# PengfeiRen96/DIR

Measured on AMD Instinct MI355X. Metric: images/sec at 256x256 bs=64, 3 stage outputs (DIR.forward eval), higher is better.
Workload: dtype f16

## Files before the change

### dir_amd/_capi.py

```python
import ctypes as C
import os

_HERE = os.path.dirname(os.path.abspath(__file__))
LIB_PATH = os.environ.get('DIR_LIB_PATH') or os.path.join(_HERE, 'lib', 'libdir_hip.so')
_lib = None


class DirHipError(RuntimeError):
    pass


class ManoTables(C.Structure):
    _fields_ = [('shapedirs_t', C.c_void_p), ('posedirs_t', C.c_void_p), ('v_template', C.c_void_p),
                ('j_template', C.c_void_p), ('j_shapedirs', C.c_void_p), ('weights', C.c_void_p), ('hands_mean', C.c_void_p),
                ('comps', C.c_void_p), ('side', C.c_int32), ('center_idx', C.c_int32), ('root_palm', C.c_int32)]


class ConvDesc(C.Structure):
    _fields_ = [(n, C.c_int32) for n in (
        'B', 'H', 'W', 'Cin', 'in_cstride', 'in_coff', 'Cout', 'out_cstride', 'out_coff', 'res_cstride', 'res_coff',
        'kh', 'kw', 'stride', 'pad', 'in_dtype', 'out_dtype', 'flags', 'Ho', 'Wo')] + [('in_scale', C.c_float), ('out_split_scale', C.c_float)]


class ConvBnBwd(C.Structure):
    _fields_ = [(n, C.c_void_p) for n in ('z', 'mean', 'rstd', 'w', 'b')] + [('relu', C.c_int32)] + [(n, C.c_void_p) for n in ('p1', 'p2')]


class ConvSrc2(C.Structure):
    _fields_ = [(n, C.c_int32) for n in ('H', 'W', 'Cin', 'in_cstride', 'in_coff', 'stride')]


class TrainWeight(C.Structure):
    _fields_ = [(n, C.c_void_p) for n in ('w', 'fwd', 'fwd_scale', 'dgrad', 'dgrad_scale')] + [(n, C.c_int32) for n in ('Cout', 'Cin', 'kh', 'kw')] + [
        ('fwd_inv_in', C.c_float), ('dgrad_inv_in', C.c_float)]


class BneckChainParams(C.Structure):
    _fields_ = [(n, C.c_void_p) for n in ('w2', 'scale2', 'shift2', 'w3', 'scale3', 'shift3', 'w1n', 'scale1n', 'shift1n', 'wd')] + [
        ('n_next', C.c_int32), ('out_decimate', C.c_int32), ('dtype', C.c_int32)]


class BneckTailParams(C.Structure):
    _fields_ = [(n, C.c_void_p) for n in ('wstream', 'scale3', 'shift3', 'scale1n', 'shift1n')] + [('planes', C.c_int32), ('n_next', C.c_int32), ('waves', C.c_int32), ('dtype', C.c_int32)]


class ResChainParams(C.Structure):
    _fields_ = [(n, C.c_void_p) for n in ('w1', 'w2', 'w3', 'pre_scale', 'pre_shift', 'scale1', 'shift1', 'scale2', 'shift2', 'shift3')] + [
        (n, C.c_int32) for n in ('Cin', 'Cmid', 'Cout', 'dtype')]


class GemmDesc(C.Structure):
    _fields_ = [(n, C.c_int32) for n in ('M', 'N', 'K', 'lda', 'ldb', 'ldc', 'trans_a', 'trans_b', 'accumulate', 'batch')] + \
               [(n, C.c_int64) for n in ('stride_a', 'stride_b', 'stride_c')]


class GemmGroups(C.Structure):
    _fields_ = [(n, C.c_int32) for n in ('ny', 'nx', 'reduce', 'reserved')] + [(n, C.c_int64) for n in ('a_y', 'a_x', 'b_y', 'b_x', 'c_y', 'c_x')]


class TokenMlp(C.Structure):
    _fields_ = [(n, C.c_void_p) for n in ('w1t', 's1', 'b1', 'w2t', 'b2')]


class PgcnLayer(C.Structure):
    _fields_ = [(n, C.c_void_p) for n in ('W', 'e1', 'bias', 'bn_scale', 'bn_shift')] + [('relu', C.c_int32), ('w_dtype', C.c_int32)]


class SteBlock(C.Structure):
    _fields_ = [(n, C.c_void_p) for n in ('ln1_w', 'ln1_b', 'qkv_wt', 'qkv_b', 'proj_wt', 'proj_b', 'ln2_w', 'ln2_b',
                                          'fc1_wt', 'fc1_b', 'fc2_wt', 'fc2_b')]


class SteParams(C.Structure):
    _fields_ = [('pos_embed', C.c_void_p), ('blocks', SteBlock * 3), ('num_blocks', C.c_int32)] + \
               [(n, C.c_void_p) for n in ('snorm_w', 'snorm_b', 'head_ln_w', 'head_ln_b', 'head_wt', 'head_b')] + \
               [('weight_dtype', C.c_int32)]


class RegressParams(C.Structure):
    _fields_ = [('mano_wt', C.c_void_p), ('mano_b', C.c_void_p * 2), ('off_w', C.c_void_p), ('off_b', C.c_void_p),
                ('emb', TokenMlp)]


class InitHeadParams(C.Structure):
    _fields_ = [('attn_w', C.c_void_p * 2), ('attn_b', C.c_float * 2), ('mano_wt', C.c_void_p),
                ('mano_b', C.c_void_p * 2), ('off_w', C.c_void_p), ('off_b', C.c_void_p)]


class BoneFusionParams(C.Structure):
    _fields_ = [(n, C.c_void_p) for n in ('w_g', 'scale', 'shift')] + [('exact_f32', C.c_int32), ('g_scale', C.c_float)]


class EvalInputs(C.Structure):
    _fields_ = [('verts_pd', C.c_void_p * 2), ('pd_offset', C.c_void_p), ('verts_gt', C.c_void_p * 2),
                ('verts2d_gt', C.c_void_p * 2), ('cam', C.c_void_p), ('jr', C.c_void_p * 2)]


class LossPred(C.Structure):
    _fields_ = [('joint_uv', C.c_void_p * 2), ('mesh_uv', C.c_void_p * 2), ('proj', C.c_void_p * 2), ('joint_xyz', C.c_void_p * 2),
                ('mesh_xyz', C.c_void_p * 2), ('offset', C.c_void_p)]


class LossTarget(C.Structure):
    _fields_ = [('joint_2d', C.c_void_p * 2), ('mesh_2d', C.c_void_p * 2), ('joint_3d', C.c_void_p * 2),
                ('mesh_3d', C.c_void_p * 2), ('center', C.c_void_p * 2), ('faces', C.c_void_p * 2),
                ('c2', C.c_int32), ('n_faces', C.c_int32)]


class LossPredGrad(C.Structure):
    _fields_ = [('joint_uv', C.c_void_p * 2), ('mesh_uv', C.c_void_p * 2), ('joint_xyz', C.c_void_p * 2),
                ('mesh_xyz', C.c_void_p * 2), ('offset', C.c_void_p)]


class EvalOutputs(C.Structure):
    _fields_ = [(n, C.c_void_p) for n in ('joint_err', 'vert_err', 'joint2d_err', 'vert2d_err', 'joints_pd', 'joints_gt',
                                          'root_err')]


class ValMetricsDesc(C.Structure):
    _fields_ = [('joints_pd', (C.c_void_p * 2) * 8), ('verts_pd', (C.c_void_p * 2) * 8), ('joints_gt', C.c_void_p * 2),
                ('verts_gt', C.c_void_p * 2), ('sample_sums', C.c_void_p), ('acc', C.c_void_p), ('batches', C.c_void_p)]


class FrameDesc(C.Structure):
    _fields_ = [('offset', C.c_longlong), ('height', C.c_int32), ('width', C.c_int32), ('row_stride', C.c_longlong)]


class OneEuroSegment(C.Structure):
    _fields_ = [('n_points', C.c_int32), ('dims', C.c_int32), ('speed_scale', C.c_float)]


class RenderLights(C.Structure):
    _fields_ = [('ambient', C.c_float * 3), ('diffuse', C.c_float * 3), ('specular', C.c_float * 3), ('location', C.c_float * 3),
                ('shininess', C.c_float)]


ABI_VERSION = 48
DT_F32, DT_BF16, DT_F16X3, DT_F16X1, DT_F16X3P, DT_F16X1P, DT_F16 = 0, 1, 3, 4, 5, 6, 7
CONV_RELU, CONV_PRE_RELU = 1, 2

_p, _i = C.c_void_p, C.c_int
_SIGNATURES = {
    'dir_abi_version': (C.c_int, []),
    'dir_last_error': (C.c_char_p, []),
    'dir_device_info': (C.c_int, [C.c_char_p, _i, C.POINTER(C.c_int)]),
    'dir_launch_log_reset': (None, []),
    'dir_launch_log_get': (C.c_int, [C.c_char_p, _i]),
    'dir_launch_log_note': (None, [C.c_char_p, C.c_longlong]),
    'dir_probe_launch': (C.c_longlong, [_i, _p, C.c_longlong, _i, _p]),
    'dir_conv2d_forward': (C.c_int, [C.POINTER(ConvDesc), _p, _p, _p, _p, _p, _p, _p, _p, _p]),
    'dir_conv2d_forward_stats': (C.c_int, [C.POINTER(ConvDesc), _p, _p, _p, _p, _p, _p, _p, _p, _p, C.POINTER(C.c_int), _p]),
    'dir_conv2d_forward_masked': (C.c_int, [C.POINTER(ConvDesc), _p, _p, _p, _p, _p, _p, _p, _p, _p, _p]),
    'dir_conv2d_forward_ex': (C.c_int, [C.POINTER(ConvDesc), _p, _p, _p, _p, _p, _p, _p, _p, _p, C.POINTER(ConvBnBwd), C.POINTER(C.c_int), _p]),
    'dir_add_upsampled': (C.c_int, [_p, _p, _i, _i, _i, _i, _i, _i, _i, _p]),
    'dir_fuse_sum': (C.c_int, [_p, _p, _p, _p, _i, _i, _i, _i, _i, _i, _i, _p]),
    'dir_pack_f16x3_weights': (C.c_int, [_p, _p, _p, _p, _i, _i, _p]),
    'dir_train_pack_conv_weights': (C.c_int, [_p, _p, _i, _i, _p]),
    'dir_gemm_f32_splitk_workspace_bytes': (C.c_longlong, [C.POINTER(GemmDesc)]),
    'dir_gemm_f32_splitk': (C.c_int, [C.POINTER(GemmDesc), _p, _p, _p, _p, _p, C.c_longlong, _p]),
    'dir_axpy_multi_f32': (C.c_int, [_p, _p, _p, _i, C.c_float, _p]),
    'dir_split_f16_forward': (C.c_int, [_p, _p, C.c_longlong, _i, _i, _i, _p, _p, _i, C.c_float, _i, _p]),
    'dir_stem_prep': (C.c_int, [_p, _p, _i, _i, _i, _i, _i, _i, _i, _p]),
    'dir_stem_prep_s2d': (C.c_int, [_p, _p, _i, _i, _i, _i, _i, _i, _p]),
    'dir_image_normalize_forward': (C.c_int, [_p, _p, C.POINTER(C.c_float), C.POINTER(C.c_float), _i, _i, _i, _p]),
    'dir_stem_prep_s2d_u8': (C.c_int, [_p, _p, C.POINTER(C.c_float), C.POINTER(C.c_float), _i, _i, _i, _i, _i, _i, _p]),
    'dir_adamw_step': (C.c_int, [_p, _p, _p, _p, C.c_longlong, C.c_double, C.c_double, C.c_double, C.c_double, C.c_double,
                                 C.c_longlong, _p]),
    'dir_stage_losses_backward': (C.c_int, [C.POINTER(LossPred), C.POINTER(LossTarget), C.c_float, _p, C.POINTER(C.c_void_p * 2),
                                            C.POINTER(C.c_void_p * 2), C.POINTER(LossPredGrad), _i, _p]),
    'dir_dense_losses_backward_workspace_bytes': (C.c_longlong, [_i, _i]),
    'dir_dense_losses_backward': (C.c_int, [_p, _p, _p, _p, C.POINTER(C.c_float), C.c_float, _p, _p, C.c_longlong, _p, _p, _i, _i, _i, _i, _p]),
    'dir_stage_losses_forward': (C.c_int, [C.POINTER(LossPred), C.POINTER(LossTarget), C.c_float, _p, _p, _i, _p]),
    'dir_dense_losses_workspace_bytes': (C.c_longlong, [_i, _i]),
    'dir_dense_losses_forward': (C.c_int, [_p, _p, _p, _p, C.POINTER(C.c_float), C.c_float, _p, C.c_longlong, _p, _i, _i, _i, _i, _p]),
    'dir_bottleneck_chain_forward': (C.c_int, [C.POINTER(BneckChainParams), _p, _p, _p, _p, _p, _i, _i, _i, _p]),
    'dir_bottleneck_tail_forward': (C.c_int, [C.POINTER(BneckTailParams), _p, _p, _p, _p, C.c_longlong, _p]),
    'dir_residual_chain_supported': (C.c_int, [_i] * 11),
    'dir_residual_chain_forward': (C.c_int, [C.POINTER(ResChainParams), _p, _p, _i, _i, _i, _i, _i, _i, _i, _p]),
    'dir_stem_pool_forward': (C.c_int, [_p, _i, C.POINTER(C.c_float), C.POINTER(C.c_float), _p, _p, _p, _p, _i, _i, _i, _p]),
    'dir_stem_pool_forward_dt': (C.c_int, [_p, _i, _i, C.POINTER(C.c_float), C.POINTER(C.c_float), _p, _p, _p, _p, _i, _i, _i, _p]),
    'dir_maxpool3x3s2': (C.c_int, [_p, _p, _i, _i, _i, _i, _i, _p]),
    'dir_upsample2x_bilinear': (C.c_int, [_p, _p, _i, _i, _i, _i, _i, _i, _i, _p]),
    'dir_init_head_forward': (C.c_int, [C.POINTER(InitHeadParams), _p, _p, _p, _i, _p, _p, _p, _i, _i, _i, _i, _i, _p]),
    'dir_bone_proj_forward': (C.c_int, [_p, _p, _p, _p, _p, _p, _i, _i, C.c_float, _i, _p]),
    'dir_conv2d_dual_forward': (C.c_int, [C.POINTER(ConvDesc), _p, C.POINTER(ConvSrc2), _p, _p, _p, _p, _p]),
    'dir_conv2d_dual_scaled_forward': (C.c_int, [C.POINTER(ConvDesc), _p, C.POINTER(ConvSrc2), _p, _p, _p, _p, _p, _p]),
    'dir_conv1x1_stream_forward': (C.c_int, [C.POINTER(ConvDesc), _p, C.POINTER(ConvSrc2), _p, _p, _p, _p, _p, _p, _p, _p]),
    'dir_conv2d_as_supported': (C.c_int, [C.POINTER(ConvDesc), _i, _i]),
    'dir_conv2d_as_forward': (C.c_int, [C.POINTER(ConvDesc), _p, _p, _p, _p, _p, _p, _i, _i, _p]),
    'dir_conv2d_as_chain_supported': (C.c_int, [C.POINTER(ConvDesc), _i, _i]),
    'dir_conv2d_as_chain_forward': (C.c_int, [C.POINTER(ConvDesc), _p, _p, _p, _p, _p, _p, _p, _i, _i, _p, _i, _i, _i, _p]),
    'dir_conv2d_sparse_forward': (C.c_int, [C.POINTER(ConvDesc), _p, _p, _p, _p, _p, _p, _p, _p]),
    'dir_grid_tokens_forward': (C.c_int, [_p, _i, _i, _i, _i, _i, _p, _p, _p, _p, _p, C.POINTER(TokenMlp),
                                          C.POINTER(TokenMlp), C.POINTER(TokenMlp), _p, _p, _i, _p]),
    'dir_pgcn_stack_forward': (C.c_int, [C.POINTER(PgcnLayer), _i, _p, _p, _p, C.c_longlong, _p, _i, _p]),
    'dir_pgcn_stack_forward_pair': (C.c_int, [C.POINTER(PgcnLayer), C.POINTER(PgcnLayer), _i, _p, _p, _p, _p, _i, _p]),
    'dir_pgcn_fused_sync_bytes': (C.c_longlong, []),
    'dir_pgcn_stack_forward_fused': (C.c_int, [C.POINTER(PgcnLayer), C.POINTER(PgcnLayer), _i, _p, _p, _p, _p, _p, _i, _i, _p]),
    'dir_ste_forward': (C.c_int, [C.POINTER(SteParams), _p, _p, _p, _i, _p]),
    'dir_regress_forward': (C.c_int, [C.POINTER(RegressParams), _p, _p, _p, _p, _p, _p, _p, _p, _i, _p]),
    'dir_bone_fusion_scratch_bytes': (C.c_size_t, [_i]),
    'dir_bone_fusion_prepare': (C.c_int, [C.POINTER(BoneFusionParams), _p, _p, _i, _p]),
    'dir_bone_fusion_forward': (C.c_int, [C.POINTER(BoneFusionParams), _p, _p, _p, _p, _i, _i, C.c_float, _i, _i, _i, _p]),
    'dir_bone_fusion_backward_workspace_bytes': (C.c_longlong, [_i, _i]),
    'dir_bone_fusion_backward': (C.c_int, [_p, _p, _p, _p, _p, _p, C.c_float, _p, _p, _p, _p, _p, C.c_longlong, _i, _i, _p]),
    'dir_gt_mano_forward': (C.c_int, [C.POINTER(ManoTables), _p, _p, _i, _p, _p, _p, _i, _i, _p, _p, _i, _p]),
    'dir_joint_regress_forward': (C.c_int, [_p, _p, _p, _i, _p]),
    'dir_eval_metrics_forward': (C.c_int, [C.POINTER(EvalInputs), C.POINTER(EvalOutputs), _i, _i, _i, _p]),
    'dir_val_metrics_forward': (C.c_int, [C.POINTER(ValMetricsDesc), _i, _i, _p]),
    'dir_mano_forward_pair': (C.c_int, [C.POINTER(ManoTables), _p, _i, _p, _i, _p, _i, _p, _p, _p, _p, _p, _i, _p]),
    'dir_mano_backward_pair': (C.c_int, [C.POINTER(ManoTables), _p, _i, _p, _i, _p, _i, _p, _p, _p, _p, _p, _i, _p, _i, _p, _i, _i, _i, _p]),
    'dir_regress_backward': (C.c_int, [_p] * 17 + [_i, _p]),
    'dir_gemm_f32': (C.c_int, [C.POINTER(GemmDesc), _p, _p, _p, _p, _p]),
    'dir_gemm_f32_grouped': (C.c_int, [C.POINTER(GemmDesc), C.POINTER(GemmGroups), _p, _p, _p, _p, _p]),
    'dir_colsum_workspace_bytes': (C.c_longlong, [_i, _i]),
    'dir_colsum_f32': (C.c_int, [_p, _p, _i, _i, _i, _i, _p, C.c_longlong, _p]),
    'dir_layernorm_forward': (C.c_int, [_p, _p, _p, _p, _p, _p, _i, _i, C.c_float, _p]),
    'dir_layernorm_backward': (C.c_int, [_p, _p, _p, _p, _p, _p, _p, _p, _i, _i, _i, _i, _p]),
    'dir_gelu_forward': (C.c_int, [_p, _p, C.c_longlong, _p]),
    'dir_gelu_backward': (C.c_int, [_p, _p, _p, C.c_longlong, _p]),
    'dir_attention_forward': (C.c_int, [_p, _p, _p, _i, _i, _i, C.c_float, _p]),
    'dir_attention_backward': (C.c_int, [_p, _p, _p, _p, _i, _i, _i, C.c_float, _p]),
    'dir_bn_train_workspace_bytes': (C.c_longlong, [_i, _i]),
    'dir_bn_train_forward': (C.c_int, [_p, _p, _p, _p, _p, _p, _p, _p, _i, _i, _i, C.c_float, C.c_float, _i, _p, _p, C.c_longlong, _p]),
    'dir_bn_train_backward_from_partials': (C.c_int, [_p, _p, _p, _p, _p, _p, _p, _p, _i, _p, _p, _p, _i, _i, _i, _i, _p, C.c_longlong, _p]),
    'dir_bn_train_stats': (C.c_int, [_p, _p, _p, _p, _p, _p, _p, _p, _p, _i, _i, _i, C.c_float, C.c_float, _p, C.c_longlong, _p]),
    'dir_bn_train_stats_from_partials': (C.c_int, [_p, _p, _i, _i, _p, _p, _p, _p, _p, _p, _p, _p, _i, _i, C.c_float, C.c_float, _p]),
    'dir_bn_train_apply': (C.c_int, [_p, _p, _p, _p, _p, _p, _i, _i, _i, _i, _p, _p]),
    'dir_bn_train_forward_from_partials': (C.c_int, [_p, _p, _p, _i, _i, _p, _p, _p, _p, _p, _p, _p, _i, _i, _i, C.c_float, C.c_float, _i, _p, _p]),
    'dir_bn_one_launch_status': (C.c_int, []),
    'dir_upsample_nearest_add_f32': (C.c_int, [_p, _p, _i, _i, _i, _i, _i, _p]),
    'dir_upsample_nearest_backward_f32': (C.c_int, [_p, _p, _i, _i, _i, _i, _i, _p]),
    'dir_bn_one_launch_enable': (C.c_int, [_i]),
    'dir_bn_train_backward': (C.c_int, [_p, _p, _p, _p, _p, _p, _p, _p, _p, _i, _i, _i, _i, _p, C.c_longlong, _p]),
    'dir_bn_frozen_workspace_bytes': (C.c_longlong, [_i, _i]),
    'dir_bn_sync_workspace_bytes': (C.c_longlong, [_i, _i]),
    'dir_bn_sync_local_stats': (C.c_int, [_p, _p, _i, _i, _i, _p, C.c_longlong, _p]),
    'dir_bn_sync_combine': (C.c_int, [_p, _i, _i, _p, _p, _p, _p, C.c_float, _p]),
    'dir_bn_sync_backward_sums': (C.c_int, [_p, _p, _p, _p, _p, _p, _p, _i, _i, _i, _i, _p, C.c_longlong, _p]),
    'dir_bn_sync_backward_apply': (C.c_int, [_p, _p, _p, _p, _p, _p, _p, _p, _i, C.c_float, _i, _i, _i, _p]),
    'dir_bn_frozen_forward': (C.c_int, [_p, _p, _p, _p, _p, _p, _p, _p, _i, _i, _i, C.c_float, _i, _p, _p]),
    'dir_bn_frozen_backward': (C.c_int, [_p, _p, _p, _p, _p, _p, _p, _p, _p, _i, _i, _i, _i, _p, C.c_longlong, _p]),
    'dir_relu_forward': (C.c_int, [_p, _p, C.c_longlong, _p]),
    'dir_relu_backward': (C.c_int, [_p, _p, _p, C.c_longlong, _p]),
    'dir_pgcn_adjacency_forward': (C.c_int, [_p, _p, _p]),
    'dir_pgcn_adjacency_backward': (C.c_int, [_p, _p, _p, _p, _p, _i, _p]),
    'dir_conv2d_splitk_workspace_bytes': (C.c_longlong, [C.POINTER(ConvDesc), _i]),
    'dir_conv2d_splitk_forward': (C.c_int, [C.POINTER(ConvDesc), _p, _p, _p, _p, _p, _p, _p, _p, _i, _p, C.c_longlong, _p]),
    'dir_conv2d_wgrad_workspace_bytes': (C.c_longlong, [C.POINTER(ConvDesc)]),
    'dir_conv2d_wgrad_f32': (C.c_int, [C.POINTER(ConvDesc), _p, _p, _p, _i, _p, C.c_longlong, _p]),
    'dir_conv2d_wgrad_f16x3_workspace_bytes': (C.c_longlong, [C.POINTER(ConvDesc)]),
    'dir_conv2d_wgrad_f16x3': (C.c_int, [C.POINTER(ConvDesc), _p, _p, _p, _i, _p, C.c_longlong, C.c_float, C.c_float, _p]),
    'dir_conv2d_wgrad_f16x3_pre': (C.c_int, [C.POINTER(ConvDesc), _p, _p, _p, _i, _p, C.c_longlong, C.c_float, C.c_float, _p, _p, _i, _p]),
    'dir_maxpool3x3s2_backward': (C.c_int, [_p, _p, _p, _i, _i, _i, _i, _p]),
    'dir_upsample2x_bilinear_backward': (C.c_int, [_p, _p, _i, _i, _i, _i, _i, _i, _p]),
    'dir_attn_pool_forward': (C.c_int, [_p, _p, _p, _p, _p, _i, _i, _i, _p]),
    'dir_attn_pool_backward': (C.c_int, [_p, _p, _p, _p, _p, _p, _p, _i, _i, _i, _i, _p]),
    'dir_bone_proj_backward_scratch_bytes': (C.c_longlong, [_i, _i]),
    'dir_bone_proj_backward': (C.c_int, [_p, _p, _p, _i, _i, C.c_float, _p, _p, _p, _i, _i, _i, _p]),
    'dir_axpy_f32': (C.c_int, [_p, _p, C.c_longlong, C.c_float, _p]),
    'dir_stage_positions': (C.c_int, [_p, _p, _p, _p, _p, _p, _p, _i, _p]),
    'dir_grid_rows_forward': (C.c_int, [_p, _p, _p, _i, _i, _i, _p]),
    'dir_grid_rows_backward': (C.c_int, [_p, _p, _i, _p, _i, _i, _i, _i, _p]),
    'dir_mano_forward': (C.c_int, [C.POINTER(ManoTables), _p, _i, _p, _i, _p, _i, _p, _p, _p, _p, _p, _i, _p]),
    'dir_jpeg_planes_bytes': (C.c_longlong, [C.c_longlong]),
    'dir_jpeg_decode_records': (C.c_int, [_p, C.c_longlong, _i, _i, _i, _p, C.c_longlong, _p, _p, _p]),
    'dir_train_noise_field': (C.c_int, [C.c_ulonglong, _p, _i, _p]),
    'dir_train_augment_images': (C.c_int, [_p, _p, _p, _p, _p, C.c_ulonglong, C.POINTER(C.c_float), C.POINTER(C.c_float), _p, _p, _p, _p, _p,
                                           _p, _i, _p]),
    'dir_train_augment_labels': (C.c_int, [_p, C.POINTER(C.c_void_p * 8), _p, C.POINTER(C.c_void_p * 10), _i, _p]),
    'dir_render_workspace_bytes': (C.c_longlong, [_i]),
    'dir_render_two_hands': (C.c_int, [_p, _p, _p, _p, _i, _i, _p, C.c_longlong, _p, _p, _p, _p, _p, _p, _p]),
    'dir_render_adjacency_bytes': (C.c_longlong, []),
    'dir_render_adjacency': (C.c_int, [_p, _p, C.c_longlong, _p]),
    'dir_render_vertex_normals': (C.c_int, [_p, _p, _p, _i, _p, _p]),
    'dir_render_shaded_workspace_bytes': (C.c_longlong, [_i]),
    'dir_render_joints': (C.c_int, [_p, _p, _p, _i, _i, C.c_float, C.c_float, _p]),
    'dir_render_shaded': (C.c_int, [_p, _p, _p, _p, _p, _p, _p, C.POINTER(RenderLights), _p, _i, _i, _p, C.c_longlong, _p, _p, _p, _p, _p, _p]),
    'dir_mesh_penetration': (C.c_int, [_p, _p, _p, _p, _i, _i, _i, _i, _i, _p, _p, _p, _p, _p, _p]),
    'dir_mesh_intersection_volume': (C.c_int, [_p, _p, _p, _p, _i, _i, _i, _i, _i, C.c_float, _i, _p, _p, _p, _p]),
    'dir_procrustes_align': (C.c_int, [_p, _p, _i, _i, _i, _p, _p, _p, _p]),
    'dir_point_set_nn': (C.c_int, [_p, _p, _i, _i, _i, _p, _p, _p]),
    'dir_threshold_counts': (C.c_int, [_p, C.c_longlong, _p, _i, _p, _p]),
    'dir_crop_matrices_from_boxes': (C.c_int, [_p, _i, C.c_double, _i, _p, _p, _p]),
    'dir_crop_matrices_from_meshes': (C.c_int, [_p, _p, _p, _p, _p, _i, C.c_double, _i, _p, _p, _p]),
    'dir_crop_frames': (C.c_int, [_p, C.c_longlong, _p, _p, _p, _i, _i, _p, _p, _p]),
    'dir_crop_frames_area': (C.c_int, [_p, C.c_longlong, _p, _p, _p, _i, _i, _p, _p, _p, _p]),
    'dir_one_euro_state_bytes': (C.c_longlong, [_i, _i, C.POINTER(C.c_longlong)]),
    'dir_one_euro_step': (C.c_int, [_p, _p, _i, C.POINTER(OneEuroSegment), _i, C.c_double, C.c_double, C.c_double, C.c_double, _i, _p, _p, _p, _p]),
}


PROFILE = None
_pending = {}
_NO_PROFILE = ('dir_conv2d_as_supported', 'dir_conv2d_as_chain_supported', 'dir_residual_chain_supported', 'dir_abi_version', 'dir_bn_one_launch_status', 'dir_bn_one_launch_enable', 'dir_last_error', 'dir_device_info', 'dir_launch_log_reset', 'dir_launch_log_get', 'dir_launch_log_note',
               'dir_bone_fusion_scratch_bytes', 'dir_dense_losses_workspace_bytes', 'dir_dense_losses_backward_workspace_bytes',
               'dir_gemm_f32_splitk_workspace_bytes', 'dir_bn_train_workspace_bytes', 'dir_bn_sync_workspace_bytes', 'dir_bn_frozen_workspace_bytes', 'dir_jpeg_planes_bytes', 'dir_render_workspace_bytes', 'dir_render_adjacency_bytes', 'dir_render_shaded_workspace_bytes', 'dir_colsum_workspace_bytes', 'dir_conv2d_wgrad_workspace_bytes', 'dir_conv2d_wgrad_f16x3_workspace_bytes',
               'dir_one_euro_state_bytes')


def annotate(**kw):
    if PROFILE is not None:
        _pending.update(kw)


class _ProfLib(object):
    def __init__(self, l):
        self._l = l

    def __getattr__(self, name):
        fn = getattr(self._l, name)
        if name in _NO_PROFILE:
            return fn
        import torch

        def call(*args):
            e0, e1 = torch.cuda.Event(enable_timing=True), torch.cuda.Event(enable_timing=True)
            self._l.dir_launch_log_reset()
            e0.record()
            rc = fn(*args)
            e1.record()
            buf = C.create_string_buffer(1024)
            self._l.dir_launch_log_get(buf, 1024)
            rec = dict(_pending, api=name, kernels=buf.value.decode(), e0=e0, e1=e1)
            _pending.clear()
            PROFILE.append(rec)
            return rc
        return call


def lib():
    global _lib
    if _lib is not None and PROFILE is not None:
        return _ProfLib(_lib)
    if _lib is None:
        import torch
        if not os.path.exists(LIB_PATH):
            raise DirHipError('%s is missing: build it with `python -c "import __graft_entry__ as g; g.build()"` '
                              '(or python dir_amd/build.py). There is no CPU fallback.' % LIB_PATH)
        l = C.CDLL(LIB_PATH)
        for name, (res, args) in _SIGNATURES.items():
            fn = getattr(l, name)
            fn.restype, fn.argtypes = res, args
        if l.dir_abi_version() != ABI_VERSION:
            raise DirHipError('libdir_hip.so ABI version %d != %d' % (l.dir_abi_version(), ABI_VERSION))
        _lib = l
    return _ProfLib(_lib) if PROFILE is not None else _lib


def check(rc, what):
    if rc != 0:
        raise DirHipError('%s failed (%d): %s' % (what, rc, lib().dir_last_error().decode()))


def ptr(t):
    return None if t is None else C.c_void_p(t.data_ptr())


def stream_ptr():
    import torch
    return C.c_void_p(torch.cuda.current_stream().cuda_stream)


def require_cuda(*tensors):
    for t in tensors:
        if t is not None and not t.is_cuda:
            raise DirHipError('dir_amd kernels run on the GPU only: got a %s tensor (no CPU fallback exists)'
                              % t.device)


def f32c(t):
    import torch
    if t.dtype != torch.float32:
        t = t.float()
    return t if t.is_contiguous() else t.contiguous()
```

### dir_amd/csrc/tail.hip

```cpp
#include "conv_common.h"

namespace dir {
namespace {

using convk::bf16_t;
using convk::f16s_t;
using convk::f32x16;
using convk::Half;
typedef __attribute__((ext_vector_type(4))) float f32x4;

#ifndef DIR_TAIL_RES16
#define DIR_TAIL_RES16 1
#endif
#ifndef DIR_TAIL_NT
#define DIR_TAIL_NT 0
#endif
#if DIR_TAIL_NT
typedef unsigned __attribute__((ext_vector_type(2))) u32x2_t;
typedef unsigned __attribute__((ext_vector_type(4))) u32x4_t;
__device__ __forceinline__ uint2 nt_load2(const uint2* p) { const u32x2_t v = __builtin_nontemporal_load(reinterpret_cast<const u32x2_t*>(p)); return make_uint2(v.x, v.y); }
__device__ __forceinline__ void nt_store4(uint4 v, uint4* p) { __builtin_nontemporal_store(u32x4_t{v.x, v.y, v.z, v.w}, reinterpret_cast<u32x4_t*>(p)); }
#define NT_LOAD(p) nt_load2(p)
#define NT_STORE(v, p) nt_store4(v, p)
#else
#define NT_LOAD(p) (*(p))
#define NT_STORE(v, p) (*(p) = (v))
#endif

constexpr int TM = 64;
constexpr int HC = 512;
constexpr int NTHR = 512;
constexpr int TPITCH = HC * 2 + 16;

struct TailArgs {
    const bf16_t* y2; const bf16_t* res; bf16_t* out; bf16_t* y1n;
    const uint4* wstream;
    const float* sc3; const float* sh3; const float* sc1n; const float* sh1n;
    int ntiles; unsigned y2_bytes;
};

template <typename H> __device__ __forceinline__ void unpack4(uint2 v, float (&f)[4]) {
    convk::unpack2<H>(v.x, f[0], f[1]);
    convk::unpack2<H>(v.y, f[2], f[3]);
}

template <int P, int N2, typename H = bf16_t>
__global__ __launch_bounds__(NTHR, 1) void tail_chain_kernel(TailArgs a) {
    convk::half_kernel_init<H>();
    constexpr int C4 = 4 * P, NH = C4 / HC;
    constexpr int YROW = P * 2;
    constexpr int GRP = P == 256 ? 4 : 8;
    constexpr int KBS = P / 16;
    constexpr int NBF = 2 * KBS;
    constexpr bool C16 = N2 == 128;
    constexpr int NCF = C16 ? HC / 32 : HC / 16;
    constexpr int NF = NBF + NCF, NG = NF / GRP;
    static_assert(NF % GRP == 0 && C4 % HC == 0 && (N2 == 128 || N2 == 256), "tail_chain_kernel: unsupported geometry");
    constexpr int YCH = TM * (P / 8) / NTHR;
    __shared__ __attribute__((aligned(16))) char s_t[TM * TPITCH];
    __shared__ __attribute__((aligned(16))) char s_y2[2][TM * YROW];
    __shared__ __attribute__((aligned(16))) float s_ss[2 * C4 + 2 * N2];
    const int tid = threadIdx.x, lane = tid & 63, wave = __builtin_amdgcn_readfirstlane(tid >> 6);
    const int l32 = lane & 31, h = lane >> 5, l16 = lane & 15, g16 = lane >> 4;

    for (int i = tid; i < C4; i += NTHR) { s_ss[i] = a.sc3[i]; s_ss[C4 + i] = a.sh3[i]; }
    for (int i = tid; i < N2; i += NTHR) { s_ss[2 * C4 + i] = a.sc1n[i]; s_ss[2 * C4 + N2 + i] = a.sh1n[i]; }

    const int tstep = gridDim.x;
    int t = blockIdx.x;
    if (t >= a.ntiles) return;

    const convk::i32x4 yd = {(int)(unsigned)(unsigned long long)a.y2, (int)(unsigned)((unsigned long long)a.y2 >> 32), (int)a.y2_bytes, 0x00020000};
    const unsigned y2_lds = (unsigned)(unsigned long long)(__attribute__((address_space(3))) char*)&s_y2[0][0];
    auto y2_dma = [&](int tile, int buf) {
#pragma unroll
        for (int i = 0; i < YCH; ++i) {
            const int slot = (8 * i + wave) * 64 + lane, px = slot / (P / 8), pos = slot % (P / 8);
            const unsigned voff = (unsigned)(((long long)tile * TM + px) * YROW) + (unsigned)((pos ^ (px & 15)) * 16);
            convk::lds_dma16_m0(yd, y2_lds + buf * (TM * YROW) + (8 * i + wave) * 1024, voff, 0);
        }
    };
#if DIR_TAIL_RES16
    uint4 xr[2][2][2];
    auto res_fetch = [&](int tile, int half) {
#pragma unroll
        for (int pb = 0; pb < 2; ++pb) {
            const bf16_t* rp = a.res + ((long long)tile * TM + 32 * pb + l32) * C4 + half * HC + 64 * wave + 8 * h;
#pragma unroll
            for (int cb = 0; cb < 2; ++cb)
#pragma unroll
                for (int j = 0; j < 2; ++j) xr[cb][pb][j] = *reinterpret_cast<const uint4*>(rp + 32 * cb + 16 * j);
        }
#else
    uint2 xr[2][2][4];
    auto res_fetch = [&](int tile, int half) {
#pragma unroll
        for (int pb = 0; pb < 2; ++pb) {
            const bf16_t* rp = a.res + ((long long)tile * TM + 32 * pb + l32) * C4 + half * HC + 64 * wave + 4 * h;
#pragma unroll
            for (int cb = 0; cb < 2; ++cb)
#pragma unroll
                for (int q = 0; q < 4; ++q) xr[cb][pb][q] = NT_LOAD(reinterpret_cast<const uint2*>(rp + 32 * cb + 8 * q));
        }
#endif
    };
    uint4 ring[2][GRP];
    auto ring_load = [&](auto Slot, int hf, int grp) {
        constexpr int slot = decltype(Slot)::value;
        const uint4* p = a.wstream + ((long long)(hf * 8 + wave) * NF + grp * GRP) * 64 + lane;
#pragma unroll
        for (int i = 0; i < GRP; ++i) ring[slot][i] = p[i * 64];
    };

    y2_dma(t, 0);
    ring_load(std::integral_constant<int, 0>{}, 0, 0);
    res_fetch(t, 0);
    convk::wait_vmcnt<0>();
    __syncthreads();
    int ybuf = 0;

    f32x16 accb[2];
    f32x16 accc32[C16 ? 1 : 2];
    f32x4 accc16[C16 ? 4 : 1];
    constexpr int NOP = C16 ? 4 : 2;
    uint4 bop[2][NOP];
    const char* ycur = s_y2[0];
    auto act_read = [&](auto F, auto Set) {
        constexpr int f = decltype(F)::value, set = decltype(Set)::value;
        if constexpr (f < NBF) {
            constexpr int ks = f % KBS;
#pragma unroll
            for (int pb = 0; pb < 2; ++pb)
                bop[set][pb] = *reinterpret_cast<const uint4*>(ycur + (32 * pb + l32) * YROW + (((2 * ks + h) ^ (l32 & 15)) << 4));
        } else {
            constexpr int fc = f - NBF;
            if constexpr (C16) {
#pragma unroll
                for (int u = 0; u < 4; ++u) bop[set][u] = *reinterpret_cast<const uint4*>(s_t + (16 * u + l16) * TPITCH + 64 * fc + 16 * g16);
            } else {
#pragma unroll
                for (int pb = 0; pb < 2; ++pb) bop[set][pb] = *reinterpret_cast<const uint4*>(s_t + (32 * pb + l32) * TPITCH + 32 * fc + 16 * h);
            }
        }
    };

    for (; t < a.ntiles; t += tstep) {
        const bool more = t + tstep < a.ntiles;
        if (more) y2_dma(t + tstep, ybuf ^ 1);
        ycur = s_y2[ybuf];
#pragma nounroll
        for (int hf = 0; hf < NH; ++hf) {
            const bool last_half = hf == NH - 1;
            if (hf == 0) {
                if constexpr (C16) {
#pragma unroll
                    for (int u = 0; u < 4; ++u) accc16[u] = f32x4{0.f, 0.f, 0.f, 0.f};
                } else {
#pragma unroll
                    for (int pb = 0; pb < 2; ++pb)
#pragma unroll
                        for (int r = 0; r < 16; ++r) accc32[pb][r] = 0.f;
                }
            }
            act_read(std::integral_constant<int, 0>{}, std::integral_constant<int, 0>{});
            [&]<int... G>(std::integer_sequence<int, G...>) {
                (([&] {
                     constexpr int grp = G, slot = G & 1;
                     if constexpr (grp + 1 < NG) ring_load(std::integral_constant<int, slot ^ 1>{}, hf, grp + 1);
                     else ring_load(std::integral_constant<int, slot ^ 1>{}, last_half ? 0 : hf + 1, 0);
                     [&]<int... I>(std::integer_sequence<int, I...>) {
                         (([&] {
                              constexpr int f = grp * GRP + I, set = f & 1;
                              if constexpr (f + 1 < NF && f + 1 != NBF) act_read(std::integral_constant<int, f + 1>{}, std::integral_constant<int, set ^ 1>{});
                              if constexpr (f < NBF) {
                                  constexpr int cb = f / KBS, ks = f - cb * KBS;
                                  if constexpr (ks == 0) {
#pragma unroll
                                      for (int pb = 0; pb < 2; ++pb)
#pragma unroll
                                          for (int r = 0; r < 16; ++r) accb[pb][r] = 0.f;
                                  }
#pragma unroll
                                  for (int pb = 0; pb < 2; ++pb)
                                      accb[pb] = Half<H>::mfma32(ring[slot][I], bop[set][pb], accb[pb]);
                                  if constexpr (ks == KBS - 1) {
#pragma unroll
                                      for (int q = 0; q < 4; ++q) {
                                          const int cl = 64 * wave + 32 * cb + 8 * q + 4 * h;
                                          const float4 sc = *reinterpret_cast<const float4*>(s_ss + hf * HC + cl);
                                          const float4 sh = *reinterpret_cast<const float4*>(s_ss + C4 + hf * HC + cl);
#pragma unroll
                                          for (int pb = 0; pb < 2; ++pb) {
                                              float v[4] = {fmaf(accb[pb][4 * q], sc.x, sh.x), fmaf(accb[pb][4 * q + 1], sc.y, sh.y),
                                                            fmaf(accb[pb][4 * q + 2], sc.z, sh.z), fmaf(accb[pb][4 * q + 3], sc.w, sh.w)};
                                              float rv[4];
#if DIR_TAIL_RES16
                                              {
                                                  const uint4 c = xr[cb][pb][q >> 1];
                                                  const auto sx = __builtin_amdgcn_permlane32_swap(c.x, c.z, false, false);
                                                  const auto sy = __builtin_amdgcn_permlane32_swap(c.y, c.w, false, false);
                                                  unpack4<H>(make_uint2(sx[q & 1], sy[q & 1]), rv);
                                              }
#else
                                              unpack4<H>(xr[cb][pb][q], rv);
#endif
#pragma unroll
                                              for (int e = 0; e < 4; ++e) v[e] += rv[e];
                                              uint2 o;
                                              o.x = Half<H>::pack2_relu(v[0], v[1]);
                                              o.y = Half<H>::pack2_relu(v[2], v[3]);
                                              *reinterpret_cast<uint2*>(s_t + (32 * pb + l32) * TPITCH + cl * 2) = o;
                                          }
                                          __builtin_amdgcn_sched_barrier(0);
                                      }
                                  }
                                  if constexpr (f == NBF - 1) {
                                      __syncthreads();
                                      act_read(std::integral_constant<int, NBF>{}, std::integral_constant<int, set ^ 1>{});
                                      if (!last_half) res_fetch(t, hf + 1);
                                      else if (more) res_fetch(t + tstep, 0);
#pragma unroll
                                      for (int i = 0; i < TM * (HC / 8) / NTHR; ++i) {
                                          const int c = tid + NTHR * i;
                                          NT_STORE(*reinterpret_cast<const uint4*>(s_t + (c >> 6) * TPITCH + (c & 63) * 16),
                                                   reinterpret_cast<uint4*>(a.out + ((long long)t * TM + (c >> 6)) * C4 + hf * HC + (c & 63) * 8));
                                          if (i & 1) __builtin_amdgcn_sched_barrier(0);
                                      }
                                  }
                              } else {
                                  if constexpr (C16) {
#pragma unroll
                                      for (int u = 0; u < 4; ++u)
                                          accc16[u] = Half<H>::mfma16(ring[slot][I], bop[set][u], accc16[u]);
                                  } else {
#pragma unroll
                                      for (int pb = 0; pb < 2; ++pb)
                                          accc32[pb] = Half<H>::mfma32(ring[slot][I], bop[set][pb], accc32[pb]);
                                  }
                              }
                              if constexpr (f == NF - 1) convk::wait_vmcnt<GRP>();
                              __builtin_amdgcn_sched_barrier(0);
                          }()),
                          ...);
                     }(std::make_integer_sequence<int, GRP>{});
                 }()),
                 ...);
            }(std::make_integer_sequence<int, NG>{});
            if (last_half) {
                if constexpr (C16) {
                    const int c0 = 16 * wave + 4 * g16;
                    const float4 sc = *reinterpret_cast<const float4*>(s_ss + 2 * C4 + c0);
                    const float4 sh = *reinterpret_cast<const float4*>(s_ss + 2 * C4 + N2 + c0);
#pragma unroll
                    for (int u = 0; u < 4; ++u) {
                        uint2 o;
                        o.x = Half<H>::pack2_relu(fmaf(accc16[u][0], sc.x, sh.x), fmaf(accc16[u][1], sc.y, sh.y));
                        o.y = Half<H>::pack2_relu(fmaf(accc16[u][2], sc.z, sh.z), fmaf(accc16[u][3], sc.w, sh.w));
                        *reinterpret_cast<uint2*>(a.y1n + ((long long)t * TM + 16 * u + l16) * N2 + c0) = o;
                    }
                } else {
#pragma unroll
                    for (int pb = 0; pb < 2; ++pb) {
                        uint2 o[4];
#pragma unroll
                        for (int q = 0; q < 4; ++q) {
                            const int c0 = 32 * wave + 8 * q + 4 * h;
                            const float4 sc = *reinterpret_cast<const float4*>(s_ss + 2 * C4 + c0);
                            const float4 sh = *reinterpret_cast<const float4*>(s_ss + 2 * C4 + N2 + c0);
                            o[q].x = Half<H>::pack2_relu(fmaf(accc32[pb][4 * q], sc.x, sh.x), fmaf(accc32[pb][4 * q + 1], sc.y, sh.y));
                            o[q].y = Half<H>::pack2_relu(fmaf(accc32[pb][4 * q + 2], sc.z, sh.z), fmaf(accc32[pb][4 * q + 3], sc.w, sh.w));
                        }
#if DIR_TAIL_RES16
#pragma unroll
                        for (int j = 0; j < 2; ++j) {
                            const auto dx = __builtin_amdgcn_permlane32_swap(o[2 * j].x, o[2 * j + 1].x, false, false);
                            const auto dy = __builtin_amdgcn_permlane32_swap(o[2 * j].y, o[2 * j + 1].y, false, false);
                            *reinterpret_cast<uint4*>(a.y1n + ((long long)t * TM + 32 * pb + l32) * N2 + 32 * wave + 16 * j + 8 * h) = make_uint4(dx[0], dy[0], dx[1], dy[1]);
                        }
#else
#pragma unroll
                        for (int q = 0; q < 4; ++q)
                            *reinterpret_cast<uint2*>(a.y1n + ((long long)t * TM + 32 * pb + l32) * N2 + 32 * wave + 8 * q + 4 * h) = o[q];
#endif
                    }
                }
            }
            __syncthreads();
        }
        ybuf ^= 1;
    }
}


constexpr int TTM = 32, TTHR = 256;

template <int P, int N2, typename H = bf16_t>
__global__ __launch_bounds__(TTHR, 2) void tail_thin_kernel(TailArgs a) {
    convk::half_kernel_init<H>();
    constexpr int C4 = 4 * P, NH = C4 / HC;
    constexpr int YROW = P * 2;
    constexpr int GRP = 8;
    constexpr int KBS = P / 16;
    constexpr int NBF = 4 * KBS;
    constexpr int NCC = N2 / 128;
    constexpr int NCF = 32 * NCC;
    constexpr int NF = NBF + NCF, NG = NF / GRP;
    static_assert(NF % GRP == 0 && NG % 2 == 0 && C4 % HC == 0 && (N2 == 128 || N2 == 256), "tail_thin_kernel: unsupported geometry");
    constexpr int YCH = TTM * (P / 8) / TTHR;
    __shared__ __attribute__((aligned(16))) char s_t[TTM * TPITCH];
    __shared__ __attribute__((aligned(16))) char s_y2[2][TTM * YROW];
    __shared__ __attribute__((aligned(16))) float s_ss[2 * C4 + 2 * N2];
    const int tid = threadIdx.x, lane = tid & 63, wave = __builtin_amdgcn_readfirstlane(tid >> 6);
    const int l32 = lane & 31, h = lane >> 5;

    for (int i = tid; i < C4; i += TTHR) { s_ss[i] = a.sc3[i]; s_ss[C4 + i] = a.sh3[i]; }
    for (int i = tid; i < N2; i += TTHR) { s_ss[2 * C4 + i] = a.sc1n[i]; s_ss[2 * C4 + N2 + i] = a.sh1n[i]; }

    const int tstep = gridDim.x;
    int t = blockIdx.x;
    if (t >= a.ntiles) return;

    const convk::i32x4 yd = {(int)(unsigned)(unsigned long long)a.y2, (int)(unsigned)((unsigned long long)a.y2 >> 32), (int)a.y2_bytes, 0x00020000};
    const unsigned y2_lds = (unsigned)(unsigned long long)(__attribute__((address_space(3))) char*)&s_y2[0][0];
    auto y2_dma = [&](int tile, int buf) {
#pragma unroll
        for (int i = 0; i < YCH; ++i) {
            const int slot = (4 * i + wave) * 64 + lane, px = slot / (P / 8), pos = slot % (P / 8);
            const unsigned voff = (unsigned)(((long long)tile * TTM + px) * YROW) + (unsigned)((pos ^ (px & 15)) * 16);
            convk::lds_dma16_m0(yd, y2_lds + buf * (TTM * YROW) + (4 * i + wave) * 1024, voff, 0);
        }
    };
    uint2 xr[4][4];
    auto res_fetch = [&](int tile, int half) {
        const bf16_t* rp = a.res + ((long long)tile * TTM + l32) * C4 + half * HC + 128 * wave + 4 * h;
#pragma unroll
        for (int cb = 0; cb < 4; ++cb)
#pragma unroll
            for (int q = 0; q < 4; ++q) xr[cb][q] = NT_LOAD(reinterpret_cast<const uint2*>(rp + 32 * cb + 8 * q));
    };
    uint4 ring[2][GRP];
    auto ring_load = [&](auto Slot, int hf, int grp) {
        constexpr int slot = decltype(Slot)::value;
        const uint4* p = a.wstream + ((long long)(hf * 4 + wave) * NF + grp * GRP) * 64 + lane;
#pragma unroll
        for (int i = 0; i < GRP; ++i) ring[slot][i] = p[i * 64];
    };

    y2_dma(t, 0);
    ring_load(std::integral_constant<int, 0>{}, 0, 0);
    res_fetch(t, 0);
    convk::wait_vmcnt<0>();
    __syncthreads();
    int ybuf = 0;

    f32x16 accb;
    f32x16 accc[NCC];
    uint4 bop[2];
    const char* ycur = s_y2[0];
    auto act_read = [&](auto F, auto Set) {
        constexpr int f = decltype(F)::value, set = decltype(Set)::value;
        if constexpr (f < NBF) {
            constexpr int ks = f % KBS;
            bop[set] = *reinterpret_cast<const uint4*>(ycur + l32 * YROW + (((2 * ks + h) ^ (l32 & 15)) << 4));
        } else {
            constexpr int ks = (f - NBF) / NCC;
            bop[set] = *reinterpret_cast<const uint4*>(s_t + l32 * TPITCH + 32 * ks + 16 * h);
        }
    };

    for (; t < a.ntiles; t += tstep) {
        const bool more = t + tstep < a.ntiles;
        if (more) y2_dma(t + tstep, ybuf ^ 1);
        ycur = s_y2[ybuf];
#pragma nounroll
        for (int hf = 0; hf < NH; ++hf) {
            const bool last_half = hf == NH - 1;
            if (hf == 0) {
#pragma unroll
                for (int cc = 0; cc < NCC; ++cc)
#pragma unroll
                    for (int r = 0; r < 16; ++r) accc[cc][r] = 0.f;
            }
            act_read(std::integral_constant<int, 0>{}, std::integral_constant<int, 0>{});
            [&]<int... G>(std::integer_sequence<int, G...>) {
                (([&] {
                     constexpr int grp = G, slot = G & 1;
                     if constexpr (grp + 1 < NG) ring_load(std::integral_constant<int, slot ^ 1>{}, hf, grp + 1);
                     else ring_load(std::integral_constant<int, slot ^ 1>{}, last_half ? 0 : hf + 1, 0);
                     [&]<int... I>(std::integer_sequence<int, I...>) {
                         (([&] {
                              constexpr int f = grp * GRP + I;
                              constexpr bool same_next = f >= NBF && f + 1 < NF && (f - NBF) / NCC == (f + 1 - NBF) / NCC;
                              constexpr int set = f < NBF ? (f & 1) : ((((f - NBF) / NCC) + NBF) & 1);
                              if constexpr (f + 1 < NF && f + 1 != NBF && !same_next)
                                  act_read(std::integral_constant<int, f + 1>{}, std::integral_constant<int, set ^ 1>{});
                              if constexpr (f < NBF) {
                                  constexpr int cb = f / KBS, ks = f - cb * KBS;
                                  if constexpr (ks == 0) {
#pragma unroll
                                      for (int r = 0; r < 16; ++r) accb[r] = 0.f;
                                  }
                                  accb = Half<H>::mfma32(ring[slot][I], bop[set], accb);
                                  if constexpr (ks == KBS - 1) {
#pragma unroll
                                      for (int q = 0; q < 4; ++q) {
                                          const int cl = 128 * wave + 32 * cb + 8 * q + 4 * h;
                                          const float4 sc = *reinterpret_cast<const float4*>(s_ss + hf * HC + cl);
                                          const float4 sh = *reinterpret_cast<const float4*>(s_ss + C4 + hf * HC + cl);
                                          float v[4] = {fmaf(accb[4 * q], sc.x, sh.x), fmaf(accb[4 * q + 1], sc.y, sh.y),
                                                        fmaf(accb[4 * q + 2], sc.z, sh.z), fmaf(accb[4 * q + 3], sc.w, sh.w)};
                                          float rv[4];
                                          unpack4<H>(xr[cb][q], rv);
#pragma unroll
                                          for (int e = 0; e < 4; ++e) v[e] += rv[e];
                                          uint2 o;
                                          o.x = Half<H>::pack2_relu(v[0], v[1]);
                                          o.y = Half<H>::pack2_relu(v[2], v[3]);
                                          *reinterpret_cast<uint2*>(s_t + l32 * TPITCH + cl * 2) = o;
                                      }
                                  }
                                  if constexpr (f == NBF - 1) {
                                      __syncthreads();
                                      act_read(std::integral_constant<int, NBF>{}, std::integral_constant<int, (NBF & 1)>{});
                                      if (!last_half) res_fetch(t, hf + 1);
                                      else if (more) res_fetch(t + tstep, 0);
#pragma unroll
                                      for (int i = 0; i < TTM * (HC / 8) / TTHR; ++i) {
                                          const int c = tid + TTHR * i;
                                          NT_STORE(*reinterpret_cast<const uint4*>(s_t + (c >> 6) * TPITCH + (c & 63) * 16),
                                                   reinterpret_cast<uint4*>(a.out + ((long long)t * TTM + (c >> 6)) * C4 + hf * HC + (c & 63) * 8));
                                          if (i & 1) __builtin_amdgcn_sched_barrier(0);
                                      }
                                  }
                              } else {
                                  constexpr int cc = (f - NBF) % NCC;
                                  accc[cc] = Half<H>::mfma32(ring[slot][I], bop[set], accc[cc]);
                              }
                              if constexpr (f == NF - 1) convk::wait_vmcnt<GRP>();
                              __builtin_amdgcn_sched_barrier(0);
                          }()),
                          ...);
                     }(std::make_integer_sequence<int, GRP>{});
                 }()),
                 ...);
            }(std::make_integer_sequence<int, NG>{});
            if (last_half) {
#pragma unroll
                for (int cc = 0; cc < NCC; ++cc)
#pragma unroll
                    for (int q = 0; q < 4; ++q) {
                        const int c0 = (N2 / 4) * wave + 32 * cc + 8 * q + 4 * h;
                        const float4 sc = *reinterpret_cast<const float4*>(s_ss + 2 * C4 + c0);
                        const float4 sh = *reinterpret_cast<const float4*>(s_ss + 2 * C4 + N2 + c0);
                        uint2 o;
                        o.x = Half<H>::pack2_relu(fmaf(accc[cc][4 * q], sc.x, sh.x), fmaf(accc[cc][4 * q + 1], sc.y, sh.y));
                        o.y = Half<H>::pack2_relu(fmaf(accc[cc][4 * q + 2], sc.z, sh.z), fmaf(accc[cc][4 * q + 3], sc.w, sh.w));
                        *reinterpret_cast<uint2*>(a.y1n + ((long long)t * TTM + l32) * N2 + c0) = o;
                    }
            }
            __syncthreads();
        }
        ybuf ^= 1;
    }
}

}
}

extern "C" int dir_bottleneck_tail_forward(const dir_bneck_tail_params* p, const void* y2, const void* residual, void* out, void* y1_next,
                                           long long M, void* stream) {
    using namespace dir;
    DIR_REQUIRE(p && y2 && residual && out && y1_next, "dir_bottleneck_tail_forward: null pointer");
    DIR_REQUIRE(p->wstream && p->scale3 && p->shift3 && p->scale1n && p->shift1n, "dir_bottleneck_tail_forward: missing parameters");
    DIR_REQUIRE(M > 0 && M % TM == 0 && M / TM < (1ll << 31), "dir_bottleneck_tail_forward: M must be a positive multiple of 64");
    DIR_REQUIRE(p->waves == 8 || p->waves == 4, "dir_bottleneck_tail_forward: the stream must be packed for 8 or 4 waves");
    DIR_REQUIRE(p->dtype == 0 || p->dtype == DIR_DT_BF16 || p->dtype == DIR_DT_F16, "dir_bottleneck_tail_forward: dtype must be bf16 (or 0) or f16");
    const bool f16 = p->dtype == DIR_DT_F16;
    TailArgs a;
    a.y2 = (const convk::bf16_t*)y2; a.res = (const convk::bf16_t*)residual; a.out = (convk::bf16_t*)out; a.y1n = (convk::bf16_t*)y1_next;
    a.wstream = (const uint4*)p->wstream; a.sc3 = p->scale3; a.sh3 = p->shift3; a.sc1n = p->scale1n; a.sh1n = p->shift1n;
    a.ntiles = (int)(M / TM);
    DIR_REQUIRE(M * p->planes * 2 < (1ll << 31), "dir_bottleneck_tail_forward: y2 must be < 2 GiB (32-bit buffer offsets)");
    a.y2_bytes = (unsigned)(M * p->planes * 2);
    static int num_cu = 0;
    if (!num_cu) {
        int dev = 0; hipDeviceProp_t pr;
        num_cu = (hipGetDevice(&dev) == hipSuccess && hipGetDeviceProperties(&pr, dev) == hipSuccess) ? pr.multiProcessorCount : 256;
    }
    hipStream_t s = (hipStream_t)stream;
    if (p->waves == 4) {
        a.ntiles = (int)(M / TTM);
        const int grid4 = a.ntiles < 2 * num_cu ? a.ntiles : 2 * num_cu;
#define DIR_TAIL4(P_, N2_) do { if (f16) DIR_LAUNCH((tail_thin_kernel<P_, N2_, f16s_t>), dim3(grid4), dim3(TTHR), 0, s, a); \
                                 else DIR_LAUNCH((tail_thin_kernel<P_, N2_, bf16_t>), dim3(grid4), dim3(TTHR), 0, s, a); } while (0)
        if (p->planes == 128 && p->n_next == 128) DIR_TAIL4(128, 128);
        else if (p->planes == 128 && p->n_next == 256) DIR_TAIL4(128, 256);
        else if (p->planes == 256 && p->n_next == 256) DIR_TAIL4(256, 256);
        else DIR_REQUIRE(false, "dir_bottleneck_tail_forward: (planes, n_next) must be (128,128), (128,256) or (256,256)");
#undef DIR_TAIL4
        return check_launch("dir_bottleneck_tail_forward");
    }
    const int grid = a.ntiles < num_cu ? a.ntiles : num_cu;
#define DIR_TAIL(P_, N2_) do { if (f16) DIR_LAUNCH((tail_chain_kernel<P_, N2_, f16s_t>), dim3(grid), dim3(NTHR), 0, s, a); \
                                else DIR_LAUNCH((tail_chain_kernel<P_, N2_, bf16_t>), dim3(grid), dim3(NTHR), 0, s, a); } while (0)
    if (p->planes == 128 && p->n_next == 128) DIR_TAIL(128, 128);
    else if (p->planes == 128 && p->n_next == 256) DIR_TAIL(128, 256);
    else if (p->planes == 256 && p->n_next == 256) DIR_TAIL(256, 256);
    else DIR_REQUIRE(false, "dir_bottleneck_tail_forward: (planes, n_next) must be (128,128), (128,256) or (256,256)");
#undef DIR_TAIL
    return check_launch("dir_bottleneck_tail_forward");
}
```

### dir_amd/engine.py

```python
import ctypes as C
import math
import json
import os
import threading

import torch

from . import _capi
from ._capi import CONV_PRE_RELU, CONV_RELU, DT_BF16, DT_F16, DT_F16X1, DT_F16X1P, DT_F16X3, DT_F16X3P, DT_F32, ConvDesc

F32 = torch.float32
IMAGENET_MEAN = (C.c_float * 3)(0.485, 0.456, 0.406)
IMAGENET_STD = (C.c_float * 3)(0.229, 0.224, 0.225)
_TLS = threading.local()


def _forced_variant():
    return getattr(_TLS, 'variant', None)


def _packing_arith():
    return getattr(_TLS, 'arith', None)


def _ann(family, flops, nbytes, shape):
    if _capi.PROFILE is not None:
        _capi.annotate(family=family, flops=float(flops), bytes=float(nbytes), shape=shape)


HALF = (torch.bfloat16, torch.float16)


def _dt(dtype):
    return DT_F32 if dtype == torch.float32 else DT_F16 if dtype == torch.float16 else DT_BF16


def _tok_wdt(dtype):
    return torch.bfloat16 if dtype in HALF else torch.float32


def bn_fold(sd, prefix, conv_bias=None, eps=1e-5):
    g, b = sd[prefix + '.weight'].double(), sd[prefix + '.bias'].double()
    m, v = sd[prefix + '.running_mean'].double(), sd[prefix + '.running_var'].double()
    scale = g / torch.sqrt(v + eps)
    shift = b - m * scale
    if conv_bias is not None:
        shift = shift + conv_bias.double() * scale
    return scale.float().contiguous(), shift.float().contiguous()


STREAM_VARIANT = 21
STREAM64_VARIANT = 22
STREAM32_VARIANT = 23
STREAMP_VARIANT = 24
STREAM_VARIANTS = (STREAM_VARIANT, STREAM64_VARIANT, STREAM32_VARIANT, STREAMP_VARIANT)
AS_VARIANTS = {25: (2, 2), 26: (2, 4), 27: (4, 2), 28: (1, 2)}


def pack_as_weights(w_ohwi, A):
    N, kh, kw, Cin = w_ohwi.shape
    assert N % (128 * A) == 0 and Cin % 64 == 0
    nt = kh * kw
    dev = w_ohwi.device
    w = w_ohwi.reshape(N, nt * Cin)
    lane = torch.arange(64, device=dev)
    l32, h = lane & 31, lane >> 5
    e = torch.arange(8, device=dev)
    g, wv, st, ks, cb = torch.meshgrid(torch.arange(N // (128 * A), device=dev), torch.arange(4, device=dev), torch.arange(nt * Cin // 64, device=dev),
                                       torch.arange(4, device=dev), torch.arange(A, device=dev), indexing='ij')
    row = (g * (128 * A) + (wv * A + cb) * 32)[..., None] + l32
    slab, tap = st // nt, st % nt
    k0 = (tap * Cin + 64 * slab + 8 * ks)[..., None] + 32 * h
    return w[row[..., None], k0[..., None] + e].contiguous()


def pack_stream_weights(w_nk, dtype=torch.bfloat16):
    out_dev = w_nk.device
    w = w_nk.detach().float().cpu()
    N, K = w.shape
    assert N % 128 == 0 and K % 64 == 0
    ncb = 2 if N % 256 == 0 else 1
    dev = w.device
    lane = torch.arange(64, device=dev)
    l32, h = lane & 31, lane >> 5
    e = torch.arange(8, device=dev)
    g, wv, c, ks, cb = torch.meshgrid(torch.arange(N // (128 * ncb), device=dev), torch.arange(4, device=dev), torch.arange(K // 64, device=dev),
                                      torch.arange(4, device=dev), torch.arange(ncb, device=dev), indexing='ij')
    row = (g * (128 * ncb) + (wv * ncb + cb) * 32)[..., None] + l32
    k0 = (64 * c + 8 * ks)[..., None] + 32 * h
    return w[row[..., None], k0[..., None] + e].to(dtype).contiguous().to(out_dev)


class ConvOp(object):
    def __init__(self, w_oihw, dtype, stride=1, pad=0, scale=None, shift=None, relu=False, pre=None, pre_relu=False,
                 out_dtype=None, arith=None):
        self.w = w_oihw.detach().permute(0, 2, 3, 1).contiguous().to(dtype)
        self.cout, self.kh, self.kw, self.cin = self.w.shape
        self.stride, self.pad, self.dtype = stride, pad, dtype
        self.out_dtype = out_dtype or dtype
        self.arith = (arith or _packing_arith()) if dtype == torch.float32 else None
        self.in_code = DT_F16X3 if self.arith == 'f16x3' else DT_F16X1 if self.arith == 'f16' else _dt(dtype)
        self.in_scale = 1.0
        if self.arith in ('f16x3', 'f16'):
            from .functional import pack_f16x3_weights
            self.w, scale = pack_f16x3_weights(self.w.reshape(self.cout, -1), scale)
            self.scale0 = scale.float().contiguous().clone()
        self.scale = None if scale is None else scale.float().contiguous()
        self.shift = None if shift is None else shift.float().contiguous()
        self.pre_scale, self.pre_shift = (None, None) if pre is None else (pre[0].contiguous(), pre[1].contiguous())
        self.flags = (CONV_RELU if relu else 0) | (CONV_PRE_RELU if pre_relu else 0)
        self.ho = self.wo = 0
        self.in_cs_override = None
        self.presplit = self.arith is not None and (ConvOp.PRESPLIT == 2 or (ConvOp.PRESPLIT == 1 and (
            self.kh * self.kw >= 9 or (self.cout >= 512 and self.cin >= 128))))
        self.split_consumer = None
        self.alg_k = self.kh * self.kw * self.cin
        self.variant = {}
        self.split, self._ws = {}, {}
        self._w_as = {}
        self.w_stream = None
        if (dtype in HALF and self.out_dtype == dtype and self.kh == 1 and self.kw == 1 and stride == 1 and pad == 0
                and self.cin % 64 == 0 and self.cout % 128 == 0 and self.cin <= 2304):
            self.w_stream = pack_stream_weights(self.w.reshape(self.cout, self.cin), dtype)

    PRESPLIT = int(os.environ.get('DIR_PRESPLIT', '1'))
    OUT_SPLIT = os.environ.get('DIR_OUT_SPLIT', '1') != '0'

    def link_split(self, consumer):
        if (self.arith is not None and isinstance(consumer, ConvOp) and consumer.arith == self.arith and consumer.pre_scale is None
                and consumer.in_cs_override is None and self.cout == consumer.cin and self.cout % 32 == 0 and self.out_dtype == F32):
            self.split_consumer = consumer

    def set_in_scale(self, s):
        assert self.arith in ('f16x3', 'f16') and s > 0 and math.frexp(s)[0] == 0.5
        self.in_scale = float(s)
        self.scale.copy_(self.scale0 / s)

    def _calibrate(self, xs):
        amax = max(float(t.abs().max()) for t in xs)
        if self.pre_scale is not None:
            amax = amax * float(self.pre_scale.abs().max()) + float(self.pre_shift.abs().max())
        self.set_in_scale(2.0 ** (10 - math.frexp(amax)[1]) if amax > 0 and math.isfinite(amax) else 1.0)

    def __call__(self, x, out=None, out_coff=0, in_coff=0, residual=None, res_coff=0, bbox=None, _replay_split=None):
        B, H, W, cbuf = x.shape
        x_arg, in_coff_arg = x, in_coff
        if self.arith is not None and getattr(_TLS, 'calibrating', False):
            self._calibrate([x[..., in_coff:in_coff + self.cin]] if self.in_cs_override is None else [x])
        ho = self.ho or (H + 2 * self.pad - self.kh) // self.stride + 1
        wo = self.wo or (W + 2 * self.pad - self.kw) // self.stride + 1
        out_given, residual_ok = out, True
        if out is None:
            out = torch.empty(B, ho, wo, self.cout, device=x.device, dtype=self.out_dtype)
        pre_scale, pre_shift, flags, in_code, in_cs = self.pre_scale, self.pre_shift, self.flags, self.in_code, self.in_cs_override or cbuf
        if getattr(x, '_dir_split', False):
            assert in_coff == 0 and cbuf == self.cin and pre_scale is None and bbox is None
            in_code = DT_F16X1P if self.arith == 'f16' else DT_F16X3P
        elif self.presplit and self.in_cs_override is None and bbox is None:
            xs = torch.empty(B, H, W, self.cin, device=x.device, dtype=F32)
            _ann('split_f16', 0, 2 * xs.numel() * 4, 'M=%d C=%d fp32 -> f16 hi | lo' % (B * H * W, self.cin))
            _capi.check(_capi.lib().dir_split_f16_forward(_capi.ptr(x), _capi.ptr(xs), B * H * W, self.cin, cbuf, in_coff, _capi.ptr(pre_scale), _capi.ptr(pre_shift),
                                                          1 if (flags & CONV_PRE_RELU) else 0, self.in_scale, 1 if self.arith == 'f16' else 0, _capi.stream_ptr()),
                        'dir_split_f16_forward')
            x, in_cs, in_coff, pre_scale, pre_shift = xs, self.cin, 0, None, None
            flags &= ~CONV_PRE_RELU
            in_code = DT_F16X1P if self.arith == 'f16' else DT_F16X3P
        d = ConvDesc(B, H, W, self.cin, in_cs, in_coff, self.cout, out.shape[3], out_coff,
                     residual.shape[3] if residual is not None else 0, res_coff, self.kh, self.kw, self.stride, self.pad,
                     in_code, _dt(out.dtype), flags, self.ho, self.wo, self.in_scale)
        cons = self.split_consumer
        write_split = (cons is not None and out_given is None and residual_ok and not getattr(_TLS, 'calibrating', False)
                       and not getattr(_TLS, 'no_out_split', False) and ConvOp.OUT_SPLIT)
        if _replay_split is not None:
            write_split = _replay_split
        if getattr(_TLS, 'capture', None) is not None:
            _TLS.capture.append((self, (x_arg,), dict(out=out, out_coff=out_coff, in_coff=in_coff_arg, residual=residual, res_coff=res_coff, bbox=bbox,
                                                  _replay_split=write_split)))
        if write_split:
            d.out_split_scale = -cons.in_scale if cons.arith == 'f16' else cons.in_scale
        v = _forced_variant() if _forced_variant() is not None else self.variant.get(B, self.variant.get(getattr(_TLS, 'parent_batch', None), 0))
        d.flags |= (v & 0xff) << 8
        if _capi.PROFILE is not None:
            nbytes = (B * H * W * self.cin * x.element_size() + self.w.numel() * self.w.element_size()
                      + B * ho * wo * self.cout * out.element_size() * (2 if residual is not None else 1))
            _capi.annotate(family='conv', flops=2.0 * B * ho * wo * self.cout * self.alg_k, bytes=nbytes, op=self, flops_real=2.0 * B * ho * wo * self.cout * self.alg_k * getattr(self, 'alg_scale', 1.0),
                           dtype=self.arith or ('f32' if self.dtype == F32 else 'bf16'),
                           shape='M=%d N=%d K=%d k%dx%d s%d' % (B * ho * wo, self.cout, self.kh * self.kw * self.cin, self.kh,
                                                              self.kw, self.stride))
        if v in AS_VARIANTS and bbox is None and pre_scale is None and self.dtype in HALF and out.dtype == self.dtype and self.arith is None:
            A_, PB_ = AS_VARIANTS[v]
            if _capi.lib().dir_conv2d_as_supported(d, A_, PB_):
                was = self._w_as.get(A_)
                if was is None:
                    was = self._w_as[A_] = pack_as_weights(self.w, A_)
                d.flags &= 0xff
                _capi.check(_capi.lib().dir_conv2d_as_forward(d, _capi.ptr(x), _capi.ptr(was), _capi.ptr(self.scale), _capi.ptr(self.shift), _capi.ptr(residual),
                                                              _capi.ptr(out), A_, PB_, _capi.stream_ptr()), 'dir_conv2d_as_forward')
                return out
            d.flags &= 0xff
        if v in STREAM_VARIANTS and self.w_stream is not None and residual is None and bbox is None and out.dtype == self.dtype:
            d.flags = (d.flags & 0xff) | ((v & 0xff) << 8 if v != STREAM_VARIANT else 0)
            _capi.check(_capi.lib().dir_conv1x1_stream_forward(d, _capi.ptr(x), None, None, _capi.ptr(self.w_stream), _capi.ptr(self.scale),
                                                               _capi.ptr(self.shift), _capi.ptr(self.pre_scale), _capi.ptr(self.pre_shift),
                                                               _capi.ptr(out), _capi.stream_ptr()), 'dir_conv1x1_stream_forward')
            return out
        S = self.splits(B, ho, wo) if (bbox is None and out.dtype in HALF and self.dtype in HALF) else 1
        if S > 1 and (_forced_variant() in (None, 0)):
            d.flags &= 0xff
            ws = self._splitk_ws(d, S, B, x.device)
            _capi.check(_capi.lib().dir_conv2d_splitk_forward(d, _capi.ptr(x), _capi.ptr(self.w), _capi.ptr(self.scale), _capi.ptr(self.shift),
                                                              _capi.ptr(self.pre_scale), _capi.ptr(self.pre_shift), _capi.ptr(residual),
                                                              _capi.ptr(out), S, _capi.ptr(ws), ws.numel(), _capi.stream_ptr()),
                        'dir_conv2d_splitk_forward')
            return out
        if bbox is not None:
            rc = _capi.lib().dir_conv2d_sparse_forward(d, _capi.ptr(x), _capi.ptr(self.w), _capi.ptr(self.scale),
                                                       _capi.ptr(self.shift), _capi.ptr(residual), _capi.ptr(out),
                                                       _capi.ptr(bbox), _capi.stream_ptr())
        else:
            rc = _capi.lib().dir_conv2d_forward(d, _capi.ptr(x), _capi.ptr(self.w), _capi.ptr(self.scale),
                                                _capi.ptr(self.shift), _capi.ptr(pre_scale),
                                                _capi.ptr(pre_shift), _capi.ptr(residual), _capi.ptr(out),
                                                _capi.stream_ptr())
        _capi.check(rc, 'dir_conv2d_forward')
        if write_split:
            out._dir_split = True
        return out


    SPLITK = os.environ.get('DIR_SPLITK', '0') == '1'

    def splits(self, B, ho, wo):
        S = self.split.get(B)
        if S is None:
            S = 1
            tiles = -(-(B * ho * wo) // 128) * -(-self.cout // 128)
            nk = self.kh * self.kw * self.cin // 64
            if ConvOp.SPLITK and self.cout % 8 == 0 and tiles <= 128 and nk >= 8:
                S = max(1, min(16, nk // 4, -(-512 // tiles)))
            self.split[B] = S
        return S

    def _splitk_ws(self, d, S, B, dev):
        key = (B, S, torch.cuda.current_stream(dev).cuda_stream)
        ws = self._ws.get(key)
        if ws is None:
            n = _capi.lib().dir_conv2d_splitk_workspace_bytes(d, S)
            assert n > 0
            ws = torch.empty(n, dtype=torch.uint8, device=dev)
            ws[:16384].zero_()
            self._ws[key] = ws
        return ws


class DualConvOp(object):
    def __init__(self, w3, s3, h3, wds, sds, hds, stride2, dtype, relu=True):
        self.relu = relu
        self.cout, self.cin = w3.shape[0], w3.shape[1]
        self.cin2, self.stride2, self.dtype = wds.shape[1], stride2, dtype
        w = torch.cat([w3.float().flatten(1) * s3.float()[:, None], wds.float().flatten(1) * sds.float()[:, None]], 1)
        self.w = w.contiguous().to(dtype)
        self.arith = _packing_arith() if dtype == torch.float32 else None
        self.scale = None
        if self.arith is not None:
            from .functional import pack_f16x3_weights
            self.w, self.scale = pack_f16x3_weights(self.w)
            self.scale0 = self.scale.clone()
        self.in_scale = 1.0
        self.shift = (h3.float() + hds.float()).contiguous()
        self.kh = self.kw = self.stride = 1
        self.pre_scale = None
        self.variant = {}
        self.w_stream = None
        if dtype in HALF and self.cin % 64 == 0 and self.cin2 % 64 == 0 and self.cout % 128 == 0:
            self.w_stream = pack_stream_weights(self.w, dtype)

    set_in_scale = ConvOp.set_in_scale
    pre_scale = None

    def __call__(self, y, x, out=None, out_coff=0, x_decimated=False):
        B, H, W, cbuf = y.shape
        if self.arith is not None and getattr(_TLS, 'calibrating', False):
            ConvOp._calibrate(self, [y[..., :self.cin], x[..., :self.cin2]])
        if out is None:
            out = torch.empty(B, H, W, self.cout, device=y.device, dtype=self.dtype)
        if getattr(_TLS, 'capture', None) is not None:
            _TLS.capture.append((self, (y, x), dict(out=out, out_coff=out_coff, x_decimated=x_decimated)))
        d = ConvDesc(B, H, W, self.cin, cbuf, 0, self.cout, out.shape[3], out_coff, 0, 0, 1, 1, 1, 0,
                     DT_F16X3 if self.arith == 'f16x3' else DT_F16X1 if self.arith == 'f16' else _dt(self.dtype), _dt(self.dtype),
                     CONV_RELU if self.relu else 0, 0, 0, self.in_scale)
        v = _forced_variant() if _forced_variant() is not None else self.variant.get(B, self.variant.get(getattr(_TLS, 'parent_batch', None), 0))
        d.flags |= (v & 0xff) << 8
        d2 = _capi.ConvSrc2(x.shape[1], x.shape[2], self.cin2, x.shape[3], 0, 1 if x_decimated else self.stride2)
        if _capi.PROFILE is not None:
            es, m = y.element_size(), B * H * W
            _capi.annotate(family='conv', flops=2.0 * m * self.cout * (self.cin + self.cin2), op=self,
                           bytes=(m * self.cin + m * self.cin2 + self.w.numel() + m * self.cout) * es,
                           dtype=self.arith or ('f32' if self.dtype == F32 else 'bf16'),
                           shape='M=%d N=%d K=%d+%d dual s%d' % (m, self.cout, self.cin, self.cin2, self.stride2))
        if v in STREAM_VARIANTS and self.w_stream is not None:
            d.flags = (d.flags & 0xff) | ((v & 0xff) << 8 if v != STREAM_VARIANT else 0)
            _capi.check(_capi.lib().dir_conv1x1_stream_forward(d, _capi.ptr(y), d2, _capi.ptr(x), _capi.ptr(self.w_stream), None, _capi.ptr(self.shift),
                                                               None, None, _capi.ptr(out), _capi.stream_ptr()), 'dir_conv1x1_stream_forward')
            return out
        if self.scale is not None:
            _capi.check(_capi.lib().dir_conv2d_dual_scaled_forward(d, _capi.ptr(y), d2, _capi.ptr(x), _capi.ptr(self.w), _capi.ptr(self.scale),
                                                                   _capi.ptr(self.shift), _capi.ptr(out), _capi.stream_ptr()),
                        'dir_conv2d_dual_scaled_forward')
            return out
        _capi.check(_capi.lib().dir_conv2d_dual_forward(d, _capi.ptr(y), d2, _capi.ptr(x), _capi.ptr(self.w), _capi.ptr(self.shift),
                                                        _capi.ptr(out), _capi.stream_ptr()), 'dir_conv2d_dual_forward')
        return out


def pack_token_mlp(sd, prefix, keep):
    w1 = sd[prefix + '.0.weight'][:, :, 0]
    s1, b1 = bn_fold(sd, prefix + '.1', sd[prefix + '.0.bias'])
    t = dict(w1t=w1.t().contiguous().float(), s1=s1, b1=b1,
             w2t=sd[prefix + '.3.weight'][:, :, 0].t().contiguous().float(), b2=sd[prefix + '.3.bias'].float().contiguous())
    keep.append(t)
    return _capi.TokenMlp(*(t[k].data_ptr() for k in ('w1t', 's1', 'b1', 'w2t', 'b2')))


def pack_pgcn(sd, prefix, keep, num_layers=4, weight_dtype=torch.float32):
    arr = (_capi.PgcnLayer * num_layers)()
    for i in range(num_layers):
        p = '%s.gconv_layers.%d' % (prefix, i)
        s, b = bn_fold(sd, p + '.bn')
        W = sd[p + '.gconv.W']
        W = W.float().contiguous() if weight_dtype == torch.float32 else W.detach().transpose(2, 3).contiguous().to(torch.bfloat16)
        t = dict(W=W, e1=sd[p + '.gconv.e_1'].float().reshape(-1).contiguous(),
                 bias=sd[p + '.gconv.bias'].float().contiguous(), s=s, b=b)
        keep.append(t)
        arr[i] = _capi.PgcnLayer(t['W'].data_ptr(), t['e1'].data_ptr(), t['bias'].data_ptr(), s.data_ptr(), b.data_ptr(), 1,
                                 _dt(weight_dtype))
    return arr


def pack_ste(sd, prefix, keep, depth=4, weight_dtype=torch.float32):
    def f(k):
        t = sd[prefix + '.' + k].float().contiguous()
        keep.append(t)
        return t.data_ptr()

    def ft(k):
        w = sd[prefix + '.' + k]
        t = w.float().t().contiguous() if weight_dtype == torch.float32 else w.detach().to(torch.bfloat16).contiguous()
        keep.append(t)
        return t.data_ptr()
    P = _capi.SteParams()
    P.weight_dtype = _dt(weight_dtype)
    pe = sd[prefix + '.spatial_pos_embed'].float().reshape(42, 128).contiguous()
    keep.append(pe)
    P.pos_embed = pe.data_ptr()
    for i in range(1, depth):
        b = 'STEblocks.%d.' % i
        P.blocks[i - 1] = _capi.SteBlock(f(b + 'norm1.weight'), f(b + 'norm1.bias'), ft(b + 'attn.qkv.weight'),
                                         f(b + 'attn.qkv.bias'), ft(b + 'attn.proj.weight'), f(b + 'attn.proj.bias'),
                                         f(b + 'norm2.weight'), f(b + 'norm2.bias'), ft(b + 'mlp.fc1.weight'),
                                         f(b + 'mlp.fc1.bias'), ft(b + 'mlp.fc2.weight'), f(b + 'mlp.fc2.bias'))
    P.num_blocks = depth - 1
    P.snorm_w, P.snorm_b = f('spatial_norm.weight'), f('spatial_norm.bias')
    P.head_ln_w, P.head_ln_b = f('head.0.weight'), f('head.0.bias')
    P.head_wt, P.head_b = ft('head.1.weight'), f('head.1.bias')
    return P


def _pad_rows(t, width=2336):
    out = torch.zeros(t.shape[0], width, device=t.device, dtype=torch.float32)
    out[:, :t.shape[1]] = t
    return out


def pack_mano(sd, prefix, side, center_idx, keep):
    f = lambda k: sd[prefix + '.' + k].float()
    t = dict(shapedirs_t=_pad_rows(f('th_shapedirs').reshape(2334, 10).t()),
             posedirs_t=_pad_rows(f('th_posedirs').reshape(2334, 135).t()),
             v_template=f('th_v_template').reshape(2334).contiguous(),
             j_template=(f('th_J_regressor').double() @ f('th_v_template').double().reshape(778, 3)).float().contiguous(),
             j_shapedirs=torch.einsum('jv,vck->jck', f('th_J_regressor').double(),
                                      f('th_shapedirs').double()).float().contiguous(),
             weights=f('th_weights').contiguous(), hands_mean=f('th_hands_mean').reshape(45).contiguous(),
             comps=f('th_selected_comps').contiguous())
    keep.append(t)
    return _capi.ManoTables(t['shapedirs_t'].data_ptr(), t['posedirs_t'].data_ptr(), t['v_template'].data_ptr(),
                            t['j_template'].data_ptr(), t['j_shapedirs'].data_ptr(), t['weights'].data_ptr(), t['hands_mean'].data_ptr(),
                            t['comps'].data_ptr(), 0 if side == 'right' else 1,
                            -1 if center_idx is None else int(center_idx), 0)


class BneckChainOp(object):

    def __init__(self, c2, c3, c1n=None, dual=None):
        self.c2, self.c3, self.c1n, self.dual = c2, c3, c1n, dual
        self.cout, self.cin, self.kh, self.kw, self.stride = 256, c2.cin, 3, 3, 1
        self.variant = {}
        dev = c2.w.device
        if dual is None:
            self.w3 = c3.w.reshape(c3.cout, c3.cin).contiguous()
            self.wd, self.s3, self.h3 = None, c3.scale, c3.shift
        else:
            self.w3 = dual.w[:, :64].contiguous()
            self.wd = dual.w[:, 64:].contiguous()
            self.s3, self.h3 = torch.ones(256, device=dev, dtype=F32), dual.shift
        self.w1n = c1n.w.reshape(c1n.cout, c1n.cin).contiguous() if c1n is not None else None
        n = (lambda t: None) if c1n is None else _capi.ptr
        self.params = _capi.BneckChainParams(_capi.ptr(c2.w), _capi.ptr(c2.scale), _capi.ptr(c2.shift), _capi.ptr(self.w3),
                                             _capi.ptr(self.s3), _capi.ptr(self.h3), n(self.w1n),
                                             n(c1n.scale if c1n is not None else None), n(c1n.shift if c1n is not None else None),
                                             _capi.ptr(self.wd) if self.wd is not None else None, c1n.cout if c1n is not None else 0, 0, _dt(c2.dtype))

    @staticmethod
    def applies(c2, c3, c1n, dtype, dual=None):
        ok = dtype in HALF and c2.cin == 64 and c2.cout == 64 and c2.kh == 3 and c2.stride == 1 and c2.scale is not None
        if dual is None:
            ok = ok and c3.cin == 64 and c3.cout == 256 and c3.scale is not None
        else:
            ok = ok and dual.cin == 64 and dual.cin2 == 64 and dual.cout == 256 and dual.stride2 == 1 and dual.relu
        return ok and (c1n is None or (c1n.cin == 256 and c1n.cout in (64, 128) and c1n.kh == 1 and c1n.stride == 1 and c1n.scale is not None))

    def __call__(self, y1, x, decimate=False):
        residual, x2 = (None, x) if self.dual is not None else (x, None)
        B, H, W, _ = y1.shape
        if getattr(_TLS, 'capture_fused', None) is not None:
            _TLS.capture_fused.append((self, (y1, x), dict(decimate=decimate)))
        self.params.out_decimate = 1 if decimate else 0
        out = torch.empty((B, H // 2, W // 2, 256) if decimate else (B, H, W, 256), device=y1.device, dtype=y1.dtype)
        y1n = torch.empty(B, H, W, self.c1n.cout, device=y1.device, dtype=y1.dtype) if self.c1n is not None else None
        if _capi.PROFILE is not None:
            m, nx = B * H * W, self.c1n is not None
            n2 = self.c1n.cout if nx else 0
            _capi.annotate(family='conv', flops=2.0 * m * (64 * 576 + 256 * 64 * (2 if x2 is not None else 1) + n2 * 256), op=self, dtype='bf16',
                           shape='M=%d chain 3x3(64)+1x1(256)%s' % (m, '+1x1(%d)' % n2 if nx else ''),
                           bytes=(m * (64 + 256 * (1 if residual is not None else 0) + (64 if decimate else 256) + n2 + (64 if x2 is not None else 0))
                                  + self.c2.w.numel() + self.w3.numel() * (2 if x2 is not None else 1) + (self.w1n.numel() if nx else 0)) * 2)
        _capi.check(_capi.lib().dir_bottleneck_chain_forward(C.byref(self.params), _capi.ptr(y1), _capi.ptr(residual), _capi.ptr(x2), _capi.ptr(out),
                                                             _capi.ptr(y1n), B, H, W, _capi.stream_ptr()), 'dir_bottleneck_chain_forward')
        return out, y1n


def pack_tail_stream(w3, w1n, waves=8, dtype=torch.bfloat16):
    out_dev = w3.device
    w3 = w3.detach().float().reshape(w3.shape[0], -1).cpu()
    w1n = w1n.detach().float().reshape(w1n.shape[0], -1).cpu()
    C4, P = w3.shape
    N2 = w1n.shape[0]
    assert w1n.shape[1] == C4 and C4 == 4 * P and C4 % 512 == 0 and N2 in (128, 256)
    dev = w3.device
    lane = torch.arange(64, device=dev)
    l32, h, l16, g16 = lane & 31, lane >> 5, lane & 15, lane >> 4
    e = torch.arange(8, device=dev)
    KBS = P // 16
    out = []
    if waves == 4:
        ncc = N2 // 128
        for hf in range(C4 // 512):
            for w in range(4):
                for cb in range(4):
                    for ks in range(KBS):
                        out.append(w3[(hf * 512 + 128 * w + 32 * cb + l32)[:, None], (16 * ks + 8 * h)[:, None] + e])
                for ks in range(32):
                    for cc in range(ncc):
                        out.append(w1n[((N2 // 4) * w + 32 * cc + l32)[:, None], (hf * 512 + 16 * ks + 8 * h)[:, None] + e])
        return torch.stack(out).to(dtype).contiguous().to(out_dev)
    for hf in range(C4 // 512):
        for w in range(8):
            for cb in range(2):
                for ks in range(KBS):
                    ch = hf * 512 + 64 * w + 32 * cb + l32
                    k0 = 16 * ks + 8 * h
                    out.append(w3[ch[:, None], k0[:, None] + e])
            if N2 == 128:
                for fc in range(16):
                    out.append(w1n[(16 * w + l16)[:, None], (hf * 512 + 32 * fc + 8 * g16)[:, None] + e])
            else:
                for fc in range(32):
                    out.append(w1n[(32 * w + l32)[:, None], (hf * 512 + 16 * fc + 8 * h)[:, None] + e])
    return torch.stack(out).to(dtype).contiguous().to(out_dev)


class BneckTailOp(object):
    GEOMETRIES = ((128, 128), (128, 256), (256, 256))
    THIN_MAX_TILES = int(os.environ.get('DIR_TAIL_THIN_MAX_TILES', '0'))
    force_waves = int(os.environ.get('DIR_TAIL_WAVES', '0'))

    def __init__(self, c3, c1n):
        self.c3, self.c1n = c3, c1n
        self.cout, self.cin, self.kh, self.kw, self.stride = c3.cout, c3.cin, 1, 1, 1
        self.variant = {}
        self.stream = {n: pack_tail_stream(c3.w.reshape(c3.cout, c3.cin), c1n.w.reshape(c1n.cout, c1n.cin), n, dtype=c3.dtype) for n in (8, 4)}
        self.params = {n: _capi.BneckTailParams(_capi.ptr(self.stream[n]), _capi.ptr(c3.scale), _capi.ptr(c3.shift), _capi.ptr(c1n.scale),
                                                _capi.ptr(c1n.shift), c3.cin, c1n.cout, n, _dt(c3.dtype)) for n in (8, 4)}

    @staticmethod
    def applies(c3, c1n, dtype):
        return (dtype in HALF and c3.kh == 1 and c3.stride == 1 and c3.scale is not None and c3.cout == 4 * c3.cin
                and c1n.kh == 1 and c1n.stride == 1 and c1n.cin == c3.cout and c1n.scale is not None and c1n.pre_scale is None
                and (c3.cin, c1n.cout) in BneckTailOp.GEOMETRIES)

    def __call__(self, y2, x, out=None, y1n=None):
        B, H, W, P = y2.shape
        M = B * H * W
        if getattr(_TLS, 'capture_fused', None) is not None:
            _TLS.capture_fused.append((self, (y2, x), {}))
        if out is None:
            out = torch.empty(B, H, W, self.c3.cout, device=y2.device, dtype=y2.dtype)
        if y1n is None:
            y1n = torch.empty(B, H, W, self.c1n.cout, device=y2.device, dtype=y2.dtype)
        if _capi.PROFILE is not None:
            c4, n2 = self.c3.cout, self.c1n.cout
            _capi.annotate(family='conv', flops=2.0 * M * (P * c4 + c4 * n2), op=self, dtype='bf16',
                           shape='M=%d tail 1x1(%d->%d)+res+1x1(->%d)' % (M, P, c4, n2),
                           bytes=(M * (P + 2 * c4 + n2) + c4 * P + n2 * c4) * 2)
        waves = self.force_waves or (4 if M // 64 <= self.THIN_MAX_TILES else 8)
        _capi.check(_capi.lib().dir_bottleneck_tail_forward(C.byref(self.params[waves]), _capi.ptr(y2), _capi.ptr(x), _capi.ptr(out), _capi.ptr(y1n),
                                                            M, _capi.stream_ptr()), 'dir_bottleneck_tail_forward')
        return out, y1n


def stem_conv_op(w, scale, shift, dtype):
    wp = torch.zeros(64, 64, 4, 1, device=w.device, dtype=F32)
    for r in range(4):
        for dy in range(2):
            ky = 2 * r + dy - 1
            if not 0 <= ky <= 6:
                continue
            for j in range(4):
                for dx in range(2):
                    kx = 2 * j + dx - 1
                    if 0 <= kx <= 6:
                        c0 = j * 16 + (dy * 2 + dx) * 4
                        wp[:, c0:c0 + 3, r, 0] = w[:, :, ky, kx]
    op = ConvOp(wp, dtype, stride=1, pad=0, scale=scale, shift=shift, relu=True)
    op.ho = op.wo = 128
    op.in_cs_override = 16
    op.alg_k = 147
    return op


class BackboneOp(object):
    fold_downsample = os.environ.get('DIR_FOLD_DOWNSAMPLE', '1') != '0'
    fused_stem = os.environ.get('DIR_FUSED_STEM', '1') != '0'
    bneck_chain = os.environ.get('DIR_BNECK_CHAIN', '1') != '0'
    bneck_tail = os.environ.get('DIR_BNECK_TAIL', '1') != '0'

    def __init__(self, sd, p, dtype, device):
        dt = self.dtype = dtype
        self.device = device
        w = sd[p + '.conv1.weight']
        wk = torch.zeros(64, 7, 8, 4, device=w.device, dtype=F32)
        wk[:, :, :7, :3] = w.permute(0, 2, 3, 1)
        self.stem_w = wk.to(dtype if dtype in HALF else torch.bfloat16).contiguous().to(device)
        s_, h_ = bn_fold(sd, p + '.bn1')
        self.stem_scale, self.stem_shift = s_.float().contiguous().to(device), h_.float().contiguous().to(device)
        self.stem = stem_conv_op(sd[p + '.conv1.weight'], s_, h_, dt)
        self.layers = []
        for li, n in enumerate((3, 4, 6, 3), start=1):
            blocks = []
            for b in range(n):
                q = '%s.layer%d.%d' % (p, li, b)
                stride = 2 if (b == 0 and li > 1) else 1
                s1, h1 = bn_fold(sd, q + '.bn1')
                s2, h2 = bn_fold(sd, q + '.bn2')
                s3, h3 = bn_fold(sd, q + '.bn3')
                blk = dict(c1=ConvOp(sd[q + '.conv1.weight'], dt, scale=s1, shift=h1, relu=True),
                           c2=ConvOp(sd[q + '.conv2.weight'], dt, stride=stride, pad=1, scale=s2, shift=h2, relu=True),
                           c3=ConvOp(sd[q + '.conv3.weight'], dt, scale=s3, shift=h3, relu=True), ds=None)
                if (q + '.downsample.0.weight') in sd:
                    sd_, hd_ = bn_fold(sd, q + '.downsample.1')
                    if self.fold_downsample:
                        blk['dual'] = DualConvOp(sd[q + '.conv3.weight'], s3, h3, sd[q + '.downsample.0.weight'], sd_, hd_, stride, dt)
                    else:
                        blk['ds'] = ConvOp(sd[q + '.downsample.0.weight'], dt, stride=stride, scale=sd_, shift=hd_)
                blk['c1'].link_split(blk['c2'])
                if 'dual' not in blk and blk['ds'] is None:
                    blk['c2'].link_split(blk['c3'])
                blocks.append(blk)
            self.layers.append(blocks)
        if self.bneck_chain:
            l1 = self.layers[0]
            for i, blk in enumerate(l1):
                nxt = l1[i + 1]['c1'] if i + 1 < len(l1) else self.layers[1][0]['c1']
                if 'dual' in blk:
                    if BneckChainOp.applies(blk['c2'], None, nxt, dt, dual=blk['dual']):
                        blk['chain'] = BneckChainOp(blk['c2'], None, nxt, dual=blk['dual'])
                elif blk['ds'] is None and BneckChainOp.applies(blk['c2'], blk['c3'], nxt, dt):
                    blk['chain'] = BneckChainOp(blk['c2'], blk['c3'], nxt)

        if self.bneck_tail:
            for li in (1, 2):
                blocks = self.layers[li]
                for i, blk in enumerate(blocks):
                    if 'dual' in blk or blk['ds'] is not None or 'chain' in blk:
                        continue
                    nxt = blocks[i + 1]['c1'] if i + 1 < len(blocks) else self.layers[li + 1][0]['c1']
                    if BneckTailOp.applies(blk['c3'], nxt, dt):
                        blk['tail'] = BneckTailOp(blk['c3'], nxt)

    def __call__(self, img):
        L, dt, dev = _capi.lib(), self.dtype, self.device
        B = img.shape[0]
        if self.fused_stem and dt in HALF:
            x = torch.empty(B, 64, 64, 64, device=dev, dtype=dt)
            u8 = img.dtype == torch.uint8
            _ann('stem', 2.0 * B * 128 * 128 * 64 * 147, img.numel() * img.element_size() + x.numel() * 2 + self.stem_w.numel() * 2,
                 'B=%d 7x7/2 conv + bn + relu + maxpool' % B)
            nb = self.subbatch
            last2 = self.layers[1][-1]
            if nb and nb < B and B % nb == 0 and 'tail' in last2 and not getattr(_TLS, 'capture_fused', None) and not getattr(_TLS, 'no_out_split', False):
                c2 = torch.empty(B, 32, 32, 512, device=dev, dtype=dt)
                y1n = torch.empty(B, 32, 32, last2['tail'].c1n.cout, device=dev, dtype=dt)
                _TLS.parent_batch = B
                try:
                    for b0 in range(0, B, nb):
                        isub = img[b0:b0 + nb]
                        xs = x[b0:b0 + nb]
                        _ann('stem', 2.0 * nb * 128 * 128 * 64 * 147, isub.numel() * isub.element_size() + xs.numel() * 2 + self.stem_w.numel() * 2,
                             'B=%d 7x7/2 conv + bn + relu + maxpool' % nb)
                        _capi.check(L.dir_stem_pool_forward_dt(_capi.ptr(isub), 2 if u8 else 0, _dt(dt), IMAGENET_MEAN, IMAGENET_STD, _capi.ptr(self.stem_w),
                                                            _capi.ptr(self.stem_scale), _capi.ptr(self.stem_shift), _capi.ptr(xs), nb, 256, 256,
                                                            _capi.stream_ptr()), 'dir_stem_pool_forward')
                        self._layers(xs, upto=2, out_last=(c2[b0:b0 + nb], y1n[b0:b0 + nb]))
                finally:
                    _TLS.parent_batch = None
                return [None, c2] + self._layers(c2, start=2, y1=y1n)
            _capi.check(L.dir_stem_pool_forward_dt(_capi.ptr(img), 2 if u8 else 0, _dt(dt), IMAGENET_MEAN, IMAGENET_STD, _capi.ptr(self.stem_w),
                                                _capi.ptr(self.stem_scale), _capi.ptr(self.stem_shift), _capi.ptr(x), B, 256, 256,
                                                _capi.stream_ptr()), 'dir_stem_pool_forward')
            return self._layers(x)
        Hs, Ws = 131, 132
        xp = torch.empty(B, Hs, Ws, 16, device=dev, dtype=dt)
        _ann('stem', 0, img.numel() * img.element_size() + xp.numel() * xp.element_size(), 'B=%d space-to-depth staging' % B)
        if img.dtype == torch.uint8:
            _capi.check(L.dir_stem_prep_s2d_u8(_capi.ptr(img), _capi.ptr(xp), IMAGENET_MEAN, IMAGENET_STD, B, 256, 256, Hs, Ws,
                                               _dt(dt), _capi.stream_ptr()), 'dir_stem_prep_s2d_u8')
        else:
            _capi.check(L.dir_stem_prep_s2d(_capi.ptr(img), _capi.ptr(xp), B, 256, 256, Hs, Ws, _dt(dt), _capi.stream_ptr()),
                        'dir_stem_prep_s2d')
        s1 = self.stem(xp)
        x = torch.empty(B, 64, 64, 64, device=dev, dtype=dt)
        _ann('stem', 0, (s1.numel() + x.numel()) * x.element_size(), 'B=%d maxpool 3x3/2' % B)
        _capi.check(L.dir_maxpool3x3s2(_capi.ptr(s1), _capi.ptr(x), B, 128, 128, 64, _dt(dt), _capi.stream_ptr()),
                    'dir_maxpool3x3s2')
        return self._layers(x)

    decimate_c1 = os.environ.get('DIR_DECIMATE_C1', '1') != '0'
    subbatch = int(os.environ.get('DIR_SUBBATCH', '0'))

    def _layers(self, x, start=0, upto=4, y1=None, out_last=None):
        feats = []
        x_dec = False
        for li in range(start, upto):
            blocks = self.layers[li]
            for bi, blk in enumerate(blocks):
                if 'chain' in blk:
                    dec = (self.decimate_c1 and li == 0 and bi == len(blocks) - 1 and blk['chain'].c1n is not None and 'dual' in self.layers[1][0]
                           and self.layers[1][0]['dual'].stride2 == 2 and 'chain' not in self.layers[1][0] and not getattr(_TLS, 'no_out_split', False))
                    x, y1 = blk['chain'](y1 if y1 is not None else blk['c1'](x), x, decimate=dec)
                    x_dec = dec
                    continue
                if 'tail' in blk and (x.shape[0] * x.shape[1] * x.shape[2]) % 64 == 0:
                    if out_last is not None and li == upto - 1 and bi == len(blocks) - 1:
                        x, y1 = blk['tail'](blk['c2'](y1 if y1 is not None else blk['c1'](x)), x, out=out_last[0], y1n=out_last[1])
                        continue
                    x, y1 = blk['tail'](blk['c2'](y1 if y1 is not None else blk['c1'](x)), x)
                elif 'dual' in blk:
                    x, y1 = blk['dual'](blk['c2'](y1 if y1 is not None else blk['c1'](x)), x, x_decimated=x_dec), None
                    x_dec = False
                else:
                    idn = blk['ds'](x) if blk['ds'] is not None else x
                    x, y1 = blk['c3'](blk['c2'](y1 if y1 is not None else blk['c1'](x)), residual=idn), None
            feats.append(None if x_dec else x)
        return feats


def backbone_standalone(module, x, compute_dtype=torch.float32):
    _capi.require_cuda(x)
    if module.training:
        raise NotImplementedError('dir_amd implements the inference path (eval-mode BatchNorm); call .eval()')
    sd = {'b.' + k: v.detach() for k, v in module.state_dict().items()}
    op = BackboneOp(sd, 'b', compute_dtype, x.device)
    op.decimate_c1 = False
    with torch.cuda.device(x.device):
        feats = op(_capi.f32c(x.detach()))
    return [f.permute(0, 3, 1, 2).float() for f in feats]


def _padc(c):
    return (c + 63) // 64 * 64


def _pad_conv_bn(sd, conv_key, bn_prefix, dtype, stride=1, relu=True):
    w = sd[conv_key]
    co, ci, kh, kw = w.shape
    wp = torch.zeros(_padc(co), _padc(ci), kh, kw, device=w.device, dtype=torch.float32)
    wp[:co, :ci] = w.float()
    sc, sh = bn_fold(sd, bn_prefix)
    scp, shp = torch.zeros(_padc(co), device=w.device), torch.zeros(_padc(co), device=w.device)
    scp[:co], shp[:co] = sc.to(w.device), sh.to(w.device)
    op = ConvOp(wp, dtype, stride=stride, pad=kh // 2, scale=scp, shift=shp, relu=relu)
    op.alg_scale = (co * ci) / float(_padc(co) * _padc(ci))
    return op


class HRNetOp(object):
    WIDTHS = (48, 96, 192, 384)
    MODULES = ((2, 1), (3, 4), (4, 3))

    def __init__(self, sd, p, dtype, device):
        dt = self.dtype = dtype
        self.device = device
        w = sd[p + '.conv1.weight'].float()
        wp = torch.zeros(64, 64, 3, 1, device=w.device)
        for j in range(3):
            wp[:, 4 * j:4 * j + 3, :, 0] = w[:, :, :, j]
        s1, h1 = bn_fold(sd, p + '.bn1')
        self.conv1 = ConvOp(wp, dt, stride=2, pad=0, scale=s1, shift=h1, relu=True)
        self.conv1.ho = self.conv1.wo = 0
        self.conv1.in_cs_override = 4
        self.conv1.alg_k = 27
        s2, h2 = bn_fold(sd, p + '.bn2')
        self.conv2 = ConvOp(sd[p + '.conv2.weight'], dt, stride=2, pad=1, scale=s2, shift=h2, relu=True)
        self.layer1 = []
        for b in range(4):
            q = '%s.layer1.%d' % (p, b)
            sa, ha = bn_fold(sd, q + '.bn1'); sb, hb = bn_fold(sd, q + '.bn2'); sc, hc = bn_fold(sd, q + '.bn3')
            blk = dict(c1=ConvOp(sd[q + '.conv1.weight'], dt, scale=sa, shift=ha, relu=True),
                       c2=ConvOp(sd[q + '.conv2.weight'], dt, pad=1, scale=sb, shift=hb, relu=True))
            if (q + '.downsample.0.weight') in sd:
                sd_, hd_ = bn_fold(sd, q + '.downsample.1')
                blk['dual'] = DualConvOp(sd[q + '.conv3.weight'], sc, hc, sd[q + '.downsample.0.weight'], sd_, hd_, 1, dt)
            else:
                blk['c3'] = ConvOp(sd[q + '.conv3.weight'], dt, scale=sc, shift=hc, relu=True)
            blk['c1'].link_split(blk['c2'])
            if 'c3' in blk:
                blk['c2'].link_split(blk['c3'])
            self.layer1.append(blk)
        self.trans = {(1, 0): _pad_conv_bn(sd, p + '.transition1.0.0.weight', p + '.transition1.0.1', dt),
                      (1, 1): _pad_conv_bn(sd, p + '.transition1.1.0.weight', p + '.transition1.1.1', dt, stride=2),
                      (2, 2): _pad_conv_bn(sd, p + '.transition2.0.weight', p + '.transition2.1', dt, stride=2),
                      (3, 3): _pad_conv_bn(sd, p + '.transition3.0.weight', p + '.transition3.1', dt, stride=2)}
        self.stages = []
        for st, n in self.MODULES:
            mods = []
            for m in range(n):
                q = '%s.stage%d.%d' % (p, st, m)
                branches = [[(_pad_conv_bn(sd, '%s.branches.%d.%d.conv1.weight' % (q, b, k), '%s.branches.%d.%d.bn1' % (q, b, k), dt),
                              _pad_conv_bn(sd, '%s.branches.%d.%d.conv2.weight' % (q, b, k), '%s.branches.%d.%d.bn2' % (q, b, k), dt))
                             for k in range(4)] for b in range(st)]
                for br in branches:
                    for c1, c2 in br:
                        c1.link_split(c2)
                fuse = {}
                for i in range(st):
                    for j in range(st):
                        f = '%s.fuse_layers.%d.%d' % (q, i, j)
                        if j > i:
                            fuse[(i, j)] = [_pad_conv_bn(sd, f + '.0.weight', f + '.1', dt, relu=False)]
                        elif j < i:
                            fuse[(i, j)] = [_pad_conv_bn(sd, '%s.%d.0.weight' % (f, t), '%s.%d.1' % (f, t), dt, stride=2, relu=(t < i - j - 1))
                                            for t in range(i - j)]
                mods.append((branches, fuse))
            self.stages.append(mods)
        self.incre = [_pad_conv_bn(sd, '%s.incre.%d.0.weight' % (p, b), '%s.incre.%d.1' % (p, b), dt) for b in range(4)]

    def _fuse_sum(self, base, srcs, factors, relu, out=None):
        import ctypes as C
        B, H, W, Cc = base.shape
        out = torch.empty_like(base) if out is None else out
        n = len(srcs)
        _ann('hr_fuse', 0, (2 * base.numel() + sum(t.numel() for t in srcs)) * base.element_size(), 'sum %dx%dx%d (%d terms)' % (H, W, Cc, n + 1))
        ps = (C.c_void_p * max(n, 1))(*[t.data_ptr() for t in srcs])
        fs = (C.c_int * max(n, 1))(*factors)
        _capi.check(_capi.lib().dir_fuse_sum(_capi.ptr(out), _capi.ptr(base), ps, fs, n, B, H, W, Cc, 1 if relu else 0, _dt(self.dtype), _capi.stream_ptr()), 'dir_fuse_sum')
        return out

    def _module(self, xs, mod):
        branches, fuse = mod
        nb = len(xs)
        ys = []
        for b in range(nb):
            y = xs[b]
            for c1, c2 in branches[b]:
                y = c2(c1(y), residual=y)
            ys.append(y)
        outs = []
        for i in range(nb):
            acc = None
            for j in range(i):
                t = ys[j]
                chain = fuse[(i, j)]
                for op in chain[:-1]:
                    t = op(t)
                acc = chain[-1](t) if acc is None else chain[-1](t, residual=acc)
            ups = [fuse[(i, j)][0](ys[j]) for j in range(i + 1, nb)]
            facs = [2 ** (j - i) for j in range(i + 1, nb)]
            if acc is None:
                outs.append(self._fuse_sum(ys[i], ups, facs, True))
            else:
                outs.append(self._fuse_sum(acc, [ys[i]] + ups, [1] + facs, True, out=acc))
        return outs

    def __call__(self, img):
        L, dt, dev = _capi.lib(), self.dtype, self.device
        assert img.dtype == F32, 'the HRNet path takes the normalised float image (NCHW)'
        B, _, H, W = img.shape
        Hp, Wp = H + 2, W + 2
        xp = torch.empty(B, Hp, Wp, 4, device=dev, dtype=dt)
        _ann('stem', 0, img.numel() * 4 + xp.numel() * xp.element_size(), 'B=%d NHWC4 staging' % B)
        _capi.check(L.dir_stem_prep(_capi.ptr(img), _capi.ptr(xp), B, H, W, Hp, Wp, 1, _dt(dt), _capi.stream_ptr()), 'dir_stem_prep')
        self.conv1.ho, self.conv1.wo = H // 2, W // 2
        x = self.conv2(self.conv1(xp))
        for blk in self.layer1:
            y = blk['c2'](blk['c1'](x))
            x = blk['dual'](y, x) if 'dual' in blk else blk['c3'](y, residual=x)
        xs = [self.trans[(1, 0)](x), self.trans[(1, 1)](x)]
        for si, (st, n) in enumerate(self.MODULES):
            if st > 2:
                xs = xs + [self.trans[(st - 1, st - 1)](xs[-1])]
            for mod in self.stages[si]:
                xs = self._module(xs, mod)
        return [self.incre[b](xs[b]) for b in range(4)]


def hrnet_standalone(module, x, compute_dtype=torch.float32):
    _capi.require_cuda(x)
    sd = {'b.' + k: v.detach() for k, v in module.state_dict().items()}
    op = HRNetOp(sd, 'b', compute_dtype, x.device)
    with torch.cuda.device(x.device):
        feats = op(_capi.f32c(x.detach()))
    return [f.permute(0, 3, 1, 2).float() for f in feats]


class ResidualOp(object):

    def __init__(self, sd, p, dtype):
        w = lambda k: sd['%s.%s.conv.weight' % (p, k)]
        b = lambda k: sd['%s.%s.conv.bias' % (p, k)]
        self.need_skip = w('skip_layer').shape[0] != w('skip_layer').shape[1]
        self.skip = ConvOp(w('skip_layer'), dtype, shift=b('skip_layer'))
        s2, h2 = bn_fold(sd, p + '.bn2', b('conv1'))
        self.c1 = ConvOp(w('conv1'), dtype, scale=s2, shift=h2, relu=True, pre=bn_fold(sd, p + '.bn1'), pre_relu=True)
        s3, h3 = bn_fold(sd, p + '.bn3', b('conv2'))
        self.c2 = ConvOp(w('conv2'), dtype, pad=1, scale=s3, shift=h3, relu=True)
        self.c3 = ConvOp(w('conv3'), dtype, shift=b('conv3'))
        self.dual = None
        if self.need_skip and self.fold_skip:
            one = torch.ones(w('conv3').shape[0], device=w('conv3').device)
            self.dual = DualConvOp(w('conv3'), one, b('conv3'), w('skip_layer'), one, b('skip_layer'), 1, dtype, relu=False)
        self.c1.link_split(self.c2)
        if self.dual is None:
            self.c2.link_split(self.c3)
        self.chain = None
        self.cout, self.cin, self.kh, self.kw, self.stride = self.c3.cout, self.c1.cin, 3, 3, 1
        self.variant = {}
        if (self.res_chain and dtype in HALF and self.dual is not None and self.dual.w_stream is not None
                and _capi.lib().dir_residual_chain_supported(_dt(dtype), self.c1.cin, self.c1.cout, self.dual.cout, 1, 32, 32, self.c1.cin, 0, self.dual.cout, 0)):
            self.chain_w = (pack_as_weights(self.c1.w, 1), pack_as_weights(self.c2.w, 1),
                            pack_as_weights(self.dual.w.reshape(self.dual.cout, 1, 1, self.dual.cin + self.dual.cin2), 1))
            self.chain = _capi.ResChainParams(*([_capi.ptr(t) for t in self.chain_w] + [_capi.ptr(t) for t in (
                self.c1.pre_scale, self.c1.pre_shift, self.c1.scale, self.c1.shift, self.c2.scale, self.c2.shift, self.dual.shift)]
                + [self.c1.cin, self.c1.cout, self.dual.cout, _dt(dtype)]))

    fold_skip = os.environ.get('DIR_FOLD_SKIP', '1') != '0'
    res_chain = os.environ.get('DIR_RES_CHAIN', '1') != '0'

    def _chain_call(self, x, out=None, out_coff=0):
        B, H, W, cbuf = x.shape
        cs = out.shape[3] if out is not None else self.cout
        if x.dtype != self.c1.dtype or (out is not None and out.dtype != x.dtype) or not x.is_contiguous() or (out is not None and not out.is_contiguous()):
            return None
        if not _capi.lib().dir_residual_chain_supported(_dt(x.dtype), self.cin, self.c1.cout, self.cout, B, H, W, cbuf, 0, cs, out_coff):
            return None
        if out is None:
            out = torch.empty(B, H, W, self.cout, device=x.device, dtype=x.dtype)
        if getattr(_TLS, 'capture', None) is not None:
            _TLS.capture.append((self, (x,), dict(out=out, out_coff=out_coff)))
        if _capi.PROFILE is not None:
            m, mid = B * H * W, self.c1.cout
            _capi.annotate(family='conv', flops=2.0 * m * (mid * self.cin + mid * 9 * mid + self.cout * (mid + self.cin)), op=self, dtype='bf16',
                           shape='M=%d residual 1x1(%d->%d)+3x3+1x1(->%d)+skip' % (m, self.cin, mid, self.cout),
                           bytes=(m * (self.cin + self.cout) + self.c1.w.numel() + self.c2.w.numel() + self.dual.w.numel()) * 2)
        _capi.check(_capi.lib().dir_residual_chain_forward(C.byref(self.chain), _capi.ptr(x), _capi.ptr(out), B, H, W, cbuf, 0, cs, out_coff,
                                                           _capi.stream_ptr()), 'dir_residual_chain_forward')
        return out

    def __call__(self, x, out=None, out_coff=0):
        if self.chain is not None and self.res_chain:
            y = self._chain_call(x, out, out_coff)
            if y is not None:
                return y
        if self.dual is not None:
            return self.dual(self.c2(self.c1(x)), x, out=out, out_coff=out_coff)
        res = self.skip(x) if self.need_skip else x
        return self.c3(self.c2(self.c1(x)), out=out, out_coff=out_coff, residual=res)


class ConvChainOp(object):

    head_chain = os.environ.get('DIR_HEAD_CHAIN', '1') != '0'

    def __init__(self, c3, c1):
        self.c3, self.c1 = c3, c1
        self.cout, self.cin, self.kh, self.kw, self.stride = c3.cout, c3.cin, c3.kh, c3.kw, c3.stride
        self.variant = c3.variant
        self.w = None
        f32_out = c1.out_dtype == F32
        if (c3.dtype in HALF and c1.dtype == c3.dtype and c3.arith is None and c3.pre_scale is None and c1.pre_scale is None and (c1.flags & ~CONV_RELU) == 0
                and (c1.kh, c1.kw, c1.stride, c1.pad, c1.cin) == (1, 1, 1, 0, c3.cout) and (f32_out or c1.out_dtype == c3.dtype)
                and _capi.lib().dir_conv2d_as_chain_supported(self._desc(1, 32, 32, c3.cin), c1.cout, _dt(c1.out_dtype))):
            w1 = c3._w_as.setdefault(2, pack_as_weights(c3.w, 2))
            if f32_out:
                wp = torch.zeros(128, 1, 1, c1.cin, device=c1.w.device, dtype=c1.w.dtype)
                wp[:c1.cout] = c1.w
                self.w = (w1, pack_as_weights(wp, 1))
            else:
                self.w = (w1, pack_as_weights(c1.w, 2))

    def _desc(self, B, H, W, cbuf):
        c3 = self.c3
        return ConvDesc(B, H, W, c3.cin, cbuf, 0, c3.cout, c3.cout, 0, 0, 0, 3, 3, c3.stride, c3.pad, _dt(c3.dtype), _dt(c3.dtype), c3.flags & CONV_RELU, 0, 0, 1.0)

    def __call__(self, x, out=None):
        c3, c1 = self.c3, self.c1
        B, H, W, cbuf = x.shape
        if (self.w is None or not self.head_chain or x.dtype != c3.dtype or not x.is_contiguous() or getattr(_TLS, 'calibrating', False)
                or (out is not None and (out.dtype != c1.out_dtype or out.shape != (B, H, W, c1.cout) or not out.is_contiguous()))):
            return c1(c3(x), out=out)
        d = self._desc(B, H, W, cbuf)
        if not _capi.lib().dir_conv2d_as_chain_supported(d, c1.cout, _dt(c1.out_dtype)):
            return c1(c3(x), out=out)
        if out is None:
            out = torch.empty(B, H, W, c1.cout, device=x.device, dtype=c1.out_dtype)
        if getattr(_TLS, 'capture', None) is not None:
            _TLS.capture.append((self, (x,), dict(out=out)))
        if _capi.PROFILE is not None:
            m = B * H * W
            _capi.annotate(family='conv', flops=2.0 * m * (c3.cout * c3.alg_k + c1.cout * c1.alg_k), op=c3, covers=(c1,), dtype='bf16',
                           shape='M=%d N=%d K=%d k3x3 s1 + 1x1 -> %d' % (m, c3.cout, c3.alg_k, c1.cout),
                           bytes=m * c3.cin * x.element_size() + (c3.w.numel() + c1.w.numel()) * c3.w.element_size() + m * c1.cout * out.element_size())
        _capi.check(_capi.lib().dir_conv2d_as_chain_forward(d, _capi.ptr(x), _capi.ptr(self.w[0]), _capi.ptr(c3.scale), _capi.ptr(c3.shift),
                                                            _capi.ptr(self.w[1]), _capi.ptr(c1.scale), _capi.ptr(c1.shift), c1.cout, 1 if c1.flags & CONV_RELU else 0,
                                                            _capi.ptr(out), c1.cout, 0, _dt(c1.out_dtype), _capi.stream_ptr()), 'dir_conv2d_as_chain_forward')
        return out


class StageOp(object):

    def __init__(self, sd, p, S, distance, dtype, root_joint, keep):
        self.S, self.distance, self.dtype = S, float(distance), dtype
        self.img2joint = (_capi.TokenMlp * 2)(pack_token_mlp(sd, p + '.img2joint_left.filters', keep),
                                              pack_token_mlp(sd, p + '.img2joint_right.filters', keep))
        self.pos_emb = (_capi.TokenMlp * 2)(pack_token_mlp(sd, p + '.pos_emb_left', keep),
                                            pack_token_mlp(sd, p + '.pos_emb_right', keep))
        self.gpos = pack_token_mlp(sd, p + '.global_pos_emb', keep)
        self.gcn = (pack_pgcn(sd, p + '.gcn_left', keep, weight_dtype=_tok_wdt(dtype)), pack_pgcn(sd, p + '.gcn_right', keep, weight_dtype=_tok_wdt(dtype)))
        self.ste = pack_ste(sd, p + '.interaction', keep, weight_dtype=_tok_wdt(dtype))
        R = _capi.RegressParams()
        t = dict(wt=torch.cat([sd[p + '.regressor.mano_left.weight'].float().t(),
                               sd[p + '.regressor.mano_right.weight'].float().t()], 1).contiguous(),
                 bl=sd[p + '.regressor.mano_left.bias'].float().contiguous(),
                 br=sd[p + '.regressor.mano_right.bias'].float().contiguous(),
                 wo=sd[p + '.regressor.offset.weight'].float().contiguous(),
                 bo=sd[p + '.regressor.offset.bias'].float().contiguous())
        keep.append(t)
        R.mano_wt, R.mano_b[0], R.mano_b[1] = (t[k].data_ptr() for k in ('wt', 'bl', 'br'))
        R.off_w, R.off_b = t['wo'].data_ptr(), t['bo'].data_ptr()
        R.emb = pack_token_mlp(sd, p + '.proj_feat_emb', keep)
        self.reg = R
        self.mano = (pack_mano(sd, p + '.regressor.mano_layer_left', 'left', root_joint, keep),
                     pack_mano(sd, p + '.regressor.mano_layer_right', 'right', root_joint, keep))
        s, h = bn_fold(sd, p + '.fusion.1', sd[p + '.fusion.0.bias'])
        self.fusion0 = ConvOp(sd[p + '.fusion.0.weight'], dtype, pad=1, scale=s, shift=h, relu=True)
        self.bone_fusion = None
        if dtype in HALF or _packing_arith() is not None:
            exact = dtype == torch.float32
            w = sd[p + '.fusion.0.weight'].detach()
            w = w.float() if exact else w.to(dtype).float()
            s_f, h_f = bn_fold(sd, p + '.fusion.1', sd[p + '.fusion.0.bias'])
            t = dict(w_g=w.reshape(256, 40, 64, 9).permute(3, 1, 2, 0).contiguous(), scale=s_f.to(w.device), shift=h_f.to(w.device))
            keep.append(t)
            self.bone_fusion = _capi.BoneFusionParams(t['w_g'].data_ptr(), t['scale'].data_ptr(), t['shift'].data_ptr(), 1 if exact else 2 if dtype == torch.float16 else 0)
        self.fusion3 = ConvOp(sd[p + '.fusion.3.weight'], dtype, shift=sd[p + '.fusion.3.bias'])


def run_mano_pair(tables_lr, para_l, para_r, B, flags=None, mesh_uv=False):
    dev = para_l.device
    out = [[torch.empty(B, 778, 3, device=dev, dtype=F32), torch.empty(B, 21, 3, device=dev, dtype=F32),
            torch.empty(B, 21, 2, device=dev, dtype=F32)] for _ in range(2)]
    if mesh_uv:
        for o in out:
            o.append(torch.empty(B, 778, 2, device=dev, dtype=F32))
    P2 = C.c_void_p * 2
    base = (para_l.data_ptr(), para_r.data_ptr())
    tabs = (_capi.ManoTables * 2)(tables_lr[0], tables_lr[1])
    _ann('mano', 2.0 * B * 1.2e6, 2 * B * (64 + 778 * 3 + 21 * 3 + 21 * 2) * 4 + 2 * (145 * 2336 + 2334 + 778 * 16 + 16 * 33 + 45 * 46) * 4,
         'B=%d x 2 hands (rot6d + PCA + blend shapes + LBS + projection)' % B)
    rc = _capi.lib().dir_mano_forward_pair(
        tabs, P2(base[0], base[1]), 64, P2(base[0] + 51 * 4, base[1] + 51 * 4), 64, P2(base[0] + 61 * 4, base[1] + 61 * 4), 64,
        P2(out[0][0].data_ptr(), out[1][0].data_ptr()), P2(out[0][1].data_ptr(), out[1][1].data_ptr()),
        P2(out[0][2].data_ptr(), out[1][2].data_ptr()), P2(out[0][3].data_ptr(), out[1][3].data_ptr()) if mesh_uv else None,
        None if flags is None else P2(flags[0].data_ptr(), flags[1].data_ptr()), B, _capi.stream_ptr())
    _capi.check(rc, 'dir_mano_forward_pair')
    return out


class DirEngine(object):
    def __init__(self, state_dict, dtype=torch.bfloat16, root_joint=0, device='cuda', sparse_fusion=True, arith=None):
        assert dtype in (torch.bfloat16, torch.float16, torch.float32)
        assert arith in (None, 'f16x3', 'f16') and (arith is None or dtype == torch.float32)
        self.arith = arith
        self.tuned_batches = set()
        self.sparse_fusion = sparse_fusion
        _capi.lib()
        self.dtype, self.device = dtype, torch.device(device)
        sd = {k: v.detach().to(self.device) for k, v in state_dict.items()}
        self.keep = []
        self._pgcn_ws = {}
        _TLS.arith = arith
        try:
            self._pack(sd, root_joint)
        finally:
            _TLS.arith = None

    def _pack(self, sd, root_joint):
        dt, keep = self.dtype, self.keep
        hr = 'backbone.stage4.0.fuse_layers.0.1.0.weight' in sd
        self.bb = HRNetOp(sd, 'backbone', dt, self.device) if hr else BackboneOp(sd, 'backbone', dt, self.device)
        p = 'init_regressor'
        H = _capi.InitHeadParams()
        t = {}
        aw, asc, ash = [], [], []
        for i, side in enumerate(('left', 'right')):
            a = '%s.attention_%s' % (p, side)
            s, h = bn_fold(sd, a + '.1', sd[a + '.0.bias'])
            aw.append(sd[a + '.0.weight']); asc.append(s); ash.append(h)
            t['aw%d' % i] = sd[a + '.3.weight'].float().reshape(-1).contiguous()
            H.attn_w[i] = t['aw%d' % i].data_ptr()
            H.attn_b[i] = float(sd[a + '.3.bias'].float().item())
            t['mb%d' % i] = sd['%s.mano_%s.bias' % (p, side)].float().contiguous()
            H.mano_b[i] = t['mb%d' % i].data_ptr()
        self.attn = ConvOp(torch.cat(aw, 0), dt, pad=1, scale=torch.cat(asc), shift=torch.cat(ash), relu=True)
        t['mwt'] = torch.cat([sd[p + '.mano_left.weight'].float().t(), sd[p + '.mano_right.weight'].float().t()],
                             1).contiguous()
        H.mano_wt = t['mwt'].data_ptr()
        t['ow'], t['ob'] = sd[p + '.offset.weight'].float().contiguous(), sd[p + '.offset.bias'].float().contiguous()
        H.off_w, H.off_b = t['ow'].data_ptr(), t['ob'].data_ptr()
        keep.append(t)
        self.init_head = H
        self.init_mano = (pack_mano(sd, p + '.mano_layer_left', 'left', root_joint, keep),
                          pack_mano(sd, p + '.mano_layer_right', 'right', root_joint, keep))
        d = 'decoder'
        self.res = {k: ResidualOp(sd, '%s.%s' % (d, k), dt) for k in (
            'skip_layer4', 'fusion_layer4', 'enhance_layer4', 'skip_layer3', 'fusion_layer3', 'enhance_layer3')}
        self.stage4 = StageOp(sd, d + '.projecter_4', 16, 1, dt, root_joint, keep)
        self.stage3 = StageOp(sd, d + '.projecter_3', 32, 2, dt, root_joint, keep)
        self.stages_x, self.res_x = [], []
        while ('%s.projecter_x.%d.fusion.0.weight' % (d, len(self.stages_x))) in sd:
            i = len(self.stages_x)
            self.stages_x.append(StageOp(sd, '%s.projecter_x.%d' % (d, i), 32, 2, dt, root_joint, keep))
            self.res_x.append(ResidualOp(sd, '%s.enhance_layer_x.%d' % (d, i), dt))
        s, h = bn_fold(sd, d + '.conv_final.1')
        self.final0 = ConvOp(sd[d + '.conv_final.0.weight'], dt, pad=1, scale=s, shift=h, relu=True)
        self.final3 = ConvOp(sd[d + '.conv_final.3.weight'], dt, shift=sd[d + '.conv_final.3.bias'])
        w0, s0, h0, w3, b3 = [], [], [], torch.zeros(6, 256, 1, 1, device=self.device), []
        for i, k in enumerate(('seg', 'dense')):
            s, h = bn_fold(sd, '%s.%s.1' % (d, k), sd['%s.%s.0.bias' % (d, k)])
            w0.append(sd['%s.%s.0.weight' % (d, k)]); s0.append(s); h0.append(h)
            w3[3 * i:3 * i + 3, 128 * i:128 * i + 128] = sd['%s.%s.3.weight' % (d, k)]
            b3.append(sd['%s.%s.3.bias' % (d, k)])
        self.heads0 = ConvOp(torch.cat(w0, 0), dt, pad=1, scale=torch.cat(s0), shift=torch.cat(h0), relu=True)
        self.heads3 = ConvOp(w3, dt, shift=torch.cat(b3), out_dtype=F32)
        self.final0.link_split(self.final3)
        self.final3.link_split(self.heads0)
        self.heads0.link_split(self.heads3)
        self.final_chain = ConvChainOp(self.final0, self.final3)
        self.heads_chain = ConvChainOp(self.heads0, self.heads3)

    def init_regressor(self, c4):
        L, dev = _capi.lib(), self.device
        B = c4.shape[0]
        hh = self.attn(c4)
        ch = hh.shape[3] // 2
        esz = hh.element_size()
        para_l = torch.empty(B, 64, device=dev, dtype=F32)
        para_r = torch.empty(B, 64, device=dev, dtype=F32)
        off = torch.empty(B, 3, device=dev, dtype=F32)
        npx = c4.shape[1] * c4.shape[2]
        _ann('init_head', 2.0 * B * (2 * npx * ch + 2 * npx * c4.shape[3] + c4.shape[3] * 128),
             (c4.numel() + hh.numel()) * esz + (c4.shape[3] * 128 + 2 * ch + 131 * 3) * 4 + B * 131 * 4, 'B=%d attention pooling + 3 Linears' % B)
        _capi.check(L.dir_init_head_forward(self.init_head, _capi.ptr(c4), C.c_void_p(hh.data_ptr()),
                                            C.c_void_p(hh.data_ptr() + ch * esz), 2 * ch, _capi.ptr(para_l),
                                            _capi.ptr(para_r), _capi.ptr(off), B, c4.shape[1] * c4.shape[2], c4.shape[3],
                                            ch, _dt(self.dtype), _capi.stream_ptr()), 'dir_init_head_forward')
        return self.mano_outputs(self.init_mano, para_l, para_r, off, self._flags[0] if self._flags is not None else None)

    def mano_outputs(self, tables, para_l, para_r, off, flags=None):
        B = para_l.shape[0]
        (vl, jl, uvl), (vr, jr, uvr) = run_mano_pair(tables, para_l, para_r, B, flags)
        return {'pd_offset': off, 'pd_mano_para_left': para_l, 'pd_mano_para_right': para_r,
                'pd_proj_left': para_l[:, 61:64], 'pd_proj_right': para_r[:, 61:64],
                'pd_mesh_xyz_left': vl, 'pd_mesh_xyz_right': vr, 'pd_joint_xyz_left': jl, 'pd_joint_xyz_right': jr,
                'pd_joint_uv_left': uvl, 'pd_joint_uv_right': uvr, 'pd_rel_joint': None}

    def stage(self, st, feat_buf, feat_cs, prev, img_out, img_coff, want_vis):
        L, dev = _capi.lib(), self.device
        B, S = feat_buf.shape[0], st.S
        sp = _capi.stream_ptr()
        x0 = torch.empty(2, B, 21, 128, device=dev, dtype=F32)
        gp = torch.empty(2, B, 21, 128, device=dev, dtype=F32)
        es = feat_buf.element_size()
        mlp = lambda cin: cin * 128 + 128 * 128
        _ann('grid_tokens', 2.0 * 2 * B * 21 * (mlp(256) + 2 * mlp(3)), 2 * B * 21 * 4 * 256 * es + (2 * mlp(256) + 3 * mlp(3)) * 4 + 4 * B * 21 * 128 * 4,
             'B=%d S=%d bilinear gather + 3 token MLPs, 2 hands' % (B, S))
        _capi.check(L.dir_grid_tokens_forward(
            _capi.ptr(feat_buf), _dt(self.dtype), S, 256, feat_cs, 0, _capi.ptr(prev['pd_joint_uv_left']),
            _capi.ptr(prev['pd_joint_uv_right']), _capi.ptr(prev['pd_joint_xyz_left']),
            _capi.ptr(prev['pd_joint_xyz_right']), _capi.ptr(prev['pd_offset']), st.img2joint, st.pos_emb,
            C.byref(st.gpos), _capi.ptr(x0), _capi.ptr(gp), B, sp), 'dir_grid_tokens_forward')
        tok = torch.empty(B, 42, 128, device=dev, dtype=F32)
        scratch = torch.empty(4, B, 21, 256, device=dev, dtype=F32)
        wes = 2 if self.dtype in HALF else 4
        _ann('pgcn', 2.0 * 4 * 2 * B * 21 * 2 * 128 * 128, 4 * 2 * (2 * 21 * 128 * 128 * wes + 2 * B * 21 * 128 * 4),
             'B=%d 4 layers x 2 hands (per-node W0/W1 %s + neighbour mix + BN + ReLU)' % (B, 'bf16' if wes == 2 else 'f32'))
        if self.pgcn_fused:
            _capi.check(L.dir_pgcn_stack_forward_fused(st.gcn[0], st.gcn[1], 4, _capi.ptr(x0), _capi.ptr(gp), _capi.ptr(tok), _capi.ptr(scratch),
                                                       _capi.ptr(self._pgcn_sync()), 0, B, sp), 'dir_pgcn_stack_forward_fused')
        else:
            _capi.check(L.dir_pgcn_stack_forward_pair(st.gcn[0], st.gcn[1], 4, _capi.ptr(x0), _capi.ptr(gp), _capi.ptr(tok),
                                                      _capi.ptr(scratch), B, sp), 'dir_pgcn_stack_forward_pair')
        y = torch.empty(B, 42, 64, device=dev, dtype=F32)
        blk = 42 * 128 * 384 + 4 * 2 * 42 * 42 * 32 + 42 * 128 * 128 + 2 * 42 * 128 * 256
        _ann('ste', 2.0 * B * (3 * blk + 42 * 128 * 64), B * 42 * (128 + 64) * 4 + (3 * (128 * 384 + 128 * 128 + 2 * 128 * 256) + 128 * 64) * wes,
             'B=%d 42 tokens x 128, 3 blocks + head' % B)
        _capi.check(L.dir_ste_forward(C.byref(st.ste), _capi.ptr(tok), None, _capi.ptr(y), B, sp), 'dir_ste_forward')
        para_l = torch.empty(B, 64, device=dev, dtype=F32)
        para_r = torch.empty(B, 64, device=dev, dtype=F32)
        off = torch.empty(B, 3, device=dev, dtype=F32)
        emb = torch.empty(B, 42, 64, device=dev, dtype=F32)
        _ann('regress', 2.0 * B * (2 * 1408 * 64 + 2691 * 3 + 42 * 2 * 64 * 64), (2 * 1408 * 64 + 2691 * 3 + 2 * 64 * 64) * 4 + B * (42 * 64 * 2 + 2 * 64 * 2 + 6) * 4,
             'B=%d 2 x Linear 1408->64 + Linear 2691->3 + proj_feat_emb' % B)
        _capi.check(L.dir_regress_forward(C.byref(st.reg), _capi.ptr(y), _capi.ptr(prev['pd_mano_para_left']),
                                          _capi.ptr(prev['pd_mano_para_right']), _capi.ptr(prev['pd_offset']),
                                          _capi.ptr(para_l), _capi.ptr(para_r), _capi.ptr(off), _capi.ptr(emb), B, sp),
                    'dir_regress_forward')
        factorised = st.bone_fusion is not None and self.factorised_fusion
        if factorised:
            scratch = torch.empty(L.dir_bone_fusion_scratch_bytes(B), device=dev, dtype=torch.uint8)
            main, side = torch.cuda.current_stream(), self._side_stream()
            side.wait_stream(main)
            with torch.cuda.stream(side):
                _ann('bone_fusion', 2.0 * B * 9 * 80 * 64 * 256, 9 * 40 * 64 * 256 * 4 + B * 42 * 64 * 4 + B * 9 * 80 * 256 * (4 if self.dtype == F32 else 2),
                     'B=%d G = f_end . W (9 taps x 80 bone ends x 256)' % B)
                _capi.check(L.dir_bone_fusion_prepare(st.bone_fusion, _capi.ptr(emb), _capi.ptr(scratch), B, _capi.stream_ptr()),
                            'dir_bone_fusion_prepare')
        res = self.mano_outputs(st.mano, para_l, para_r, off, self._flags[self._stage_index(st)] if self._flags is not None else None)
        vis = torch.empty(B, 1280, S, S, device=dev, dtype=F32) if want_vis else None
        if factorised:
            main.wait_stream(side)
            if self.arith is not None and getattr(_TLS, 'calibrating', False):
                amax = float(scratch.view(F32)[:B * 9 * 40 * 256 * 2].abs().max())
                st.bone_fusion.g_scale = 2.0 ** (10 - math.frexp(amax)[1]) if amax > 0 and math.isfinite(amax) else 1.0
            fused = torch.empty(B, S, S, 256, device=dev, dtype=self.dtype)
            _ann('bone_fusion', 2.0 * B * S * S * 256 * 720, (B * 9 * 80 * 256 + B * S * S * 256) * (4 if self.dtype == F32 else 2) + B * 42 * 2 * 4,
                 'B=%d S=%d factorised bone_proj + 3x3 fusion conv (K=720)' % (B, S))
            _capi.check(L.dir_bone_fusion_forward(st.bone_fusion, _capi.ptr(res['pd_joint_uv_left']),
                                                  _capi.ptr(res['pd_joint_uv_right']), _capi.ptr(scratch),
                                                  _capi.ptr(fused), B, S, st.distance, 256, 0, 1, sp), 'dir_bone_fusion_forward')
            if want_vis:
                _ann('proj_feat', 30.0 * B * S * S * 40, B * 1280 * S * S * 4 + B * 42 * 64 * 4, 'B=%d S=%d proj_feat output (fp32 NCHW)' % (B, S))
                _capi.check(L.dir_bone_proj_forward(_capi.ptr(res['pd_joint_uv_left']), _capi.ptr(res['pd_joint_uv_right']),
                                                    _capi.ptr(emb), None, _capi.ptr(vis), None, B, S, st.distance,
                                                    _dt(self.dtype), sp), 'dir_bone_proj_forward')
            st.fusion3(fused, out=img_out, out_coff=img_coff)
        else:
            bone = torch.empty(B, S, S, 2560, device=dev, dtype=self.dtype)
            bbox = torch.empty(B, 40, 4, device=dev, dtype=torch.int32)
            _ann('bone_proj', 30.0 * B * S * S * 40, bone.numel() * bone.element_size() + (B * 1280 * S * S * 4 if want_vis else 0) + B * 42 * 64 * 4,
                 'B=%d S=%d materialised bone map' % (B, S))
            _capi.check(L.dir_bone_proj_forward(_capi.ptr(res['pd_joint_uv_left']), _capi.ptr(res['pd_joint_uv_right']),
                                                _capi.ptr(emb), _capi.ptr(bone), _capi.ptr(vis), _capi.ptr(bbox), B, S,
                                                st.distance, _dt(self.dtype), sp), 'dir_bone_proj_forward')
            st.fusion3(st.fusion0(bone, bbox=bbox if self.sparse_fusion else None), out=img_out, out_coff=img_coff)
        res['joint_feat'] = emb
        res['vis_img_feat'] = vis
        return res

    pgcn_fused = os.environ.get('DIR_PGCN_FUSED', '0') == '1'

    def _pgcn_sync(self):
        key = torch.cuda.current_stream(self.device).cuda_stream
        ws = self._pgcn_ws.get(key)
        if ws is None:
            ws = torch.zeros(int(_capi.lib().dir_pgcn_fused_sync_bytes()) // 4, dtype=torch.int32, device=self.device)
            self._pgcn_ws[key] = ws
        return ws

    def pgcn_sync_error(self):
        return any(int(ws[-4].item()) != 0 for ws in self._pgcn_ws.values())

    def _stage_index(self, st):
        return 1 if st is self.stage4 else 2 if st is self.stage3 else 3 + self.stages_x.index(st)

    def upsample_into(self, x, out, coff):
        B, H, W, Cc = x.shape
        _ann('upsample', 0, 5 * x.numel() * x.element_size(), 'B=%d %dx%dx%d -> 2x' % (B, H, W, Cc))
        _capi.check(_capi.lib().dir_upsample2x_bilinear(_capi.ptr(x), _capi.ptr(out), B, H, W, Cc, out.shape[3], coff,
                                                        _dt(self.dtype), _capi.stream_ptr()), 'dir_upsample2x_bilinear')

    factorised_fusion = os.environ.get('DIR_FACTORISED_FUSION', '1') != '0'
    overlap = os.environ.get('DIR_OVERLAP', '0') == '1'

    def _side_stream(self):
        if not self.overlap:
            return torch.cuda.current_stream()
        if getattr(self, '_side', None) is None:
            self._side = torch.cuda.Stream(device=self.device)
        return self._side

    CONV_VARIANTS = (0, 1, 2, 3, 4, 17, 18, 20, 8, 9, 10, 11, 12, 13, 14, 15, STREAM_VARIANT, STREAM64_VARIANT, STREAM32_VARIANT, 25, 26, 27, 28)

    def _profiled_forwards(self, img, n):
        _capi.PROFILE = []
        try:
            for _ in range(n):
                self.forward(img)
            torch.cuda.synchronize()
            return [r for r in _capi.PROFILE if r.get('op') is not None]
        finally:
            _capi.PROFILE = None

    PIPE_MARGIN = float(os.environ.get('DIR_TUNE_PIPE_MARGIN', '0.03'))
    TUNE_EXCLUDE = tuple(int(v) for v in os.environ.get('DIR_TUNE_EXCLUDE', '').split(',') if v)
    STREAM_MARGIN = float(os.environ.get('DIR_TUNE_STREAM_MARGIN', '0.03'))

    def autotune(self, img, reps=2):
        B = img.shape[0]
        saved_overlap, saved_profile = self.overlap, _capi.PROFILE
        self.overlap = False
        best, covers = {}, {}
        try:
            for v in self.CONV_VARIANTS:
                if v in self.TUNE_EXCLUDE:
                    continue
                _TLS.variant = v
                self._profiled_forwards(img, 1)
                acc = {}
                for rec in self._profiled_forwards(img, reps):
                    acc.setdefault(rec['op'], []).append(rec['e0'].elapsed_time(rec['e1']))
                    covers[rec['op']] = rec.get('covers', ())
                for op, ts in acc.items():
                    t = min(ts)
                    margin = self.PIPE_MARGIN if v in (8, 9, 10, 11, 12, 13, 14, 15) else self.STREAM_MARGIN if v in STREAM_VARIANTS else 0.03
                    if op not in best or t < best[op][0] * (1.0 - margin):
                        best[op] = (t, v)
        finally:
            _TLS.variant = None
            _capi.PROFILE = saved_profile
            self.overlap = saved_overlap
        for op, (t, v) in best.items():
            op.variant[B] = v
        self.tuned_batches.add(B)
        self._tuned_order = getattr(self, '_tuned_order', {})
        self._tuned_order[B] = self._layer_ops(dict(op=op, covers=covers.get(op, ())) for op in best)
        for op in self._tuned_order[B]:
            op.variant.setdefault(B, 0)
        return {op: op.variant[B] for op in self._tuned_order[B]}

    @staticmethod
    def _layer_ops(recs):
        ops = []
        for rec in recs:
            for op in (rec['op'],) + tuple(rec.get('covers', ())):
                if op not in ops:
                    ops.append(op)
        return ops

    def autotune_energy(self, img, seconds=None, slack=2.6, idle_w=None, log=None, max_calls=None, min_saving=0.0, near=1.12):
        import time as _time
        from . import power
        B = img.shape[0]
        if B not in getattr(self, '_tuned_order', {}):
            self.autotune(img)
        counter = power.energy_joules() is not None
        if not counter and power.smi_sample() is None:
            raise RuntimeError('autotune_energy: neither the amdsmi energy counter nor rocm-smi gives a reading on this machine')
        if seconds is None:
            seconds = 0.2 if counter else 0.8
        saved_overlap, self.overlap = self.overlap, False
        torch.cuda.synchronize(self.device)
        if idle_w is None:
            idle_w = power.IDLE_W
        rows = []
        try:
            _TLS.capture = []
            self.forward(img)
            torch.cuda.synchronize(self.device)
            calls, _TLS.capture = _TLS.capture, None
            seen = set()
            for op, args, kw in (calls if max_calls is None else calls[:max_calls]):
                if id(op) in seen:
                    continue
                seen.add(id(op))
                times = {}
                for v in self.CONV_VARIANTS:
                    if v in self.TUNE_EXCLUDE:
                        continue
                    _TLS.variant = v
                    for _ in range(3):
                        op(*args, **kw)
                    e0, e1 = torch.cuda.Event(enable_timing=True), torch.cuda.Event(enable_timing=True)
                    e0.record()
                    for _ in range(10):
                        op(*args, **kw)
                    e1.record()
                    torch.cuda.synchronize(self.device)
                    times[v] = e0.elapsed_time(e1) / 10 * 1e3
                tb = min(times.values())
                row = {}
                for v, us in times.items():
                    if us > slack * tb:
                        continue
                    _TLS.variant = v
                    burst = max(10, min(100, int(0.02 / (us * 1e-6))))
                    if counter:
                        for _ in range(burst):
                            op(*args, **kw)
                        torch.cuda.synchronize(self.device)
                        e0 = power.energy_joules()
                    else:
                        smp = power.Sampler(skip=0.6 * seconds, period=0.03).start()
                    t0, n = _time.perf_counter(), 0
                    while _time.perf_counter() - t0 < seconds:
                        for _ in range(burst):
                            op(*args, **kw)
                        torch.cuda.synchronize(self.device)
                        n += burst
                    dt = _time.perf_counter() - t0
                    if counter:
                        e1 = power.energy_joules()
                        w = (e1[0] - e0[0]) / dt if e0 and e1 else float('nan')
                    else:
                        w = power.median(smp.stop(), 'w')
                    if w == w:
                        row[v] = (dt / n * 1e6, w)
                _TLS.variant = None
                if not row:
                    continue
                joules = lambda v: row[v][0] * max(row[v][1] - idle_w, 1.0)
                fastest = min(row, key=lambda v: row[v][0])
                base = min((v for v in row if row[v][0] <= near * row[fastest][0]), key=joules)
                best = min(row, key=joules)
                if joules(best) > (1.0 - min_saving) * joules(base):
                    best = base
                op.variant[B] = best
                rows.append(dict(cout=op.cout, cin=getattr(op, 'cin', 0), kh=getattr(op, 'kh', 1), stride=getattr(op, 'stride', 1), chosen=best,
                                 us=round(row[best][0], 1), w=round(row[best][1]), fastest=fastest, fastest_us=round(row[fastest][0], 1),
                                 fastest_w=round(row[fastest][1])))
                if log is not None:
                    log(rows[-1])
                for c in ((op.c1,) if isinstance(op, ConvChainOp) else ()):
                    c.variant.setdefault(B, 0)
        finally:
            _TLS.capture, _TLS.variant = None, None
            self.overlap = saved_overlap
        return {'idle_w': idle_w, 'layers': rows, 'instrument': 'amdsmi energy accumulator, %.2f s windows' % seconds if counter else 'rocm-smi power, last 40 %% of %.2f s windows' % seconds}

    TUNING_DIR = os.path.join(os.path.dirname(os.path.abspath(__file__)), 'tuning')

    def load_tuning_table(self, img, name):
        path = os.path.join(self.TUNING_DIR, name + '.json')
        if not os.path.exists(path):
            return None
        with open(path) as f:
            t = json.load(f)
        if t.get('batch') != img.shape[0] or any(int(r[5]) not in self.CONV_VARIANTS for r in t['table']):
            return None
        try:
            self.import_tuning(img, t['table'])
        except ValueError:
            return None
        return t.get('meta', {})

    def export_tuning(self, B):
        return [[op.cout, op.cin, op.kh, op.kw, op.stride, op.variant.get(B, 0)] for op in self._tuned_order[B]]

    def import_tuning(self, img, table):
        B = img.shape[0]
        saved_overlap, saved_profile, self.overlap = self.overlap, _capi.PROFILE, False
        try:
            ops = self._layer_ops(self._profiled_forwards(img, 1))
        finally:
            _capi.PROFILE, self.overlap = saved_profile, saved_overlap
        if len(ops) != len(table) or any([op.cout, op.cin, op.kh, op.kw, op.stride] != row[:5] for op, row in zip(ops, table)):
            raise ValueError('tuning table does not match this engine')
        for op, row in zip(ops, table):
            op.variant[B] = int(row[5])
        self.tuned_batches.add(B)
        self._tuned_order = getattr(self, '_tuned_order', {})
        self._tuned_order[B] = ops

    pending_tuning = None

    def export_all_tuning(self):
        return {B: self.export_tuning(B) for B in getattr(self, '_tuned_order', {})}

    def tune_for(self, img):
        B = img.shape[0]
        if B in self.tuned_batches:
            return
        if self.pending_tuning and B in self.pending_tuning:
            try:
                self.import_tuning(img, self.pending_tuning[B])
                return
            except ValueError:
                pass
        order = getattr(self, '_tuned_order', {})
        if order:
            self.copy_tuning(min(order, key=lambda b: abs(b - B)), B)
        else:
            self.autotune(img)

    def copy_tuning(self, B_from, B_to):
        for op in self._tuned_order.get(B_from, []):
            op.variant[B_to] = op.variant.get(B_from, 0)
        self._tuned_order[B_to] = self._tuned_order[B_from]
        self.tuned_batches.add(B_to)

    calibrated = False

    def calibrate(self, img):
        if self.arith is None:
            return
        _TLS.calibrating = True
        try:
            self.forward(img)
            torch.cuda.synchronize(self.device)
        finally:
            _TLS.calibrating = False
        self.calibrated = True

    _flags = None

    def forward(self, img, want_proj_feat=True, taps=None, reflection_flags=None):
        _capi.require_cuda(img)
        self._flags = reflection_flags
        _TLS.no_out_split = taps is not None
        try:
            return self._forward(img, want_proj_feat, taps)
        finally:
            self._flags = None
            _TLS.no_out_split = False

    def _forward(self, img, want_proj_feat, taps):
        if img.dtype == torch.uint8:
            assert img.is_contiguous() and img.shape[1:] == (256, 256, 3)
        else:
            assert img.dtype == F32 and img.is_contiguous() and img.shape[1:] == (3, 256, 256)
        dt, dev = self.dtype, self.device
        B = img.shape[0]
        feats = self.bb(img)
        c1, c2, c3, c4 = feats
        cat4 = torch.empty(B, 16, 16, 2304, device=dev, dtype=dt)
        cat3 = torch.empty(B, 32, 32, 512, device=dev, dtype=dt)
        main = torch.cuda.current_stream()
        side = self._side_stream()
        ev_tok = torch.cuda.Event()
        side.wait_stream(main)
        with torch.cuda.stream(side):
            self.res['skip_layer4'](c3, out=cat4, out_coff=2048)
            ev_s4 = torch.cuda.Event()
            ev_s4.record()
        init = self.init_regressor(c4)
        self.upsample_into(c4, cat4, 0)
        main.wait_event(ev_s4)
        enh4_in = torch.empty(B, 16, 16, 512, device=dev, dtype=dt)
        self.res['fusion_layer4'](cat4, out=enh4_in, out_coff=0)
        ev_tok.record()
        with torch.cuda.stream(side):
            side.wait_event(ev_tok)
            self.res['skip_layer3'](c2, out=cat3, out_coff=256)
        r4 = self.stage(self.stage4, enh4_in, 512, init, enh4_in, 256, False)
        e4 = self.res['enhance_layer4'](enh4_in)
        self.upsample_into(e4, cat3, 0)
        main.wait_stream(side)
        enh3_in = torch.empty(B, 32, 32, 512, device=dev, dtype=dt)
        self.res['fusion_layer3'](cat3, out=enh3_in, out_coff=0)
        nx = len(self.stages_x)
        r3 = self.stage(self.stage3, enh3_in, 512, r4, enh3_in, 256, want_proj_feat and nx == 0)
        extra, buf, prev = [], enh3_in, r3
        for i in range(nx):
            nxt = torch.empty(B, 32, 32, 512, device=dev, dtype=dt)
            (self.res['enhance_layer3'] if i == 0 else self.res_x[i - 1])(buf, out=nxt, out_coff=0)
            prev = self.stage(self.stages_x[i], nxt, 512, prev, nxt, 256, want_proj_feat and i == nx - 1)
            extra.append(prev)
            buf = nxt
        e3 = (self.res['enhance_layer3'] if nx == 0 else self.res_x[nx - 1])(buf)
        feat = self.final_chain(e3)
        sd6 = self.heads_chain(feat)
        seg, dense = sd6[..., :3], sd6[..., 3:]
        if taps is not None:
            taps.update(c1=c1, c2=c2, c3=c3, c4=c4, fusion4=enh4_in[..., :256], proj4=enh4_in[..., 256:], enh4=e4,
                        fusion3=enh3_in[..., :256], proj3=enh3_in[..., 256:], enh3=e3, final=feat,
                        skip4=cat4[..., 2048:])
        outs = []
        for o in [init, r4, r3] + extra:
            outs.append({k: o[k] for k in ('pd_joint_uv_left', 'pd_joint_uv_right', 'pd_mesh_xyz_left',
                                           'pd_mesh_xyz_right', 'pd_joint_xyz_left', 'pd_joint_xyz_right',
                                           'pd_proj_left', 'pd_proj_right', 'pd_offset', 'pd_rel_joint')})
        outs.append({'dense': dense.permute(0, 3, 1, 2), 'seg': seg.permute(0, 3, 1, 2),
                     'proj_feat': (extra[-1] if extra else r3)['vis_img_feat']})
        return outs


class ForwardPipeline(object):

    def __init__(self, eng, imgs, want_proj_feat=True, streams=None):
        assert len(imgs) >= 1 and (streams is None or len(streams) == len(imgs))
        self.eng, self.imgs = eng, list(imgs)
        self.streams, self.graphs, self.outs, self.done = [], [], [], []
        cur = torch.cuda.current_stream()
        for i, img in enumerate(self.imgs):
            s = streams[i] if streams is not None else torch.cuda.Stream(device=eng.device)
            s.wait_stream(cur)
            with torch.cuda.stream(s):
                eng.forward(img, want_proj_feat)
                s.synchronize()
                g = torch.cuda.CUDAGraph()
                with torch.cuda.graph(g, stream=s):
                    o = eng.forward(img, want_proj_feat)
            self.streams.append(s); self.graphs.append(g); self.outs.append(o)
            self.done.append(torch.cuda.Event())
        torch.cuda.synchronize(eng.device)

    def __len__(self):
        return len(self.graphs)

    def refill(self, slot, batch):
        with torch.cuda.stream(self.streams[slot]):
            self.imgs[slot].copy_(batch, non_blocking=True)

    def launch(self, slot):
        s = self.streams[slot]
        with torch.cuda.stream(s):
            self.graphs[slot].replay()
            self.done[slot].record(s)

    def wait(self, slot):
        self.done[slot].synchronize()
        return self.outs[slot]
```

### include/dir_hip.h

```cpp
#ifndef DIR_HIP_H
#define DIR_HIP_H

#include <stddef.h>
#include <stdint.h>

#ifdef __cplusplus
extern "C" {
#endif

#define DIR_OK 0
#define DIR_E_INVALID (-1)
#define DIR_E_LAUNCH (-2)
#define DIR_E_NODEVICE (-3)

#define DIR_ABI_VERSION 48

int dir_abi_version(void);
const char* dir_last_error(void);
int dir_device_info(char* arch_host, int arch_len, int* num_cu_host);
void dir_launch_log_reset(void);
int dir_launch_log_get(char* buf_host, int len);
void dir_launch_log_note(const char* name, long long times);
long long dir_probe_launch(int mode, void* buf, long long bytes, int iters, void* stream);

typedef struct dir_mano_tables {
    const float* shapedirs_t;
    const float* posedirs_t;
    const float* v_template;
    const float* j_template;
    const float* j_shapedirs;
    const float* weights;
    const float* hands_mean;
    const float* comps;
    int32_t side;
    int32_t center_idx;
    int32_t root_palm;
} dir_mano_tables;

int dir_mano_forward(const dir_mano_tables* tables_host, const float* pose, int pose_stride,
                     const float* betas, int betas_stride, const float* cam, int cam_stride,
                     float* verts, float* joints, float* joint_uv, float* mesh_uv, int32_t* flags_out,
                     int B, void* stream);

int dir_mano_forward_pair(const dir_mano_tables* tables_lr_host, const float* const* pose_lr_host, int pose_stride,
                          const float* const* betas_lr_host, int betas_stride, const float* const* cam_lr_host,
                          int cam_stride, float* const* verts_lr_host, float* const* joints_lr_host,
                          float* const* joint_uv_lr_host, float* const* mesh_uv_lr_host, int32_t* const* flags_lr_host, int B,
                          void* stream);

int dir_mano_backward_pair(const dir_mano_tables* tables_lr_host, const float* const* pose_lr_host, int pose_stride,
                           const float* const* betas_lr_host, int betas_stride, const float* const* cam_lr_host, int cam_stride,
                           const float* const* g_verts_lr_host, const float* const* g_joints_lr_host,
                           const float* const* g_joint_uv_lr_host, const float* const* g_mesh_uv_lr_host,
                           float* const* g_pose_lr_host, int g_pose_stride, float* const* g_betas_lr_host, int g_betas_stride,
                           float* const* g_cam_lr_host, int g_cam_stride, int hands, int B, void* stream);

int dir_regress_backward(const float* w_left, const float* w_right, const float* w_offset, const float* tok,
                         const float* prev_para_left, const float* prev_para_right, const float* prev_offset,
                         const float* g_para_left, const float* g_para_right, const float* g_offset,
                         float* gw_left, float* gb_left, float* gw_right, float* gb_right, float* gw_offset, float* gb_offset,
                         float* g_tok, int B, void* stream);

typedef struct dir_gemm_desc {
    int32_t M, N, K, lda, ldb, ldc, trans_a, trans_b, accumulate, batch;
    int64_t stride_a, stride_b, stride_c;
} dir_gemm_desc;
int dir_gemm_f32(const dir_gemm_desc* desc_host, const float* A, const float* B, const float* bias, float* C, void* stream);
typedef struct dir_gemm_groups {
    int32_t ny, nx, reduce, reserved;
    int64_t a_y, a_x, b_y, b_x, c_y, c_x;
} dir_gemm_groups;
int dir_gemm_f32_grouped(const dir_gemm_desc* desc_host, const dir_gemm_groups* groups_host, const float* A, const float* B, const float* bias,
                         float* C, void* stream);
long long dir_gemm_f32_splitk_workspace_bytes(const dir_gemm_desc* desc_host);
int dir_gemm_f32_splitk(const dir_gemm_desc* desc_host, const float* A, const float* B, const float* bias, float* C, float* workspace,
                        long long workspace_bytes, void* stream);
long long dir_colsum_workspace_bytes(int R, int N);
int dir_colsum_f32(const float* x, float* out, int R, int N, int ld, int accumulate, float* workspace, long long workspace_bytes, void* stream);
int dir_layernorm_forward(const float* x, const float* w, const float* b, float* y, float* mean, float* rstd, int R, int C, float eps, void* stream);
int dir_layernorm_backward(const float* gy, const float* x, const float* w, const float* mean, const float* rstd, float* gx, float* gw,
                           float* gb, int R, int C, int accumulate_x, int accumulate_wb, void* stream);
int dir_gelu_forward(const float* x, float* y, long long n, void* stream);
int dir_gelu_backward(const float* gy, const float* x, float* gx, long long n, void* stream);
int dir_attention_forward(const float* qkv, float* probs, float* out, int B, int T, int H, float scale, void* stream);
int dir_attention_backward(const float* qkv, const float* probs, const float* gout, float* gqkv, int B, int T, int H, float scale, void* stream);
long long dir_bn_train_workspace_bytes(int R, int C);
int dir_bn_one_launch_status(void);
int dir_bn_one_launch_enable(int on);
int dir_bn_train_forward(const float* x, const float* w, const float* b, float* y, float* save_mean, float* save_rstd, float* running_mean,
                         float* running_var, int R, int C, int ld, float eps, float momentum, int relu, const float* residual,
                         float* workspace, long long workspace_bytes, void* stream);
int dir_bn_train_backward(const float* gy, const float* x, const float* w, const float* b, const float* save_mean, const float* save_rstd, float* gx,
                          float* gw, float* gb, int R, int C, int ld, int relu, float* workspace, long long workspace_bytes, void* stream);
int dir_bn_train_backward_from_partials(const float* gy, const float* x, const float* w, const float* b, const float* save_mean, const float* save_rstd,
                                        const float* p1, const float* p2, int chunks, float* gx, float* gw, float* gb, int R, int C, int ld, int relu,
                                        float* workspace, long long workspace_bytes, void* stream);
int dir_bn_train_stats(const float* x, const float* w, const float* b, float* save_mean, float* save_rstd, float* pre_scale, float* pre_shift,
                       float* running_mean, float* running_var, int R, int C, int ld, float eps, float momentum, float* workspace,
                       long long workspace_bytes, void* stream);
int dir_bn_train_stats_from_partials(float* p1, float* p2, int chunk_rows, int cap_rows, const float* w, const float* b, float* save_mean, float* save_rstd,
                                     float* pre_scale, float* pre_shift, float* running_mean, float* running_var, int R, int C, float eps, float momentum,
                                     void* stream);
int dir_bn_train_apply(const float* x, const float* w, const float* b, const float* save_mean, const float* save_rstd, float* y, int R, int C, int ld,
                       int relu, const float* residual, void* stream);
int dir_bn_train_forward_from_partials(const float* x, float* p1, float* p2, int chunk_rows, int cap_rows, const float* w, const float* b, float* y,
                                       float* save_mean, float* save_rstd, float* running_mean, float* running_var, int R, int C, int ld, float eps,
                                       float momentum, int relu, const float* residual, void* stream);
long long dir_bn_frozen_workspace_bytes(int R, int C);
int dir_bn_frozen_forward(const float* x, const float* w, const float* b, float* y, float* save_mean, float* save_rstd, const float* running_mean,
                          const float* running_var, int R, int C, int ld, float eps, int relu, const float* residual, void* stream);
int dir_bn_frozen_backward(const float* gy, const float* x, const float* w, const float* b, const float* save_mean, const float* save_rstd, float* gx,
                           float* gw, float* gb, int R, int C, int ld, int relu, float* workspace, long long workspace_bytes, void* stream);
long long dir_bn_sync_workspace_bytes(int R, int C);
int dir_bn_sync_local_stats(const float* x, float* part, int R, int C, int ld, float* workspace, long long workspace_bytes, void* stream);
int dir_bn_sync_combine(const float* parts, int world, int C, float* mean, float* var, float* running_mean, float* running_var, float momentum, void* stream);
int dir_bn_sync_backward_sums(const float* gy, const float* x, const float* w, const float* b, const float* save_mean, const float* save_rstd, float* sums,
                              int R, int C, int ld, int relu, float* workspace, long long workspace_bytes, void* stream);
int dir_bn_sync_backward_apply(const float* gy, const float* x, const float* w, const float* b, const float* save_mean, const float* save_rstd,
                               const float* sums_pooled, float* gx, int R, float rows_pooled, int C, int ld, int relu, void* stream);
int dir_relu_forward(const float* x, float* y, long long n, void* stream);
int dir_relu_backward(const float* gy, const float* y, float* gx, long long n, void* stream);
int dir_upsample_nearest_add_f32(const float* src, float* dst, int B, int h, int w, int C, int factor, void* stream);
int dir_upsample_nearest_backward_f32(const float* gy, float* gx, int B, int h, int w, int C, int factor, void* stream);
int dir_grid_rows_forward(const float* feat_nhwc, const float* uv, float* rows, int B, int S, int C, void* stream);
int dir_grid_rows_backward(const float* const* g_rows_h_host, const float* const* uv_h_host, int hands, float* g_feat_nhwc, int B, int S, int C,
                           int zero_first, void* stream);
int dir_maxpool3x3s2_backward(const float* x, const float* gy, float* gx, int B, int H, int W, int C, void* stream);
int dir_upsample2x_bilinear_backward(const float* gy, float* gx, int B, int H, int W, int C, int gy_cstride, int gy_coff, void* stream);
int dir_attn_pool_forward(const float* feat, const float* logit, float* attn, float* pooled, float* mean, int B, int HW, int C, void* stream);
int dir_attn_pool_backward(const float* feat, const float* attn, const float* pooled, const float* g_pooled, const float* g_mean, float* g_feat,
                           float* g_logit, int B, int HW, int C, int accumulate, void* stream);
long long dir_bone_proj_backward_scratch_bytes(int B, int hands);
int dir_bone_proj_backward(const float* const* uv_lr_host, const float* emb, const float* g_img, int img_cstride, int img_coff, float distance,
                           float* g_emb, float* const* g_uv_lr_host, float* scratch, int B, int S, int hands, void* stream);
int dir_axpy_f32(float* dst, const float* src, long long n, float alpha, void* stream);
int dir_axpy_multi_f32(float* const* dst_host, const float* const* src_host, const long long* n_host, int count, float alpha, void* stream);
int dir_stage_positions(const float* xyz_left, const float* xyz_right, const float* offset, float* pos_left, float* pos_right,
                        float* gpos_left, float* gpos_right, int B, void* stream);
int dir_pgcn_adjacency_forward(const float* e1, float* A, void* stream);
int dir_pgcn_adjacency_backward(const float* e1, const float* gz, const float* h1, float* scratch40, float* g_e1, int B, void* stream);

#define DIR_DT_F32 0
#define DIR_DT_BF16 1
#define DIR_DT_U8 2
#define DIR_DT_F16X3 3
#define DIR_DT_F16X1 4
#define DIR_DT_F16X3P 5
#define DIR_DT_F16X1P 6
#define DIR_DT_F16 7
#define DIR_CONV_RELU 1
#define DIR_CONV_PRE_RELU 2
#define DIR_CONV_VARIANT(v) (((v) & 0xff) << 8)

typedef struct dir_conv_desc {
    int32_t B, H, W;
    int32_t Cin, in_cstride, in_coff;
    int32_t Cout, out_cstride, out_coff;
    int32_t res_cstride, res_coff;
    int32_t kh, kw, stride, pad;
    int32_t in_dtype, out_dtype;
    int32_t flags;
    int32_t Ho, Wo;
    float in_scale;
    float out_split_scale;
} dir_conv_desc;

int dir_conv2d_forward(const dir_conv_desc* desc_host, const void* x, const void* w, const float* scale,
                       const float* shift, const float* pre_scale, const float* pre_shift,
                       const void* residual, void* y, void* stream);
int dir_conv2d_forward_masked(const dir_conv_desc* desc, const void* x, const void* w, const float* scale, const float* shift, const float* pre_scale,
                              const float* pre_shift, const void* residual, const float* mask, void* y, void* stream);
typedef struct dir_conv_bn_bwd {
    const float *z, *mean, *rstd, *w, *b;
    int32_t relu;
    float *p1, *p2;
} dir_conv_bn_bwd;
int dir_conv2d_forward_ex(const dir_conv_desc* desc, const void* x, const void* w, const float* scale, const float* shift, const float* pre_scale,
                          const float* pre_shift, const void* residual, const float* mask, void* y, const dir_conv_bn_bwd* bn, int* chunk_rows, void* stream);
int dir_conv2d_forward_stats(const dir_conv_desc* desc, const void* x, const void* w, const float* scale, const float* shift, const float* pre_scale,
                             const float* pre_shift, void* y, float* p1, float* p2, int* chunk_rows, void* stream);

int dir_split_f16_forward(const float* x, void* y, long long pixels, int C, int in_cstride, int in_coff, const float* pre_scale,
                          const float* pre_shift, int pre_relu, float in_scale, int hi_only, void* stream);

int dir_pack_f16x3_weights(const float* w, void* packed, float* scale_out, const float* scale_in, int N, int K, void* stream);

typedef struct {
    const float* w; void* fwd; float* fwd_scale; void* dgrad; float* dgrad_scale;
    int32_t Cout, Cin, kh, kw;
    float fwd_inv_in, dgrad_inv_in;
} dir_train_weight;
int dir_train_pack_conv_weights(const dir_train_weight* table, const int* wg_start, int entries, int total_workgroups, void* stream);

long long dir_conv2d_splitk_workspace_bytes(const dir_conv_desc* d, int splits);
int dir_conv2d_splitk_forward(const dir_conv_desc* d, const void* x, const void* w, const float* scale, const float* shift,
                              const float* pre_scale, const float* pre_shift, const void* residual, void* y, int splits,
                              void* workspace, long long workspace_bytes, void* stream);

long long dir_conv2d_wgrad_workspace_bytes(const dir_conv_desc* d);
int dir_conv2d_wgrad_f32(const dir_conv_desc* d, const float* x, const float* gy, float* gw, int accumulate, float* workspace,
                         long long workspace_bytes, void* stream);

long long dir_conv2d_wgrad_f16x3_workspace_bytes(const dir_conv_desc* d);
int dir_conv2d_wgrad_f16x3(const dir_conv_desc* d, const float* x, const float* gy, float* gw, int accumulate, float* workspace,
                           long long workspace_bytes, float x_scale, float gy_scale, void* stream);
int dir_conv2d_wgrad_f16x3_pre(const dir_conv_desc* d, const float* x, const float* gy, float* gw, int accumulate, float* workspace,
                               long long workspace_bytes, float x_scale, float gy_scale, const float* pre_scale, const float* pre_shift, int pre_relu,
                               void* stream);

typedef struct dir_conv_src2 {
    int32_t H, W, Cin, in_cstride, in_coff, stride;
} dir_conv_src2;
int dir_conv2d_dual_forward(const dir_conv_desc* desc, const void* x, const dir_conv_src2* src2, const void* x2, const void* w,
                            const float* shift, void* y, void* stream);
int dir_conv2d_dual_scaled_forward(const dir_conv_desc* desc, const void* x, const dir_conv_src2* src2, const void* x2, const void* w,
                                   const float* scale, const float* shift, void* y, void* stream);

int dir_conv1x1_stream_forward(const dir_conv_desc* desc, const void* x, const dir_conv_src2* src2, const void* x2,
                               const void* w_stream, const float* scale, const float* shift, const float* pre_scale,
                               const float* pre_shift, void* y, void* stream);

int dir_conv2d_as_supported(const dir_conv_desc* desc, int blocks_per_wave, int pixel_blocks);
int dir_conv2d_as_forward(const dir_conv_desc* desc, const void* x, const void* w_as, const float* scale, const float* shift,
                          const void* residual, void* y, int blocks_per_wave, int pixel_blocks, void* stream);

int dir_conv2d_as_chain_supported(const dir_conv_desc* desc, int cout2, int out2_dtype);
int dir_conv2d_as_chain_forward(const dir_conv_desc* desc, const void* x, const void* w_as, const float* scale, const float* shift,
                                const void* w2_as, const float* scale2, const float* shift2, int cout2, int relu2,
                                void* y, int out_cstride, int out_coff, int out_dtype, void* stream);

int dir_conv2d_sparse_forward(const dir_conv_desc* desc_host, const void* x, const void* w, const float* scale,
                              const float* shift, const void* residual, void* y, const int32_t* group_bbox,
                              void* stream);

int dir_stem_prep(const float* img_nchw, void* out, int B, int H, int W, int Hp, int Wp, int pad, int dtype,
                  void* stream);
int dir_stem_prep_s2d(const float* img_nchw, void* out, int B, int H, int W, int Hs, int Ws, int dtype, void* stream);
int dir_maxpool3x3s2(const void* x, void* y, int B, int H, int W, int C, int dtype, void* stream);
int dir_upsample2x_bilinear(const void* x, void* y, int B, int H, int W, int C, int out_cstride, int out_coff,
                            int dtype, void* stream);
int dir_add_upsampled(void* acc, const void* src, int B, int H, int W, int C, int factor, int relu, int dtype, void* stream);
int dir_fuse_sum(void* out, const void* base, const void* const* srcs, const int* factors, int nsrc, int B, int H, int W, int C, int relu, int dtype,
                 void* stream);

typedef struct dir_init_head_params {
    const float* attn_w[2];
    float attn_b[2];
    const float* mano_wt;
    const float* mano_b[2];
    const float* off_w;
    const float* off_b;
} dir_init_head_params;
int dir_init_head_forward(const dir_init_head_params* params_host, const void* c4, const void* h_left,
                          const void* h_right, int h_cstride, float* para_left, float* para_right, float* offset,
                          int B, int HW, int C, int Ch, int dtype, void* stream);

int dir_bone_proj_forward(const float* uv_left, const float* uv_right, const float* emb, void* out, float* vis_nchw,
                          int32_t* group_bbox, int B, int S, float distance, int dtype, void* stream);

typedef struct dir_token_mlp {
    const float* w1t;
    const float* s1;
    const float* b1;
    const float* w2t;
    const float* b2;
} dir_token_mlp;

int dir_grid_tokens_forward(const void* feat, int feat_dtype, int S, int C, int feat_cstride, int feat_coff,
                            const float* uv_left,
                            const float* uv_right, const float* xyz_left, const float* xyz_right, const float* offset,
                            const dir_token_mlp* img2joint_lr_host, const dir_token_mlp* pos_emb_lr_host,
                            const dir_token_mlp* global_pos_emb_host, float* x0, float* gpos, int B, void* stream);

typedef struct dir_pgcn_layer {
    const float* W;
    const float* e1;
    const float* bias;
    const float* bn_scale;
    const float* bn_shift;
    int32_t relu;
    int32_t w_dtype;
} dir_pgcn_layer;
int dir_pgcn_stack_forward(const dir_pgcn_layer* layers_host, int num_layers, const float* x, const float* add,
                           float* out, long long out_bstride, float* scratch, int B, void* stream);

int dir_pgcn_stack_forward_pair(const dir_pgcn_layer* layers_left_host, const dir_pgcn_layer* layers_right_host,
                                int num_layers, const float* x_lr, const float* add_lr, float* tokens, float* scratch,
                                int B, void* stream);

long long dir_pgcn_fused_sync_bytes(void);
int dir_pgcn_stack_forward_fused(const dir_pgcn_layer* layers_left_host, const dir_pgcn_layer* layers_right_host, int num_layers,
                                 const float* x_lr, const float* add_lr, float* tokens, float* scratch, void* sync_ws, int splits, int B,
                                 void* stream);

typedef struct dir_ste_block {
    const float *ln1_w, *ln1_b, *qkv_wt, *qkv_b, *proj_wt, *proj_b, *ln2_w, *ln2_b, *fc1_wt, *fc1_b, *fc2_wt, *fc2_b;
} dir_ste_block;
typedef struct dir_ste_params {
    const float* pos_embed;
    dir_ste_block blocks[3];
    int32_t num_blocks;
    const float *snorm_w, *snorm_b, *head_ln_w, *head_ln_b, *head_wt , *head_b;
    int32_t weight_dtype;
} dir_ste_params;
int dir_ste_forward(const dir_ste_params* params_host, const float* x, float* x_pos_out, float* y, int B,
                    void* stream);

typedef struct dir_regress_params {
    const float* mano_wt;
    const float* mano_b[2];
    const float* off_w;
    const float* off_b;
    dir_token_mlp emb;
} dir_regress_params;
int dir_regress_forward(const dir_regress_params* params_host, const float* tok, const float* prev_para_left,
                        const float* prev_para_right, const float* prev_offset, float* para_left, float* para_right,
                        float* offset, float* emb, int B, void* stream);

typedef struct dir_bone_fusion_params {
    const float* w_g;
    const float* scale;
    const float* shift;
    int32_t exact_f32;
    float g_scale;
} dir_bone_fusion_params;
size_t dir_bone_fusion_scratch_bytes(int B);
int dir_bone_fusion_prepare(const dir_bone_fusion_params* params_host, const float* emb, void* scratch, int B, void* stream);
int dir_bone_fusion_forward(const dir_bone_fusion_params* params_host, const float* uv_left, const float* uv_right,
                            const void* scratch, void* y, int B, int S, float distance, int out_cstride, int out_coff,
                            int relu, void* stream);
long long dir_bone_fusion_backward_workspace_bytes(int B, int S);
int dir_bone_fusion_backward(const float* w_g, const float* emb, const float* uv_left, const float* uv_right, const void* g_scratch,
                             const float* gy, float distance, float* g_w_g, float* g_emb, float* g_uv_left, float* g_uv_right,
                             void* workspace, long long workspace_bytes, int B, int S, void* stream);

int dir_joint_regress_forward(const float* jr, const float* verts, float* joints, int B, void* stream);

typedef struct dir_eval_inputs {
    const float* verts_pd[2];
    const float* pd_offset;
    const float* verts_gt[2];
    const float* verts2d_gt[2];
    const float* cam;
    const float* jr[2];
} dir_eval_inputs;
typedef struct dir_eval_outputs {
    float *joint_err, *vert_err, *joint2d_err, *vert2d_err, *joints_pd, *joints_gt, *root_err;
} dir_eval_outputs;
int dir_eval_metrics_forward(const dir_eval_inputs* in_host, const dir_eval_outputs* out_host, int B, int root_joint,
                             int use_scale, void* stream);

#define DIR_VAL_MAX_STAGES 8
typedef struct dir_val_metrics_desc {
    const float* joints_pd[DIR_VAL_MAX_STAGES][2];
    const float* verts_pd[DIR_VAL_MAX_STAGES][2];
    const float* joints_gt[2];
    const float* verts_gt[2];
    double* sample_sums;
    double* acc;
    long long* batches;
} dir_val_metrics_desc;
int dir_val_metrics_forward(const dir_val_metrics_desc* desc_host, int n_stages, int B, void* stream);

int dir_gt_mano_forward(const dir_mano_tables* tables_host, const float* root_rotation, const float* pose, int ncomps,
                        const float* shape, const float* trans, const float* scale, int center_idx, int new_skel,
                        float* verts, float* joints, int B, void* stream);

int dir_image_normalize_forward(const uint8_t* img_bgr_hwc, float* out_nchw, const float* mean_host, const float* std_host,
                                int B, int H, int W, void* stream);
int dir_stem_prep_s2d_u8(const uint8_t* img_bgr_hwc, void* out, const float* mean_host, const float* std_host, int B, int H,
                         int W, int Hs, int Ws, int dtype, void* stream);

int dir_stem_pool_forward(const void* img, int img_dtype, const float* mean_host, const float* std_host, const void* w_packed,
                          const float* scale, const float* shift, void* y, int B, int H, int W, void* stream);
int dir_stem_pool_forward_dt(const void* img, int img_dtype, int out_dtype, const float* mean_host, const float* std_host, const void* w_packed,
                             const float* scale, const float* shift, void* y, int B, int H, int W, void* stream);

typedef struct dir_bneck_chain_params {
    const void* w2; const float* scale2; const float* shift2;
    const void* w3; const float* scale3; const float* shift3;
    const void* w1n; const float* scale1n; const float* shift1n;
    const void* wd;
    int32_t n_next;
    int32_t out_decimate;
    int32_t dtype;
} dir_bneck_chain_params;
int dir_bottleneck_chain_forward(const dir_bneck_chain_params* p, const void* y1, const void* residual, const void* x2, void* out,
                                 void* y1_next, int B, int H, int W, void* stream);

typedef struct dir_bneck_tail_params {
    const void* wstream;
    const float* scale3; const float* shift3;
    const float* scale1n; const float* shift1n;
    int32_t planes;
    int32_t n_next;
    int32_t waves;
    int32_t dtype;
} dir_bneck_tail_params;
int dir_bottleneck_tail_forward(const dir_bneck_tail_params* p, const void* y2, const void* residual, void* out, void* y1_next,
                                long long M, void* stream);

typedef struct dir_res_chain_params {
    const void* w1; const void* w2; const void* w3;
    const float* pre_scale; const float* pre_shift;
    const float* scale1; const float* shift1;
    const float* scale2; const float* shift2;
    const float* shift3;
    int32_t Cin, Cmid, Cout;
    int32_t dtype;
} dir_res_chain_params;
int dir_residual_chain_supported(int dtype, int Cin, int Cmid, int Cout, int B, int H, int W, int in_cstride, int in_coff, int out_cstride,
                                 int out_coff);
int dir_residual_chain_forward(const dir_res_chain_params* p, const void* x, void* out, int B, int H, int W, int in_cstride, int in_coff,
                               int out_cstride, int out_coff, void* stream);

typedef struct dir_loss_pred {
    const float* joint_uv[2];
    const float* mesh_uv[2];
    const float* proj[2];
    const float* joint_xyz[2];
    const float* mesh_xyz[2];
    const float* offset;
} dir_loss_pred;
typedef struct dir_loss_target {
    const float* joint_2d[2];
    const float* mesh_2d[2];
    const float* joint_3d[2];
    const float* mesh_3d[2];
    const float* center[2];
    const int32_t* faces[2];
    int32_t c2, n_faces;
} dir_loss_target;
int dir_stage_losses_forward(const dir_loss_pred* pred_host, const dir_loss_target* gt_host, float coord_weight, double* scratch,
                             float* out13, int B, void* stream);
long long dir_dense_losses_workspace_bytes(int B, int S);
int dir_dense_losses_forward(const float* seg_logits, const float* dense_pred, const float* gt_seg, const float* gt_dense,
                             const float* class_weight_host, float dense_weight, void* workspace, long long workspace_bytes,
                             float* out3, int B, int S, int H, int W, void* stream);

int dir_adamw_step(float* param, const float* grad, float* exp_avg, float* exp_avg_sq, long long n, double lr, double beta1,
                   double beta2, double eps, double weight_decay, long long step, void* stream);

typedef struct dir_loss_pred_grad {
    float* joint_uv[2]; float* mesh_uv[2]; float* joint_xyz[2]; float* mesh_xyz[2]; float* offset;
} dir_loss_pred_grad;
int dir_stage_losses_backward(const dir_loss_pred* pred_host, const dir_loss_target* gt_host, float coord_weight, const float* grad_out13,
                              const int32_t* const* vert_face_offsets, const int32_t* const* vert_face_index,
                              const dir_loss_pred_grad* grads_host, int B, void* stream);
long long dir_dense_losses_backward_workspace_bytes(int B, int S);
int dir_dense_losses_backward(const float* seg_logits, const float* dense_pred, const float* gt_seg, const float* gt_dense,
                              const float* class_weight_host, float dense_weight, const float* grad_out3, void* workspace,
                              long long workspace_bytes, float* grad_seg, float* grad_dense, int B, int S, int H, int W, void* stream);

long long dir_jpeg_planes_bytes(long long record_bytes);
int dir_jpeg_decode_records(const void* records, long long record_stride, int B, int H, int W, void* planes_scratch, long long scratch_bytes, void* out_bgr,
                            int32_t* err_flag, void* stream);


#define DIR_AUG_MAX_BLUR 9
#define DIR_AUG_MAX_BATCH 4096
typedef struct dir_aug_params {
    float M[6];
    int32_t flip;
    int32_t blur;
    double a[3];
    double b;
    float kernel[DIR_AUG_MAX_BLUR * DIR_AUG_MAX_BLUR];
    float pad_[3];
} dir_aug_params;
int dir_train_noise_field(unsigned long long seed, float* out, int B, void* stream);
int dir_train_augment_images(const dir_aug_params* params, const uint8_t* img, const uint8_t* mask, const uint8_t* dense,
                             const float* noise, unsigned long long seed, const float* mean_host, const float* std_host,
                             uint8_t* blur_scratch, float* img_nchw, float* img_rgb, float* mask_rgb, float* seg,
                             float* dense_out, int B, void* stream);
int dir_train_augment_labels(const dir_aug_params* params, const float* const* in_host, const float* camera, float* const* out_host,
                             int B, void* stream);

#define DIR_RENDER_VERTS 1556
#define DIR_RENDER_FACES 3076
#define DIR_RENDER_MIN_SIZE 16
#define DIR_RENDER_MAX_SIZE 1024
#define DIR_RENDER_MAX_BATCH 4096
long long dir_render_workspace_bytes(int B);
int dir_render_two_hands(const float* verts, const int32_t* faces, const float* K, const float* colors, int B, int S, void* workspace,
                         long long workspace_bytes, int32_t* pix_to_face, float* zbuf, float* bary, uint8_t* mask, uint8_t* color_u8,
                         float* color_f32, void* stream);

typedef struct dir_render_lights {
    float ambient[3], diffuse[3], specular[3];
    float location[3];
    float shininess;
} dir_render_lights;
long long dir_render_adjacency_bytes(void);
int dir_render_adjacency(const int32_t* faces, void* adjacency, long long adjacency_bytes, void* stream);
int dir_render_vertex_normals(const float* verts, const int32_t* faces, const void* adjacency, int B, float* normals, void* stream);
long long dir_render_shaded_workspace_bytes(int B);
int dir_render_shaded(const float* verts, const int32_t* faces, const void* adjacency, const float* K, const float* scale,
                      const float* trans2d, const float* colors, const dir_render_lights* lights, const uint8_t* background, int B, int S,
                      void* workspace, long long workspace_bytes, int32_t* pix_to_face, float* zbuf, float* bary, float* shaded_f32,
                      uint8_t* overlay_u8, void* stream);

int dir_render_joints(uint8_t* image, const float* uv_left, const float* uv_right, int B, int S, float joint_radius, float bone_radius,
                      void* stream);

#define DIR_MESH_MAX_VERTS 4096
#define DIR_MESH_MAX_FACES 8192
#define DIR_MESH_MAX_BATCH 65536
#define DIR_MESH_MAX_CELLS (1 << 24)
int dir_mesh_penetration(const float* verts_a, const int32_t* faces_a, const float* verts_b, const int32_t* faces_b, int B, int Va, int Fa,
                         int Vb, int Fb, float* winding, float* dist, int32_t* count, float* max_depth, float* sum_depth, void* stream);
int dir_mesh_intersection_volume(const float* verts_a, const int32_t* faces_a, const float* verts_b, const int32_t* faces_b, int B, int Va,
                                 int Fa, int Vb, int Fb, float h, int max_cells, float* volume, int32_t* n_both, int32_t* cells,
                                 void* stream);

#define DIR_ALIGN_SCALE 1
#define DIR_ALIGN_MAX_THRESHOLDS 1024
#define DIR_ALIGN_MAX_VALUES 2147483647LL
int dir_procrustes_align(const float* pd, const float* gt, int B, int N, int flags, float* transform, float* aligned, float* err,
                         void* stream);
int dir_point_set_nn(const float* a, const float* b, int B, int Na, int Nb, float* d_ab, float* d_ba, void* stream);
int dir_threshold_counts(const float* err, long long n, const float* thresholds, int K, long long* counts, void* stream);

#define DIR_CROP_MIN_SCALE 0.015625
#define DIR_CROP_MAX_SCALE 64.0
#define DIR_CROP_MAX_COORD 1048576.0
#define DIR_CROP_MIN_SIZE 16
#define DIR_CROP_MAX_SIZE 1024
#define DIR_CROP_MAX_BATCH 4096
#define DIR_CROP_MAX_SIDE 65536
#define DIR_CROP_MAX_STRIDE 1048576
#define DIR_CROP_INVALID 1
#define DIR_CROP_BAD_DESC 2
#define DIR_CROP_BAD_MATRIX 3
typedef struct dir_frame_desc {
    long long offset;
    int32_t height, width;
    long long row_stride;
} dir_frame_desc;
int dir_crop_matrices_from_boxes(const float* boxes, int B, double ratio, int size, double* M, int32_t* valid, void* stream);
int dir_crop_matrices_from_meshes(const float* mesh_left, const float* mesh_right, const float* proj_left, const float* proj_right,
                                  const double* M_prev, int B, double ratio, int size, double* M_next, int32_t* valid, void* stream);
int dir_crop_frames(const uint8_t* frames, long long frames_bytes, const dir_frame_desc* descs, const double* M, const int32_t* valid,
                    int B, int size, uint8_t* out, int32_t* status, void* stream);
int dir_crop_frames_area(const uint8_t* frames, long long frames_bytes, const dir_frame_desc* descs, const double* M, const int32_t* valid,
                         int B, int size, uint8_t* out, int32_t* status, int32_t* area, void* stream);

#define DIR_ONE_EURO_MAX_SEGMENTS 16
#define DIR_ONE_EURO_MAX_VALUES 16384
typedef struct dir_one_euro_segment {
    int32_t n_points, dims;
    float speed_scale;
} dir_one_euro_segment;
long long dir_one_euro_state_bytes(int F, int S, long long* offsets);
int dir_one_euro_step(const float* x, const int32_t* valid, int B, const dir_one_euro_segment* segments, int S, double fps, double min_cutoff,
                      double beta, double d_cutoff, int max_gap, void* state, float* y, int32_t* updated, void* stream);

#ifdef __cplusplus
}
#endif
#endif
```

Before: 28970.

## Fuse layer2 bottleneck 3x3 conv into the tail chain kernel

Adds a templated variant of the bottleneck tail kernel that computes the 3x3 conv (128->128, BN+ReLU) for a spatial 8x16 tile plus halo directly in LDS, then feeds it into the existing 1x1 expand, residual, and next-block 1x1 stages. Enabled by default for layer2 (li==1) blocks via DIR_L2_CHAIN. This removes a separate c2 conv launch and the global write/read of its intermediate activation. The trade-offs are halo recompute and reads, higher LDS use that may lower occupancy, and a tile ordering that groups tiles into contiguous chunks per block.

```diff
diff --git a/dir_amd/_capi.py b/dir_amd/_capi.py
--- a/dir_amd/_capi.py
+++ b/dir_amd/_capi.py
@@ -44,6 +44,10 @@
     _fields_ = [(n, C.c_void_p) for n in ('wstream', 'scale3', 'shift3', 'scale1n', 'shift1n')] + [('planes', C.c_int32), ('n_next', C.c_int32), ('waves', C.c_int32), ('dtype', C.c_int32)]
 
 
+class BneckC2TailParams(C.Structure):
+    _fields_ = [('tail', BneckTailParams)] + [(n, C.c_void_p) for n in ('w2', 'scale2', 'shift2')]
+
+
 class ResChainParams(C.Structure):
     _fields_ = [(n, C.c_void_p) for n in ('w1', 'w2', 'w3', 'pre_scale', 'pre_shift', 'scale1', 'shift1', 'scale2', 'shift2', 'shift3')] + [
         (n, C.c_int32) for n in ('Cin', 'Cmid', 'Cout', 'dtype')]
@@ -135,7 +139,7 @@
                 ('shininess', C.c_float)]
 
 
-ABI_VERSION = 48
+ABI_VERSION = 49
 DT_F32, DT_BF16, DT_F16X3, DT_F16X1, DT_F16X3P, DT_F16X1P, DT_F16 = 0, 1, 3, 4, 5, 6, 7
 CONV_RELU, CONV_PRE_RELU = 1, 2
 
@@ -175,6 +179,8 @@
     'dir_dense_losses_forward': (C.c_int, [_p, _p, _p, _p, C.POINTER(C.c_float), C.c_float, _p, C.c_longlong, _p, _i, _i, _i, _i, _p]),
     'dir_bottleneck_chain_forward': (C.c_int, [C.POINTER(BneckChainParams), _p, _p, _p, _p, _p, _i, _i, _i, _p]),
     'dir_bottleneck_tail_forward': (C.c_int, [C.POINTER(BneckTailParams), _p, _p, _p, _p, C.c_longlong, _p]),
+    'dir_bottleneck_c2tail_supported': (C.c_int, [C.POINTER(BneckC2TailParams), _i, _i, _i]),
+    'dir_bottleneck_c2tail_forward': (C.c_int, [C.POINTER(BneckC2TailParams), _p, _p, _p, _p, _i, _i, _i, _p]),
     'dir_residual_chain_supported': (C.c_int, [_i] * 11),
     'dir_residual_chain_forward': (C.c_int, [C.POINTER(ResChainParams), _p, _p, _i, _i, _i, _i, _i, _i, _i, _p]),
     'dir_stem_pool_forward': (C.c_int, [_p, _i, C.POINTER(C.c_float), C.POINTER(C.c_float), _p, _p, _p, _p, _i, _i, _i, _p]),
@@ -293,7 +299,7 @@
 
 PROFILE = None
 _pending = {}
-_NO_PROFILE = ('dir_conv2d_as_supported', 'dir_conv2d_as_chain_supported', 'dir_residual_chain_supported', 'dir_abi_version', 'dir_bn_one_launch_status', 'dir_bn_one_launch_enable', 'dir_last_error', 'dir_device_info', 'dir_launch_log_reset', 'dir_launch_log_get', 'dir_launch_log_note',
+_NO_PROFILE = ('dir_conv2d_as_supported', 'dir_conv2d_as_chain_supported', 'dir_residual_chain_supported', 'dir_bottleneck_c2tail_supported', 'dir_abi_version', 'dir_bn_one_launch_status', 'dir_bn_one_launch_enable', 'dir_last_error', 'dir_device_info', 'dir_launch_log_reset', 'dir_launch_log_get', 'dir_launch_log_note',
                'dir_bone_fusion_scratch_bytes', 'dir_dense_losses_workspace_bytes', 'dir_dense_losses_backward_workspace_bytes',
                'dir_gemm_f32_splitk_workspace_bytes', 'dir_bn_train_workspace_bytes', 'dir_bn_sync_workspace_bytes', 'dir_bn_frozen_workspace_bytes', 'dir_jpeg_planes_bytes', 'dir_render_workspace_bytes', 'dir_render_adjacency_bytes', 'dir_render_shaded_workspace_bytes', 'dir_colsum_workspace_bytes', 'dir_conv2d_wgrad_workspace_bytes', 'dir_conv2d_wgrad_f16x3_workspace_bytes',
                'dir_one_euro_state_bytes')
diff --git a/dir_amd/csrc/tail.hip b/dir_amd/csrc/tail.hip
--- a/dir_amd/csrc/tail.hip
+++ b/dir_amd/csrc/tail.hip
@@ -32,11 +32,22 @@
 constexpr int NTHR = 512;
 constexpr int TPITCH = HC * 2 + 16;
 
+constexpr int C2_TH = 8, C2_TW = 16, C2_NPX = C2_TH * C2_TW;
+constexpr int C2_PWD = C2_TW + 2, C2_NPP = (C2_TH + 2) * C2_PWD;
+constexpr int C2_YPITCH = 272;
+constexpr int C2_Y1ROW = 5120;
+constexpr int C2_Y1BYTES = (C2_TH + 2) * C2_Y1ROW, C2_Y2BYTES = C2_NPX * C2_YPITCH;
+constexpr int C2_FRAG = 4 * 64;
+constexpr int C2_STEPS = 18;
+constexpr int C2_NPIECE = (C2_NPP * 16 + NTHR - 1) / NTHR;
+
 struct TailArgs {
     const bf16_t* y2; const bf16_t* res; bf16_t* out; bf16_t* y1n;
     const uint4* wstream;
     const float* sc3; const float* sh3; const float* sc1n; const float* sh1n;
     int ntiles; unsigned y2_bytes;
+    const uint4* w2; const float* sc2; const float* sh2;
+    int H, W, tiles_x, tiles_y;
 };
 
 template <typename H> __device__ __forceinline__ void unpack4(uint2 v, float (&f)[4]) {
@@ -44,9 +55,10 @@
     convk::unpack2<H>(v.y, f[2], f[3]);
 }
 
-template <int P, int N2, typename H = bf16_t>
+template <int P, int N2, typename H = bf16_t, bool C2 = false>
 __global__ __launch_bounds__(NTHR, 1) void tail_chain_kernel(TailArgs a) {
     convk::half_kernel_init<H>();
+    static_assert(!C2 || P == 128, "tail_chain_kernel: the fused 3x3 is built for P = 128");
     constexpr int C4 = 4 * P, NH = C4 / HC;
     constexpr int YROW = P * 2;
     constexpr int GRP = P == 256 ? 4 : 8;
@@ -58,20 +70,36 @@
     static_assert(NF % GRP == 0 && C4 % HC == 0 && (N2 == 128 || N2 == 256), "tail_chain_kernel: unsupported geometry");
     constexpr int YCH = TM * (P / 8) / NTHR;
     __shared__ __attribute__((aligned(16))) char s_t[TM * TPITCH];
-    __shared__ __attribute__((aligned(16))) char s_y2[2][TM * YROW];
-    __shared__ __attribute__((aligned(16))) float s_ss[2 * C4 + 2 * N2];
+    __shared__ __attribute__((aligned(16))) char s_y2[C2 ? C2_Y1BYTES + C2_Y2BYTES : 2 * TM * YROW];
+    __shared__ __attribute__((aligned(16))) float s_ss[2 * C4 + 2 * N2 + (C2 ? 2 * P : 0)];
+    constexpr int NU = C2 ? 2 : NH;
     const int tid = threadIdx.x, lane = tid & 63, wave = __builtin_amdgcn_readfirstlane(tid >> 6);
     const int l32 = lane & 31, h = lane >> 5, l16 = lane & 15, g16 = lane >> 4;
 
     for (int i = tid; i < C4; i += NTHR) { s_ss[i] = a.sc3[i]; s_ss[C4 + i] = a.sh3[i]; }
     for (int i = tid; i < N2; i += NTHR) { s_ss[2 * C4 + i] = a.sc1n[i]; s_ss[2 * C4 + N2 + i] = a.sh1n[i]; }
-
-    const int tstep = gridDim.x;
-    int t = blockIdx.x;
-    if (t >= a.ntiles) return;
+    if constexpr (C2) {
+        if (tid < P) { s_ss[2 * C4 + 2 * N2 + tid] = a.sc2[tid]; s_ss[2 * C4 + 2 * N2 + P + tid] = a.sh2[tid]; }
+    }
+
+    int tstep = gridDim.x, t = blockIdx.x, tend = a.ntiles;
+    if constexpr (C2) {
+        if ((gridDim.x & 7) == 0 && a.ntiles % 8 == 0) {
+            const int per = a.ntiles >> 3;
+            t = (blockIdx.x & 7) * per + (blockIdx.x >> 3); tstep = gridDim.x >> 3; tend = ((blockIdx.x & 7) + 1) * per;
+        }
+    }
+    if (t >= tend) return;
+    auto tile_base = [&](auto tile) {
+        const int tx = tile % a.tiles_x, r_ = tile / a.tiles_x, b = r_ / a.tiles_y, ty = r_ - b * a.tiles_y;
+        return (b * a.H + ty * C2_TH) * a.W + tx * C2_TW;
+    };
+    auto gpix = [&](int tb, int u, int p) -> long long { return (long long)tb * TM + p; };
+    auto gpix2 = [&](int tb, int rows, int lrow, int lcol) -> long long { return ((long long)tb + rows * a.W) + (lrow * a.W + lcol); };
+    auto launder = [](int v) { asm volatile("" : "+v"(v)); return v; };
 
     const convk::i32x4 yd = {(int)(unsigned)(unsigned long long)a.y2, (int)(unsigned)((unsigned long long)a.y2 >> 32), (int)a.y2_bytes, 0x00020000};
-    const unsigned y2_lds = (unsigned)(unsigned long long)(__attribute__((address_space(3))) char*)&s_y2[0][0];
+    const unsigned y2_lds = (unsigned)(unsigned long long)(__attribute__((address_space(3))) char*)&s_y2[0];
     auto y2_dma = [&](int tile, int buf) {
 #pragma unroll
         for (int i = 0; i < YCH; ++i) {
@@ -85,7 +113,9 @@
     auto res_fetch = [&](int tile, int half) {
 #pragma unroll
         for (int pb = 0; pb < 2; ++pb) {
-            const bf16_t* rp = a.res + ((long long)tile * TM + 32 * pb + l32) * C4 + half * HC + 64 * wave + 8 * h;
+            const bf16_t* rp;
+            if constexpr (C2) { const int ll = launder(lane); rp = a.res + gpix2(tile, 4 * half + 2 * pb, (ll & 31) >> 4, ll & 15) * C4 + 64 * wave + 8 * (ll >> 5); }
+            else rp = a.res + gpix(tile, half, 32 * pb + l32) * C4 + half * HC + 64 * wave + 8 * h;
 #pragma unroll
             for (int cb = 0; cb < 2; ++cb)
 #pragma unroll
@@ -96,7 +126,9 @@
     auto res_fetch = [&](int tile, int half) {
 #pragma unroll
         for (int pb = 0; pb < 2; ++pb) {
-            const bf16_t* rp = a.res + ((long long)tile * TM + 32 * pb + l32) * C4 + half * HC + 64 * wave + 4 * h;
+            const bf16_t* rp;
+            if constexpr (C2) rp = a.res + gpix2(tile, 4 * half + 2 * pb, l32 >> 4, l32 & 15) * C4 + 64 * wave + 4 * h;
+            else rp = a.res + gpix(tile, half, 32 * pb + l32) * C4 + half * HC + 64 * wave + 4 * h;
 #pragma unroll
             for (int cb = 0; cb < 2; ++cb)
 #pragma unroll
@@ -112,9 +144,57 @@
         for (int i = 0; i < GRP; ++i) ring[slot][i] = p[i * 64];
     };
 
-    y2_dma(t, 0);
+    const int cb2 = wave & 3, pg2 = wave >> 2;
+    char* const s_y1 = s_y2;
+    char* const s_y2t = s_y2 + (C2 ? C2_Y1BYTES : 0);
+    const __amdgpu_buffer_rsrc_t r2 = __builtin_amdgcn_make_buffer_rsrc((void*)a.w2, 0, C2 ? P * 9 * P * 2 : 0, 0x00020000);
+    const int vB = (cb2 * C2_STEPS * C2_FRAG + lane) * 16;
+    convk::u32x4 wr[C2 ? 3 : 1][4];
+    auto wload = [&](auto S) {
+        constexpr int s = decltype(S)::value;
+#pragma unroll
+        for (int ks = 0; ks < 4; ++ks)
+            wr[s % 3][ks] = __builtin_bit_cast(convk::u32x4, __builtin_amdgcn_raw_buffer_load_b128(r2, vB, (s * C2_FRAG + ks * 64) * 16, 0));
+    };
+    static_assert(C2_NPIECE % 2 == 0, "patch pieces per unit");
+    constexpr int NPU = C2_NPIECE / 2;
+    uint4 pv[C2 ? NPU : 1];
+    auto patch_fetch = [&](auto tile, int u) {
+        const int tx = tile % a.tiles_x, r_ = tile / a.tiles_x, b = r_ / a.tiles_y, y0 = (r_ - b * a.tiles_y) * C2_TH, x0 = tx * C2_TW;
+        const int tl = launder(tid);
+#pragma unroll
+        for (int i = 0; i < NPU; ++i) {
+            const int e = tl + NTHR * (NPU * u + i), pp = min(e >> 4, C2_NPP - 1), pr = pp / C2_PWD, pc = pp - pr * C2_PWD;
+            const int iy = min(max(y0 - 1 + pr, 0), a.H - 1), ix = min(max(x0 - 1 + pc, 0), a.W - 1);
+            pv[i] = *reinterpret_cast<const uint4*>(a.y2 + ((long long)(b * a.H + iy) * a.W + ix) * P + (e & 15) * 8);
+        }
+    };
+    auto patch_store = [&](auto tile, int u) {
+        const int tx = tile % a.tiles_x, r_ = tile / a.tiles_x, b = r_ / a.tiles_y, y0 = (r_ - b * a.tiles_y) * C2_TH, x0 = tx * C2_TW;
+        const int tl = launder(tid);
+#pragma unroll
+        for (int i = 0; i < NPU; ++i) {
+            const int e = tl + NTHR * (NPU * u + i), pp = e >> 4, pr = pp / C2_PWD, pc = pp - pr * C2_PWD;
+            const int iy = y0 - 1 + pr, ix = x0 - 1 + pc;
+            const bool in = iy >= 0 && iy < a.H && ix >= 0 && ix < a.W;
+            if (pp < C2_NPP) *reinterpret_cast<uint4*>(s_y1 + pr * C2_Y1ROW + pc * C2_YPITCH + (e & 15) * 16) = in ? pv[i] : make_uint4(0u, 0u, 0u, 0u);
+        }
+    };
+
+    int tb = t, tbn = t;
+    if constexpr (C2) {
+        tb = tbn = tile_base(t);
+        patch_fetch(t, 0);
+        patch_store(t, 0);
+        patch_fetch(t, 1);
+        wload(std::integral_constant<int, 0>{});
+        wload(std::integral_constant<int, 1>{});
+    } else {
+        y2_dma(t, 0);
+    }
     ring_load(std::integral_constant<int, 0>{}, 0, 0);
-    res_fetch(t, 0);
+    res_fetch(tb, 0);
+    if constexpr (C2) patch_store(t, 1);
     convk::wait_vmcnt<0>();
     __syncthreads();
     int ybuf = 0;
@@ -124,14 +204,15 @@
     f32x4 accc16[C16 ? 4 : 1];
     constexpr int NOP = C16 ? 4 : 2;
     uint4 bop[2][NOP];
-    const char* ycur = s_y2[0];
+    const char* ycur = s_y2;
     auto act_read = [&](auto F, auto Set) {
         constexpr int f = decltype(F)::value, set = decltype(Set)::value;
         if constexpr (f < NBF) {
             constexpr int ks = f % KBS;
 #pragma unroll
             for (int pb = 0; pb < 2; ++pb)
-                bop[set][pb] = *reinterpret_cast<const uint4*>(ycur + (32 * pb + l32) * YROW + (((2 * ks + h) ^ (l32 & 15)) << 4));
+                if constexpr (C2) bop[set][pb] = *reinterpret_cast<const uint4*>(ycur + (32 * pb + l32) * C2_YPITCH + ((2 * ks + h) << 4));
+                else bop[set][pb] = *reinterpret_cast<const uint4*>(ycur + (32 * pb + l32) * YROW + (((2 * ks + h) ^ (l32 & 15)) << 4));
         } else {
             constexpr int fc = f - NBF;
             if constexpr (C16) {
@@ -144,14 +225,70 @@
         }
     };
 
-    for (; t < a.ntiles; t += tstep) {
-        const bool more = t + tstep < a.ntiles;
-        if (more) y2_dma(t + tstep, ybuf ^ 1);
-        ycur = s_y2[ybuf];
+    for (; t < tend; t += tstep) {
+        const bool more = t + tstep < tend;
+        const int tn = more ? t + tstep : t;
+        if constexpr (C2) {
+            tb = tbn;
+            tbn = tile_base(tn);
+            {
+                f32x16 acc[2];
+#pragma unroll
+                for (int j = 0; j < 2; ++j)
+#pragma unroll
+                    for (int r = 0; r < 16; ++r) acc[j][r] = 0.f;
+                const char* bB = s_y1 + (4 * pg2 + (l32 >> 4)) * C2_Y1ROW + (l32 & 15) * C2_YPITCH + 64 * h;
+                uint4 bv[2][2];
+                auto bread = [&](auto I) {
+                    constexpr int i = decltype(I)::value, s = i >> 2, ks = i & 3, slab = s / 9, tap = s % 9, ky = tap / 3, kx = tap % 3;
+#pragma unroll
+                    for (int j = 0; j < 2; ++j) bv[i & 1][j] = *reinterpret_cast<const uint4*>(bB + (ky + 2 * j) * C2_Y1ROW + kx * C2_YPITCH + slab * 128 + 16 * ks);
+                };
+                bread(std::integral_constant<int, 0>{});
+                [&]<int... Ss>(std::integer_sequence<int, Ss...>) {
+                    (([&] {
+                         constexpr int s = Ss;
+                         __builtin_amdgcn_sched_barrier(0);
+                         if constexpr (s + 2 < C2_STEPS) wload(std::integral_constant<int, s + 2>{});
+                         [&]<int... Ks>(std::integer_sequence<int, Ks...>) {
+                             (([&] {
+                                  constexpr int i = 4 * s + Ks;
+                                  if constexpr (i + 1 < 4 * C2_STEPS) bread(std::integral_constant<int, i + 1>{});
+                                  __builtin_amdgcn_sched_barrier(0);
+#pragma unroll
+                                  for (int j = 0; j < 2; ++j) acc[j] = Half<H>::mfma32(wr[s % 3][Ks], bv[i & 1][j], acc[j]);
+                              }()),
+                              ...);
+                         }(std::make_integer_sequence<int, 4>{});
+                     }()),
+                     ...);
+                }(std::make_integer_sequence<int, C2_STEPS>{});
+#pragma unroll
+                for (int j = 0; j < 2; ++j)
+#pragma unroll
+                    for (int q = 0; q < 4; ++q) {
+                        const int c0 = 32 * cb2 + 8 * q + 4 * h;
+                        const float4 sc = *reinterpret_cast<const float4*>(s_ss + 2 * C4 + 2 * N2 + c0);
+                        const float4 sh = *reinterpret_cast<const float4*>(s_ss + 2 * C4 + 2 * N2 + P + c0);
+                        uint2 o;
+                        o.x = Half<H>::pack2_relu(fmaf(acc[j][4 * q], sc.x, sh.x), fmaf(acc[j][4 * q + 1], sc.y, sh.y));
+                        o.y = Half<H>::pack2_relu(fmaf(acc[j][4 * q + 2], sc.z, sh.z), fmaf(acc[j][4 * q + 3], sc.w, sh.w));
+                        const int ll = launder(lane);
+                        *reinterpret_cast<uint2*>(s_y2t + (64 * pg2 + 32 * j + (ll & 31)) * C2_YPITCH + (32 * cb2 + 8 * q + 4 * (ll >> 5)) * 2) = o;
+                    }
+            }
+            __syncthreads();
+        } else {
+            if (more) y2_dma(t + tstep, ybuf ^ 1);
+            ycur = s_y2 + ybuf * (TM * YROW);
+            tb = t; tbn = t + tstep;
+        }
 #pragma nounroll
-        for (int hf = 0; hf < NH; ++hf) {
-            const bool last_half = hf == NH - 1;
-            if (hf == 0) {
+        for (int hf = 0; hf < NU; ++hf) {
+            const bool last_half = hf == NU - 1;
+            const int whf = C2 ? 0 : hf;
+            if constexpr (C2) ycur = s_y2t + 64 * hf * C2_YPITCH;
+            if (C2 || hf == 0) {
                 if constexpr (C16) {
 #pragma unroll
                     for (int u = 0; u < 4; ++u) accc16[u] = f32x4{0.f, 0.f, 0.f, 0.f};
@@ -166,8 +303,8 @@
             [&]<int... G>(std::integer_sequence<int, G...>) {
                 (([&] {
                      constexpr int grp = G, slot = G & 1;
-                     if constexpr (grp + 1 < NG) ring_load(std::integral_constant<int, slot ^ 1>{}, hf, grp + 1);
-                     else ring_load(std::integral_constant<int, slot ^ 1>{}, last_half ? 0 : hf + 1, 0);
+                     if constexpr (grp + 1 < NG) ring_load(std::integral_constant<int, slot ^ 1>{}, whf, grp + 1);
+                     else ring_load(std::integral_constant<int, slot ^ 1>{}, (C2 || last_half) ? 0 : hf + 1, 0);
                      [&]<int... I>(std::integer_sequence<int, I...>) {
                          (([&] {
                               constexpr int f = grp * GRP + I, set = f & 1;
@@ -187,8 +324,8 @@
 #pragma unroll
                                       for (int q = 0; q < 4; ++q) {
                                           const int cl = 64 * wave + 32 * cb + 8 * q + 4 * h;
-                                          const float4 sc = *reinterpret_cast<const float4*>(s_ss + hf * HC + cl);
-                                          const float4 sh = *reinterpret_cast<const float4*>(s_ss + C4 + hf * HC + cl);
+                                          const float4 sc = *reinterpret_cast<const float4*>(s_ss + whf * HC + cl);
+                                          const float4 sh = *reinterpret_cast<const float4*>(s_ss + C4 + whf * HC + cl);
 #pragma unroll
                                           for (int pb = 0; pb < 2; ++pb) {
                                               float v[4] = {fmaf(accb[pb][4 * q], sc.x, sh.x), fmaf(accb[pb][4 * q + 1], sc.y, sh.y),
@@ -217,17 +354,23 @@
                                   if constexpr (f == NBF - 1) {
                                       __syncthreads();
                                       act_read(std::integral_constant<int, NBF>{}, std::integral_constant<int, set ^ 1>{});
-                                      if (!last_half) res_fetch(t, hf + 1);
+                                      if constexpr (C2) res_fetch(last_half ? tbn : tb, last_half ? 0 : 1);
+                                      else if (!last_half) res_fetch(t, hf + 1);
                                       else if (more) res_fetch(t + tstep, 0);
 #pragma unroll
                                       for (int i = 0; i < TM * (HC / 8) / NTHR; ++i) {
                                           const int c = tid + NTHR * i;
+                                          if constexpr (C2)
+                                              NT_STORE(*reinterpret_cast<const uint4*>(s_t + (c >> 6) * TPITCH + (c & 63) * 16),
+                                                       reinterpret_cast<uint4*>(a.out + gpix2(tb, 4 * hf + (i >> 1), 0, wave + 8 * (i & 1)) * C4 + lane * 8));
+                                          else
                                           NT_STORE(*reinterpret_cast<const uint4*>(s_t + (c >> 6) * TPITCH + (c & 63) * 16),
-                                                   reinterpret_cast<uint4*>(a.out + ((long long)t * TM + (c >> 6)) * C4 + hf * HC + (c & 63) * 8));
+                                                   reinterpret_cast<uint4*>(a.out + gpix(tb, hf, c >> 6) * C4 + whf * HC + (c & 63) * 8));
                                           if (i & 1) __builtin_amdgcn_sched_barrier(0);
                                       }
                                   }
                               } else {
+                                  if constexpr (C2 && f == NBF + 2) patch_fetch(tn, hf);
                                   if constexpr (C16) {
 #pragma unroll
                                       for (int u = 0; u < 4; ++u)
@@ -238,7 +381,7 @@
                                           accc32[pb] = Half<H>::mfma32(ring[slot][I], bop[set][pb], accc32[pb]);
                                   }
                               }
-                              if constexpr (f == NF - 1) convk::wait_vmcnt<GRP>();
+                              if constexpr (f == NF - 1 && !C2) convk::wait_vmcnt<GRP>();
                               __builtin_amdgcn_sched_barrier(0);
                           }()),
                           ...);
@@ -246,7 +389,7 @@
                  }()),
                  ...);
             }(std::make_integer_sequence<int, NG>{});
-            if (last_half) {
+            if (C2 || last_half) {
                 if constexpr (C16) {
                     const int c0 = 16 * wave + 4 * g16;
                     const float4 sc = *reinterpret_cast<const float4*>(s_ss + 2 * C4 + c0);
@@ -256,7 +399,8 @@
                         uint2 o;
                         o.x = Half<H>::pack2_relu(fmaf(accc16[u][0], sc.x, sh.x), fmaf(accc16[u][1], sc.y, sh.y));
                         o.y = Half<H>::pack2_relu(fmaf(accc16[u][2], sc.z, sh.z), fmaf(accc16[u][3], sc.w, sh.w));
-                        *reinterpret_cast<uint2*>(a.y1n + ((long long)t * TM + 16 * u + l16) * N2 + c0) = o;
+                        if constexpr (C2) *reinterpret_cast<uint2*>(a.y1n + gpix2(tb, 4 * hf + u, 0, l16) * N2 + c0) = o;
+                        else *reinterpret_cast<uint2*>(a.y1n + gpix(tb, hf, 16 * u + l16) * N2 + c0) = o;
                     }
                 } else {
 #pragma unroll
@@ -275,16 +419,22 @@
                         for (int j = 0; j < 2; ++j) {
                             const auto dx = __builtin_amdgcn_permlane32_swap(o[2 * j].x, o[2 * j + 1].x, false, false);
                             const auto dy = __builtin_amdgcn_permlane32_swap(o[2 * j].y, o[2 * j + 1].y, false, false);
-                            *reinterpret_cast<uint4*>(a.y1n + ((long long)t * TM + 32 * pb + l32) * N2 + 32 * wave + 16 * j + 8 * h) = make_uint4(dx[0], dy[0], dx[1], dy[1]);
+                            *reinterpret_cast<uint4*>(a.y1n + (C2 ? gpix2(tb, 4 * hf + 2 * pb, (launder(lane) & 31) >> 4, launder(lane) & 15) : gpix(tb, hf, 32 * pb + l32)) * N2 + 32 * wave + 16 * j + 8 * h) = make_uint4(dx[0], dy[0], dx[1], dy[1]);
                         }
 #else
 #pragma unroll
                         for (int q = 0; q < 4; ++q)
-                            *reinterpret_cast<uint2*>(a.y1n + ((long long)t * TM + 32 * pb + l32) * N2 + 32 * wave + 8 * q + 4 * h) = o[q];
+                            *reinterpret_cast<uint2*>(a.y1n + (C2 ? gpix2(tb, 4 * hf + 2 * pb, l32 >> 4, l32 & 15) : gpix(tb, hf, 32 * pb + l32)) * N2 + 32 * wave + 8 * q + 4 * h) = o[q];
 #endif
                     }
                 }
             }
+            if constexpr (C2) patch_store(tn, hf);
+            if (!C2 || !last_half) __syncthreads();
+        }
+        if constexpr (C2) {
+            wload(std::integral_constant<int, 0>{});
+            wload(std::integral_constant<int, 1>{});
             __syncthreads();
         }
         ybuf ^= 1;
@@ -480,6 +630,7 @@
     a.y2 = (const convk::bf16_t*)y2; a.res = (const convk::bf16_t*)residual; a.out = (convk::bf16_t*)out; a.y1n = (convk::bf16_t*)y1_next;
     a.wstream = (const uint4*)p->wstream; a.sc3 = p->scale3; a.sh3 = p->shift3; a.sc1n = p->scale1n; a.sh1n = p->shift1n;
     a.ntiles = (int)(M / TM);
+    a.w2 = nullptr; a.sc2 = a.sh2 = nullptr; a.H = a.W = a.tiles_x = a.tiles_y = 0;
     DIR_REQUIRE(M * p->planes * 2 < (1ll << 31), "dir_bottleneck_tail_forward: y2 must be < 2 GiB (32-bit buffer offsets)");
     a.y2_bytes = (unsigned)(M * p->planes * 2);
     static int num_cu = 0;
@@ -510,3 +661,44 @@
 #undef DIR_TAIL
     return check_launch("dir_bottleneck_tail_forward");
 }
+
+extern "C" int dir_bottleneck_c2tail_supported(const dir_bneck_c2tail_params* p, int B, int H, int W) {
+    using namespace dir;
+    if (!p) return 0;
+    if (p->tail.dtype != DIR_DT_BF16 && p->tail.dtype != DIR_DT_F16) return 0;
+    if (p->tail.planes != 128 || (p->tail.n_next != 128 && p->tail.n_next != 256) || p->tail.waves != 8) return 0;
+    if (B <= 0 || H < C2_TH || W < C2_TW || H % C2_TH || W % C2_TW) return 0;
+    if ((long long)B * H * W * (4 * p->tail.planes) >= (1ll << 31)) return 0;
+    return 1;
+}
+
+extern "C" int dir_bottleneck_c2tail_forward(const dir_bneck_c2tail_params* p, const void* y1, const void* residual, void* out, void* y1_next,
+                                             int B, int H, int W, void* stream) {
+    using namespace dir;
+    DIR_REQUIRE(p && y1 && residual && out && y1_next, "dir_bottleneck_c2tail_forward: null pointer");
+    DIR_REQUIRE(p->tail.wstream && p->tail.scale3 && p->tail.shift3 && p->tail.scale1n && p->tail.shift1n && p->w2 && p->scale2 && p->shift2,
+                "dir_bottleneck_c2tail_forward: missing parameters");
+    DIR_REQUIRE(dir_bottleneck_c2tail_supported(p, B, H, W),
+                "dir_bottleneck_c2tail_forward: unsupported (bf16 / f16 storage, planes 128, n_next 128 or 256, a stream packed for 8 waves, H a multiple "
+                "of 8 and W of 16, tensors below 2^31 elements)");
+    TailArgs a;
+    a.y2 = (const convk::bf16_t*)y1; a.res = (const convk::bf16_t*)residual; a.out = (convk::bf16_t*)out; a.y1n = (convk::bf16_t*)y1_next;
+    a.wstream = (const uint4*)p->tail.wstream; a.sc3 = p->tail.scale3; a.sh3 = p->tail.shift3; a.sc1n = p->tail.scale1n; a.sh1n = p->tail.shift1n;
+    a.w2 = (const uint4*)p->w2; a.sc2 = p->scale2; a.sh2 = p->shift2;
+    a.H = H; a.W = W; a.tiles_x = W / C2_TW; a.tiles_y = H / C2_TH; a.ntiles = B * a.tiles_x * a.tiles_y;
+    a.y2_bytes = 0;
+    static int num_cu = 0;
+    if (!num_cu) {
+        int dev = 0; hipDeviceProp_t pr;
+        num_cu = (hipGetDevice(&dev) == hipSuccess && hipGetDeviceProperties(&pr, dev) == hipSuccess) ? pr.multiProcessorCount : 256;
+    }
+    const int grid = a.ntiles < num_cu ? a.ntiles : num_cu;
+    hipStream_t s = (hipStream_t)stream;
+    const bool f16 = p->tail.dtype == DIR_DT_F16;
+#define DIR_C2TAIL(N2_) do { if (f16) DIR_LAUNCH((tail_chain_kernel<128, N2_, f16s_t, true>), dim3(grid), dim3(NTHR), 0, s, a); \
+                              else DIR_LAUNCH((tail_chain_kernel<128, N2_, bf16_t, true>), dim3(grid), dim3(NTHR), 0, s, a); } while (0)
+    if (p->tail.n_next == 128) DIR_C2TAIL(128);
+    else DIR_C2TAIL(256);
+#undef DIR_C2TAIL
+    return check_launch("dir_bottleneck_c2tail_forward");
+}
diff --git a/dir_amd/engine.py b/dir_amd/engine.py
--- a/dir_amd/engine.py
+++ b/dir_amd/engine.py
@@ -518,6 +518,53 @@
         return out, y1n
 
 
+class BneckC2TailOp(object):
+
+    l2_chain = os.environ.get('DIR_L2_CHAIN', '1') != '0'
+
+    def __init__(self, c2, tail):
+        self.c2, self.tail = c2, tail
+        self.cout, self.cin, self.kh, self.kw, self.stride = c2.cout, c2.cin, c2.kh, c2.kw, c2.stride
+        self.variant = c2.variant
+        self.w2 = pack_as_weights(c2.w, 1)
+        self.params = _capi.BneckC2TailParams(tail.params[8], _capi.ptr(self.w2), _capi.ptr(c2.scale), _capi.ptr(c2.shift))
+
+    @staticmethod
+    def applies(c2, tail, dtype):
+        return (dtype in HALF and c2.dtype == dtype and c2.out_dtype == dtype and c2.arith is None and c2.pre_scale is None and c2.scale is not None
+                and (c2.kh, c2.kw, c2.stride, c2.pad, c2.cin, c2.cout) == (3, 3, 1, 1, 128, 128) and c2.flags == CONV_RELU
+                and tail.c3.cin == 128 and tail.c3.dtype == dtype)
+
+    def supported(self, B, H, W):
+        return bool(_capi.lib().dir_bottleneck_c2tail_supported(C.byref(self.params), B, H, W))
+
+    def __call__(self, y1, x, out=None, y1n=None):
+        B, H, W, P = y1.shape
+        c4, n2 = self.tail.c3.cout, self.tail.c1n.cout
+        if (y1.dtype != self.c2.dtype or x.dtype != y1.dtype or P != self.c2.cin or tuple(x.shape) != (B, H, W, c4) or not y1.is_contiguous() or not x.is_contiguous()
+                or (out is not None and (out.dtype != y1.dtype or tuple(out.shape) != (B, H, W, c4) or not out.is_contiguous()))
+                or (y1n is not None and (y1n.dtype != y1.dtype or tuple(y1n.shape) != (B, H, W, n2) or not y1n.is_contiguous()))
+                or not self.supported(B, H, W)):
+            return None
+        if getattr(_TLS, 'capture_fused', None) is not None:
+            _TLS.capture_fused.append((self, (y1, x), {}))
+        if out is None:
+            out = torch.empty(B, H, W, c4, device=y1.device, dtype=y1.dtype)
+        if y1n is None:
+            y1n = torch.empty(B, H, W, n2, device=y1.device, dtype=y1.dtype)
+        if getattr(_TLS, 'capture', None) is not None:
+            _TLS.capture.append((self, (y1, x), dict(out=out, y1n=y1n)))
+        if _capi.PROFILE is not None:
+            m, c2 = B * H * W, self.c2
+            _capi.annotate(family='conv', flops=2.0 * m * c2.cout * c2.alg_k + 2.0 * m * (P * c4 + c4 * n2), op=c2, covers=(self.tail,), dtype='bf16',
+                           shape='M=%d 3x3(%d)+tail 1x1(%d->%d)+res+1x1(->%d)' % (m, P, P, c4, n2),
+                           bytes=(m * c2.cin * y1.element_size() + c2.w.numel() * c2.w.element_size() + m * c2.cout * y1.element_size()
+                                  + (m * (P + 2 * c4 + n2) + c4 * P + n2 * c4) * 2))
+        _capi.check(_capi.lib().dir_bottleneck_c2tail_forward(C.byref(self.params), _capi.ptr(y1), _capi.ptr(x), _capi.ptr(out), _capi.ptr(y1n),
+                                                              B, H, W, _capi.stream_ptr()), 'dir_bottleneck_c2tail_forward')
+        return out, y1n
+
+
 def stem_conv_op(w, scale, shift, dtype):
     wp = torch.zeros(64, 64, 4, 1, device=w.device, dtype=F32)
     for r in range(4):
@@ -596,6 +643,10 @@
                     nxt = blocks[i + 1]['c1'] if i + 1 < len(blocks) else self.layers[li + 1][0]['c1']
                     if BneckTailOp.applies(blk['c3'], nxt, dt):
                         blk['tail'] = BneckTailOp(blk['c3'], nxt)
+                        if li == 1 and BneckC2TailOp.l2_chain and BneckC2TailOp.applies(blk['c2'], blk['tail'], dt):
+                            fused = BneckC2TailOp(blk['c2'], blk['tail'])
+                            if fused.supported(1, 32, 32):
+                                blk['c2tail'] = fused
 
     def __call__(self, img):
         L, dt, dev = _capi.lib(), self.dtype, self.device
@@ -660,10 +711,12 @@
                     x_dec = dec
                     continue
                 if 'tail' in blk and (x.shape[0] * x.shape[1] * x.shape[2]) % 64 == 0:
-                    if out_last is not None and li == upto - 1 and bi == len(blocks) - 1:
-                        x, y1 = blk['tail'](blk['c2'](y1 if y1 is not None else blk['c1'](x)), x, out=out_last[0], y1n=out_last[1])
+                    dst = dict(out=out_last[0], y1n=out_last[1]) if out_last is not None and li == upto - 1 and bi == len(blocks) - 1 else {}
+                    y1 = y1 if y1 is not None else blk['c1'](x)
+                    r = blk['c2tail'](y1, x, **dst) if 'c2tail' in blk and BneckC2TailOp.l2_chain else None
+                    x, y1 = r if r is not None else blk['tail'](blk['c2'](y1), x, **dst)
+                    if dst:
                         continue
-                    x, y1 = blk['tail'](blk['c2'](y1 if y1 is not None else blk['c1'](x)), x)
                 elif 'dual' in blk:
                     x, y1 = blk['dual'](blk['c2'](y1 if y1 is not None else blk['c1'](x)), x, x_decimated=x_dec), None
                     x_dec = False
diff --git a/include/dir_hip.h b/include/dir_hip.h
--- a/include/dir_hip.h
+++ b/include/dir_hip.h
@@ -13,7 +13,7 @@
 #define DIR_E_LAUNCH (-2)
 #define DIR_E_NODEVICE (-3)
 
-#define DIR_ABI_VERSION 48
+#define DIR_ABI_VERSION 49
 
 int dir_abi_version(void);
 const char* dir_last_error(void);
@@ -400,6 +400,15 @@
 int dir_bottleneck_tail_forward(const dir_bneck_tail_params* p, const void* y2, const void* residual, void* out, void* y1_next,
                                 long long M, void* stream);
 
+typedef struct dir_bneck_c2tail_params {
+    dir_bneck_tail_params tail;
+    const void* w2;
+    const float* scale2; const float* shift2;
+} dir_bneck_c2tail_params;
+int dir_bottleneck_c2tail_supported(const dir_bneck_c2tail_params* p, int B, int H, int W);
+int dir_bottleneck_c2tail_forward(const dir_bneck_c2tail_params* p, const void* y1, const void* residual, void* out, void* y1_next,
+                                  int B, int H, int W, void* stream);
+
 typedef struct dir_res_chain_params {
     const void* w1; const void* w2; const void* w3;
     const float* pre_scale; const float* pre_shift;
```

Result: no change. 29300, median of 6 (+1.1%).
